# imironhead/ml_super_resolution

Measured on AMD Instinct MI355X. Metric: VDSR-20 training patches/sec (41x41, batch 256 per GPU); fwd HR megapixels/sec alongside, higher is better.
Workload: dtype f32; 1 GPU; BASELINE configs[2]: VDSR 20-layer 3x3x64 residual, RGB, batch 256x41x41 per GPU, fwd+bwd+TF-Adam, random-init weights; global_batch=256, patch=41, parallelism=dp1

## Files before the change

### include/srx.h

```cpp
#ifndef SRX_H_
#define SRX_H_

#include <stddef.h>
#include <stdint.h>

#ifdef __cplusplus
extern "C" {
#endif

typedef void* srx_stream_t;

typedef enum {
    SRX_OK = 0,
    SRX_ERR_BAD_ARG = -1,
    SRX_ERR_UNSUPPORTED = -2,
    SRX_ERR_WORKSPACE = -3,
    SRX_ERR_LAUNCH = -4,
    SRX_ERR_ALIGN = -5
} srx_status;

typedef enum { SRX_PAD_SAME = 0, SRX_PAD_VALID = 1 } srx_pad_mode;

typedef enum {
    SRX_ACT_NONE = 0,
    SRX_ACT_RELU = 1,
    SRX_ACT_TANH = 2,
    SRX_ACT_LRELU = 3,
    SRX_ACT_SIGMOID = 4
} srx_act;

typedef enum { SRX_OP_FWD = 0, SRX_OP_BWD_DATA = 1, SRX_OP_BWD_FILTER = 2 } srx_conv_op;

typedef enum { SRX_PRECISION_FP32 = 0, SRX_PRECISION_BF16X3 = 1 } srx_precision;

typedef struct {
    int32_t N, H, W, Cin, Cout, KH, KW;
    int32_t stride;
    int32_t pad_mode;
    int32_t act;
    int32_t post_add_relu;
    int32_t precision;
    int32_t subpixel_r;
} srx_conv_desc;

const char* srx_version(void);
const char* srx_last_error(void);

int srx_set_conv_path(int pipelined);

int srx_set_wgrad_path(int path);

int srx_conv_chain(const srx_conv_desc* d, int op, int in_act, int layers, const float* const* x, const float* const* w,
                   const float* const* bias, const float* const* aux, float* const* y, srx_stream_t stream);

int srx_conv_chain_supported(const srx_conv_desc* d, int op, int in_act);

int srx_set_chain(int on);

int srx_set_chain_fixed(int on);

int srx_conv2d_precision_supported(const srx_conv_desc* d, int op);

size_t srx_conv2d_workspace_bytes(const srx_conv_desc* d, int op);

int srx_conv2d_fwd(const srx_conv_desc* d, const float* x, const float* w, const float* bias,
                   const float* skip, float* y, void* ws, size_t ws_bytes, srx_stream_t stream);

int srx_conv2d_bwd_data(const srx_conv_desc* d, const float* dpre, const float* w,
                        const float* x_in, int in_act, float* dx_out, void* ws, size_t ws_bytes,
                        srx_stream_t stream);

int srx_conv2d_bwd_data_acc(const srx_conv_desc* d, const float* dpre, const float* w, const float* dx_acc,
                            float* dx_out, void* ws, size_t ws_bytes, srx_stream_t stream);

int srx_conv2d_bwd_filter(const srx_conv_desc* d, const float* x, const float* dpre, float* dw,
                          float* dbias, const float* w_for_decay, float wd_scale, void* ws,
                          size_t ws_bytes, srx_stream_t stream);

int srx_conv2d_bwd_filter_partials(const srx_conv_desc* d, const float* x, const float* dpre, void* ws,
                                   size_t ws_bytes, int* n_partials, srx_stream_t stream);
int srx_conv2d_bwd_filter_reduce(const srx_conv_desc* d, const void* ws, int n_partials, float* dw,
                                 float* dbias, const float* w_for_decay, float wd_scale,
                                 srx_stream_t stream);

int srx_conv2d_bwd_filter_batch(const srx_conv_desc* d, int n_layers, const float* const* x, const float* const* dpre,
                                float* const* dw, float* const* dbias, const float* const* w_for_decay, float wd_scale,
                                void* ws, size_t ws_bytes, srx_stream_t stream);
size_t srx_conv2d_bwd_filter_batch_workspace_bytes(const srx_conv_desc* d, int n_layers);
int srx_conv2d_bwd_filter_batch_plan(const srx_conv_desc* d, int n_layers, int* wgs_per_layer, int* grid);
int srx_set_wgrad_batch(int on);

int srx_act_bwd(const float* dy, const float* y, float* dpre, size_t numel, int act,
                srx_stream_t stream);

int srx_depth_to_space(const float* in, float* out, int N, int H, int W, int C, int r,
                       srx_stream_t stream);

int srx_stream_copy(const void* in, void* out, size_t bytes, srx_stream_t stream);

int srx_espcn_forward(const float* x, const float* w1, const float* b1, const float* w2, const float* b2,
                      const float* w3, const float* b3, float* hr, int N, int H, int W, int r,
                      srx_stream_t stream);
int srx_espcn_forward_keep(const float* x, const float* w1, const float* b1, const float* w2, const float* b2,
                           const float* w3, const float* b3, float* t1, float* t2, float* y, int N, int H, int W, int r,
                           srx_stream_t stream);

int srx_srcnn_forward(const float* x, const float* w1, const float* b1, const float* w2, const float* b2,
                      const float* w3, const float* b3, float* y, int N, int H, int W, srx_stream_t stream);

int srx_space_to_depth(const float* in, float* out, int N, int H, int W, int C, int r,
                       srx_stream_t stream);

int srx_mse_fwd_bwd(const float* pred, const float* target, size_t numel, float inv_numel,
                    float* loss_out, int accumulate, float* dpred, void* scratch,
                    srx_stream_t stream);

int srx_l2_loss(const float* w, const float* mask, size_t numel, float scale, float* loss_out,
                int accumulate, void* scratch, srx_stream_t stream);

size_t srx_reduce_scratch_bytes(void);

int srx_adam_tf_step(float* w, const float* g, float* m, float* v, size_t numel, float lr,
                     float beta1, float beta2, float eps, int64_t t, float grad_scale,
                     srx_stream_t stream);

int srx_adam_tf_step_dev(float* w, const float* g, float* m, float* v, size_t numel, void* state,
                         float beta1, float beta2, float eps, float grad_scale, srx_stream_t stream);

int srx_momentum_clip_step(float* w, const float* g, float* acc, size_t numel, float lr,
                           float momentum, float cap, float grad_scale, srx_stream_t stream);

int srx_rownorm_loss_fwd_bwd(const float* pred, const float* target, size_t rows, size_t row_len,
                             float* loss_out, float* dpred, float* row_norms, srx_stream_t stream);

int srx_psnr(const float* a, const float* b, float* out, int N, size_t per_image, float max_val,
             srx_stream_t stream);

int srx_ssim(const float* a, const float* b, float* out, int N, int H, int W, int C, float max_val,
             void* scratch, srx_stream_t stream);
size_t srx_ssim_scratch_bytes(int N);

#define SRX_SCORES_MAX_CAND 4
#define SRX_SCORES_RGB 0
#define SRX_SCORES_Y   1
#define SRX_SCORES_MAX_TAP_STRIDE 46
typedef struct srx_scores_desc {
    int32_t N, H, W, C;
    int32_t n_cand;
    int32_t space;
    int32_t unit_clip;
    float   max_val;
} srx_scores_desc;
size_t srx_image_scores_scratch_bytes(const srx_scores_desc* d);
int srx_image_scores_plan(const srx_scores_desc* d, int* tile_h, int* tile_w, int* tiles_y, int* tiles_x);
size_t srx_image_scores_lds_bytes(const srx_scores_desc* d);
int srx_image_scores(const srx_scores_desc* d, const float* ref, const float* const* cand, float* out, void* scratch,
                     srx_stream_t stream);

int srx_saturate_u8(const float* x, uint8_t* out, size_t numel, srx_stream_t stream);

#define SRX_FEATURE_MOSAIC_TW 128
int srx_feature_mosaic_u8(const float* x, uint8_t* out, int N, int H, int W, srx_stream_t stream);

#define SRX_SUMMARY_PANEL_MAX_SRC 8
#define SRX_SUMMARY_RANGE_BLOCKS 256
typedef struct srx_panel_src {
    const float* x;
    int32_t W;
    int32_t reserved;
    int64_t row_pitch;
    int64_t image_pitch;
} srx_panel_src;
size_t srx_summary_panel_bytes(const srx_panel_src* srcs, int n_src, int N, int H, int r);
size_t srx_summary_panel_range_bytes(void);
int srx_summary_panel_u8(const srx_panel_src* srcs, int n_src, int N, int H, int r, const float* range_dev, uint8_t* out,
                         srx_stream_t stream);
int srx_summary_panel_range(const srx_panel_src* srcs, int n_src, int N, int H, int r, float* range_dev,
                            srx_stream_t stream);

int srx_affine(const float* x, float* out, size_t numel, float a, float b, srx_stream_t stream);


int srx_u8_to_unit_float(const uint8_t* in, float* out, size_t numel, srx_stream_t stream);

int srx_gaussian_blur(const float* in, float* out, float* tmp, int N, int H, int W, int C, float sigma,
                      srx_stream_t stream);

int srx_resize_bilinear(const float* in, float* out, int N, int H, int W, int C, int OH, int OW,
                        srx_stream_t stream);


typedef struct srx_patch_src {
    uint64_t offset;
    int32_t width, height;
    int32_t x, y;
    int32_t flip;
    float scaling_factor;
} srx_patch_src;

int srx_vdsr_patch_table_check(const srx_patch_src* table_host, int B, int S, size_t arena_bytes);

int srx_vdsr_patch_pairs(const uint8_t* arena, const srx_patch_src* table_dev, int B, int S,
                         float* sd, float* hd, srx_stream_t stream);


int srx_espcn_patch_table_check(const srx_patch_src* table_host, int n, int r, int p, size_t arena_bytes);

int srx_espcn_patch_pairs(const uint8_t* arena, const srx_patch_src* table_dev, int B, int r, int p,
                          float* lr, float* label, srx_stream_t stream);


#define SRX_ESPCN_EVAL_TILE 16

typedef struct srx_eval_image {
    uint64_t offset;
    int32_t width, height;
    uint64_t lr_offset;
    uint32_t first_tile;
    uint32_t reserved;
} srx_eval_image;

int srx_espcn_eval_table_check(const srx_eval_image* table_host, int n, int r, size_t arena_bytes, size_t lr_floats);

size_t srx_espcn_eval_tiles(const srx_eval_image* table_host, int n, int r);

int srx_espcn_eval_pairs(const uint8_t* arena, const srx_eval_image* table_dev, int n, int r,
                         float* lr, float* label, srx_stream_t stream);


int srx_enet_pairs_table_words(int S);

int srx_enet_pairs_tables(int S, int32_t* words_host);

int srx_enet_patch_table_check(const srx_patch_src* table_host, int B, int S, size_t arena_bytes);

int srx_enet_patch_pairs(const uint8_t* arena, const srx_patch_src* table_dev, int B, int S, const int32_t* tables_dev,
                         float* sd, float* bq, float* hd, srx_stream_t stream);


int srx_srcnn_pairs_band(int S, int f);

int srx_srcnn_pairs_lds_bytes(int S, int f);

// ... 95 lines not shown
```

### ml_super_resolution_amd/_lib.py

```python
import ctypes
import os

_HERE = os.path.dirname(os.path.abspath(__file__))
LIB_PATH = os.path.join(_HERE, 'libsrx.so')

SRX_OK = 0
PAD_SAME, PAD_VALID = 0, 1
ACT_NONE, ACT_RELU, ACT_TANH, ACT_LRELU, ACT_SIGMOID = 0, 1, 2, 3, 4
OP_FWD, OP_BWD_DATA, OP_BWD_FILTER = 0, 1, 2
PRECISION_FP32, PRECISION_BF16X3 = 0, 1
PRECISION_BY_NAME = {'highest': PRECISION_FP32, 'high': PRECISION_BF16X3}

ACT_BY_NAME = {None: ACT_NONE, 'none': ACT_NONE, 'relu': ACT_RELU, 'tanh': ACT_TANH,
               'lrelu': ACT_LRELU, 'leaky_relu': ACT_LRELU, 'sigmoid': ACT_SIGMOID}
PAD_BY_NAME = {'same': PAD_SAME, 'valid': PAD_VALID}

EXPORTS = [
    'srx_version', 'srx_last_error', 'srx_set_conv_path', 'srx_set_wgrad_path', 'srx_set_chain', 'srx_set_chain_fixed', 'srx_conv_chain', 'srx_conv_chain_supported', 'srx_conv2d_precision_supported', 'srx_conv2d_workspace_bytes', 'srx_conv2d_fwd',
    'srx_conv2d_bwd_data', 'srx_conv2d_bwd_filter', 'srx_conv2d_bwd_filter_partials', 'srx_conv2d_bwd_filter_reduce',
    'srx_conv2d_bwd_filter_batch', 'srx_conv2d_bwd_filter_batch_workspace_bytes', 'srx_conv2d_bwd_filter_batch_plan', 'srx_set_wgrad_batch', 'srx_act_bwd', 'srx_depth_to_space',
    'srx_space_to_depth', 'srx_stream_copy', 'srx_mse_fwd_bwd', 'srx_l2_loss', 'srx_reduce_scratch_bytes',
    'srx_adam_tf_step', 'srx_adam_tf_step_dev', 'srx_momentum_clip_step', 'srx_rownorm_loss_fwd_bwd', 'srx_psnr', 'srx_ssim', 'srx_ssim_scratch_bytes', 'srx_saturate_u8', 'srx_affine', 'srx_u8_to_unit_float', 'srx_gaussian_blur', 'srx_resize_bilinear',
    'srx_upsample_nearest', 'srx_upsample_nearest_bwd', 'srx_add_relu_grad',
    'srx_conv2d_bwd_data_acc', 'srx_conv3x3_blocked', 'srx_conv3x3_blocked_bwd_filter_workspace_bytes', 'srx_conv3x3_blocked_bwd_filter',
    'srx_conv3x3_blocked_ex', 'srx_conv3x3_blocked_bwd_filter_ex_workspace_bytes', 'srx_conv3x3_blocked_bwd_filter_ex',
    'srx_espcn_forward', 'srx_espcn_forward_keep', 'srx_debug_poison_lds', 'srx_srcnn_forward', 'srx_maxpool2x2', 'srx_maxpool2x2_bwd', 'srx_maxpool2x2_bwd_masked', 'srx_subsample2', 'srx_subsample2_bwd',
    'srx_channel_blocks_to_nhwc', 'srx_nhwc_to_channel_blocks', 'srx_channel_normalize', 'srx_channel_normalize_bwd',
    'srx_extract_patches16', 'srx_texture_gram', 'srx_texture_gram_bwd', 'srx_pil_resample_ksize', 'srx_pil_resample_coeffs', 'srx_resample_u8', 'srx_u8_to_pm1', 'srx_log_loss', 'srx_vgg_preprocess', 'srx_add_scaled', 'srx_resize_bicubic_tf', 'srx_column_sums', 'srx_gemm_workspace_bytes', 'srx_gemm',
    'srx_feature_mosaic_u8', 'srx_summary_panel_bytes', 'srx_summary_panel_range_bytes', 'srx_summary_panel_u8', 'srx_summary_panel_range',
    'srx_vdsr_patch_table_check', 'srx_vdsr_patch_pairs',
    'srx_espcn_patch_table_check', 'srx_espcn_patch_pairs',
    'srx_espcn_eval_table_check', 'srx_espcn_eval_tiles', 'srx_espcn_eval_pairs',
    'srx_enet_pairs_table_words', 'srx_enet_pairs_tables', 'srx_enet_patch_table_check', 'srx_enet_patch_pairs',
    'srx_image_scores_scratch_bytes', 'srx_image_scores_plan', 'srx_image_scores_lds_bytes', 'srx_image_scores',
    'srx_srcnn_pairs_band', 'srx_srcnn_pairs_lds_bytes', 'srx_srcnn_patch_table_check', 'srx_srcnn_patch_pairs',
]


class SrxError(RuntimeError):
    pass


class ConvDesc(ctypes.Structure):
    _fields_ = [(n, ctypes.c_int32) for n in
                ('N', 'H', 'W', 'Cin', 'Cout', 'KH', 'KW', 'stride', 'pad_mode', 'act',
                 'post_add_relu', 'precision', 'subpixel_r')]


class PatchSrc(ctypes.Structure):
    _fields_ = [('offset', ctypes.c_uint64), ('width', ctypes.c_int32), ('height', ctypes.c_int32), ('x', ctypes.c_int32),
                ('y', ctypes.c_int32), ('flip', ctypes.c_int32), ('scaling_factor', ctypes.c_float)]


class EvalImage(ctypes.Structure):
    _fields_ = [('offset', ctypes.c_uint64), ('width', ctypes.c_int32), ('height', ctypes.c_int32), ('lr_offset', ctypes.c_uint64),
                ('first_tile', ctypes.c_uint32), ('reserved', ctypes.c_uint32)]


ESPCN_EVAL_TILE = 16


class PanelSrc(ctypes.Structure):
    _fields_ = [('x', ctypes.c_void_p), ('W', ctypes.c_int32), ('reserved', ctypes.c_int32), ('row_pitch', ctypes.c_int64),
                ('image_pitch', ctypes.c_int64)]


class ScoresDesc(ctypes.Structure):
    _fields_ = [(n, ctypes.c_int32) for n in ('N', 'H', 'W', 'C', 'n_cand', 'space', 'unit_clip')] + [('max_val', ctypes.c_float)]


SCORES_MAX_CAND = 4
SCORES_RGB, SCORES_Y = 0, 1
SCORES_MAX_TAP_STRIDE = 46
SCORES_SPACE_BY_NAME = {'rgb': SCORES_RGB, 'y': SCORES_Y}


class GemmDesc(ctypes.Structure):
    _fields_ = ([(n, ctypes.c_int32) for n in ('M', 'N', 'K', 'batch')] +
                [(n, ctypes.c_int64) for n in ('a_row_stride', 'a_col_stride', 'a_batch_stride', 'b_row_stride',
                                               'b_col_stride', 'b_batch_stride', 'c_row_stride', 'c_col_stride',
                                               'c_batch_stride')] +
                [('alpha', ctypes.c_float), ('act', ctypes.c_int32), ('accumulate', ctypes.c_int32)])


_lib = None


def lib():
    global _lib
    if _lib is not None:
        return _lib
    if not os.path.exists(LIB_PATH):
        raise SrxError('libsrx.so not found at %s -- build it with `make -C %s` (or '
                       '__graft_entry__.build()); there is no CPU fallback' %
                       (LIB_PATH, os.path.join(_HERE, 'csrc')))
    import torch
    L = ctypes.CDLL(LIB_PATH)
    vp, sz, i, f = ctypes.c_void_p, ctypes.c_size_t, ctypes.c_int, ctypes.c_float
    dp = ctypes.POINTER(ConvDesc)
    L.srx_version.restype = ctypes.c_char_p
    L.srx_last_error.restype = ctypes.c_char_p
    L.srx_set_conv_path.argtypes = [i]
    L.srx_set_wgrad_path.argtypes = [i]
    L.srx_set_chain.argtypes = [i]
    L.srx_set_chain_fixed.argtypes = [i]
    L.srx_conv_chain_supported.argtypes = [dp, i, i]
    L.srx_conv_chain.argtypes = [dp, i, i, i, vp, vp, vp, vp, vp, vp]
    L.srx_conv2d_precision_supported.argtypes = [dp, i]
    L.srx_conv2d_workspace_bytes.argtypes = [dp, i]
    L.srx_conv2d_workspace_bytes.restype = sz
    L.srx_reduce_scratch_bytes.restype = sz
    L.srx_conv2d_fwd.argtypes = [dp, vp, vp, vp, vp, vp, vp, sz, vp]
    L.srx_conv2d_bwd_data.argtypes = [dp, vp, vp, vp, i, vp, vp, sz, vp]
    L.srx_conv2d_bwd_filter.argtypes = [dp, vp, vp, vp, vp, vp, f, vp, sz, vp]
    L.srx_conv2d_bwd_filter_partials.argtypes = [dp, vp, vp, vp, sz, ctypes.POINTER(ctypes.c_int), vp]
    L.srx_conv2d_bwd_filter_reduce.argtypes = [dp, vp, i, vp, vp, vp, f, vp]
    L.srx_conv2d_bwd_filter_batch.argtypes = [dp, i, vp, vp, vp, vp, vp, f, vp, sz, vp]
    L.srx_conv2d_bwd_filter_batch_workspace_bytes.argtypes = [dp, i]
    L.srx_conv2d_bwd_filter_batch_workspace_bytes.restype = sz
    L.srx_conv2d_bwd_filter_batch_plan.argtypes = [dp, i, ctypes.POINTER(ctypes.c_int), ctypes.POINTER(ctypes.c_int)]
    L.srx_set_wgrad_batch.argtypes = [i]
    L.srx_act_bwd.argtypes = [vp, vp, vp, sz, i, vp]
    L.srx_depth_to_space.argtypes = [vp, vp, i, i, i, i, i, vp]
    L.srx_space_to_depth.argtypes = [vp, vp, i, i, i, i, i, vp]
    L.srx_stream_copy.argtypes = [vp, vp, sz, vp]
    L.srx_mse_fwd_bwd.argtypes = [vp, vp, sz, f, vp, i, vp, vp, vp]
    L.srx_l2_loss.argtypes = [vp, vp, sz, f, vp, i, vp, vp]
    L.srx_adam_tf_step.argtypes = [vp, vp, vp, vp, sz, f, f, f, f, ctypes.c_int64, f, vp]
    L.srx_adam_tf_step_dev.argtypes = [vp, vp, vp, vp, sz, vp, f, f, f, f, vp]
    L.srx_momentum_clip_step.argtypes = [vp, vp, vp, sz, f, f, f, f, vp]
    L.srx_rownorm_loss_fwd_bwd.argtypes = [vp, vp, sz, sz, vp, vp, vp, vp]
    L.srx_psnr.argtypes = [vp, vp, vp, i, sz, f, vp]
    L.srx_ssim.argtypes = [vp, vp, vp, i, i, i, i, f, vp, vp]
    L.srx_ssim_scratch_bytes.argtypes = [i]
    L.srx_ssim_scratch_bytes.restype = sz
    sp, ip = ctypes.POINTER(ScoresDesc), ctypes.POINTER(ctypes.c_int)
    L.srx_image_scores_scratch_bytes.argtypes = [sp]
    L.srx_image_scores_scratch_bytes.restype = sz
    L.srx_image_scores_plan.argtypes = [sp, ip, ip, ip, ip]
    L.srx_image_scores_lds_bytes.argtypes = [sp]
    L.srx_image_scores_lds_bytes.restype = sz
    L.srx_image_scores.argtypes = [sp, vp, vp, vp, vp, vp]
    L.srx_saturate_u8.argtypes = [vp, vp, sz, vp]
    L.srx_feature_mosaic_u8.argtypes = [vp, vp, i, i, i, vp]
    L.srx_summary_panel_bytes.argtypes = [vp, i, i, i, i]
    L.srx_summary_panel_bytes.restype = sz
    L.srx_summary_panel_range_bytes.restype = sz
    L.srx_summary_panel_u8.argtypes = [vp, i, i, i, i, vp, vp, vp]
    L.srx_summary_panel_range.argtypes = [vp, i, i, i, i, vp, vp]
    L.srx_vdsr_patch_table_check.argtypes = [vp, i, i, sz]
    L.srx_vdsr_patch_pairs.argtypes = [vp, vp, i, i, vp, vp, vp]
    L.srx_espcn_patch_table_check.argtypes = [vp, i, i, i, sz]
    L.srx_espcn_patch_pairs.argtypes = [vp, vp, i, i, i, vp, vp, vp]
    L.srx_espcn_eval_table_check.argtypes = [vp, i, i, sz, sz]
    L.srx_espcn_eval_tiles.argtypes = [vp, i, i]
    L.srx_espcn_eval_tiles.restype = sz
    L.srx_espcn_eval_pairs.argtypes = [vp, vp, i, i, vp, vp, vp]
    L.srx_enet_pairs_table_words.argtypes = [i]
    L.srx_enet_pairs_tables.argtypes = [i, vp]
    L.srx_enet_patch_table_check.argtypes = [vp, i, i, sz]
    L.srx_enet_patch_pairs.argtypes = [vp, vp, i, i, vp, vp, vp, vp, vp]
    L.srx_srcnn_pairs_band.argtypes = [i, i]
    L.srx_srcnn_pairs_lds_bytes.argtypes = [i, i]
    L.srx_srcnn_patch_table_check.argtypes = [vp, i, i, i, i, sz]
    L.srx_srcnn_patch_pairs.argtypes = [vp, vp, i, i, i, i, vp, vp, vp]
    L.srx_affine.argtypes = [vp, vp, sz, f, f, vp]
    L.srx_u8_to_unit_float.argtypes = [vp, vp, sz, vp]
    L.srx_gaussian_blur.argtypes = [vp, vp, vp, i, i, i, i, f, vp]
    L.srx_resize_bilinear.argtypes = [vp, vp, i, i, i, i, i, i, vp]
    L.srx_upsample_nearest.argtypes = [vp, vp, i, i, i, i, i, vp]
    L.srx_upsample_nearest_bwd.argtypes = [vp, vp, i, i, i, i, i, vp]
    L.srx_add_relu_grad.argtypes = [vp, vp, vp, vp, sz, vp]
    L.srx_conv2d_bwd_data_acc.argtypes = [dp, vp, vp, vp, vp, vp, sz, vp]
    L.srx_espcn_forward.argtypes = [vp] * 8 + [i, i, i, i, vp]
    L.srx_espcn_forward_keep.argtypes = [vp] * 10 + [i, i, i, i, vp]
    L.srx_debug_poison_lds.argtypes = [vp]
    L.srx_srcnn_forward.argtypes = [vp, vp, vp, vp, vp, vp, vp, vp, i, i, i, vp]
    L.srx_conv3x3_blocked.argtypes = [vp, vp, vp, vp, i, vp, i, i, i, i, i, i, i, vp]
    L.srx_conv3x3_blocked_bwd_filter_workspace_bytes.restype = sz
    L.srx_conv3x3_blocked_bwd_filter_workspace_bytes.argtypes = [i, i, i, i, i]
    L.srx_conv3x3_blocked_bwd_filter.argtypes = [vp, vp, vp, vp, i, i, i, i, i, vp, sz, vp]
    L.srx_conv3x3_blocked_ex.argtypes = [vp, vp, vp, vp, i, vp, i, i, i, i, i, i, i, i, vp]
    L.srx_conv3x3_blocked_bwd_filter_ex_workspace_bytes.restype = sz
    L.srx_conv3x3_blocked_bwd_filter_ex_workspace_bytes.argtypes = [i, i, i, i, i, i]
    L.srx_conv3x3_blocked_bwd_filter_ex.argtypes = [vp, vp, vp, vp, i, i, i, i, i, i, vp, sz, vp]
    L.srx_texture_gram.argtypes = [vp, vp, i, i, i, i, f, vp]
    L.srx_texture_gram_bwd.argtypes = [vp, vp, vp, i, i, i, i, f, f, vp]
    L.srx_pil_resample_ksize.argtypes = [i, i, i]
    L.srx_pil_resample_coeffs.argtypes = [i, i, i, vp, vp]
    L.srx_resample_u8.argtypes = [vp, vp, ctypes.c_long, i, i, ctypes.c_long, vp, vp, i, vp]
    L.srx_u8_to_pm1.argtypes = [vp, vp, sz, vp]
    L.srx_maxpool2x2.argtypes = [vp, vp, i, i, i, i, vp]
    L.srx_maxpool2x2_bwd.argtypes = [vp, vp, vp, i, i, i, i, vp]
    L.srx_maxpool2x2_bwd_masked.argtypes = [vp, vp, vp, i, i, i, i, i, vp]
    L.srx_subsample2.argtypes = [vp, vp, i, i, i, i, i, i, vp]
    L.srx_subsample2_bwd.argtypes = [vp, vp, i, i, i, i, i, i, vp]
    L.srx_channel_blocks_to_nhwc.argtypes = [vp, vp, sz, i, vp]
    L.srx_nhwc_to_channel_blocks.argtypes = [vp, vp, sz, i, vp]
    L.srx_channel_normalize.argtypes = [vp, vp, sz, i, f, vp]
    L.srx_channel_normalize_bwd.argtypes = [vp, vp, vp, sz, i, f, vp]
    L.srx_extract_patches16.argtypes = [vp, vp, i, i, i, i, i, vp]
    L.srx_log_loss.argtypes = [vp, f, i, f, f, f, vp, i, vp, vp]
    L.srx_vgg_preprocess.argtypes = [vp, vp, sz, i, vp]
    L.srx_column_sums.argtypes = [vp, vp, i, i, i, vp]
    L.srx_add_scaled.argtypes = [vp, vp, vp, sz, f, f, vp]
    L.srx_resize_bicubic_tf.argtypes = [vp, vp, i, i, i, i, i, i, vp]
    L.srx_gemm_workspace_bytes.argtypes = [i, i, i, i]
    L.srx_gemm_workspace_bytes.restype = sz
    L.srx_gemm.argtypes = [ctypes.POINTER(GemmDesc), vp, vp, vp, vp, vp, sz, vp]
    for name in EXPORTS:
        getattr(L, name)
    _lib = L
    return L


def check(rc, what):
    if rc != SRX_OK:
        raise SrxError('%s failed (status %d): %s' % (what, rc, lib().srx_last_error().decode()))
```

### ml_super_resolution_amd/csrc/conv_kernels.hip.h

```cpp
#pragma once
#include <hip/hip_runtime.h>
#include <stdint.h>
#include <type_traits>

namespace srx {

typedef float f32x4 __attribute__((ext_vector_type(4)));

enum { ACT_NONE = 0, ACT_RELU = 1, ACT_TANH = 2, ACT_LRELU = 3, ACT_SIGMOID = 4 };

struct ConvArgs {
    const float* x;
    const float* w;
    const float* bias;
    const float* skip;
    const float* mask;
    float* y;
    int N, H, W, OH, OW, Cin, Cout;
    int pad_t, pad_l;
    int TH, TW, NTX, RS;
    int units_total;
    int act, post_relu, mask_act;
    float inv_rs;
    int stagger;
// ... 2627 lines not shown
                       "+a"(bnext[21]), "+a"(bnext[22]), "+a"(bnext[23]), "+a"(bnext[24]), "+a"(bnext[25]),        \
                       "+a"(bnext[26]), "+a"(bnext[27]), "+a"(bnext[28]), "+a"(bnext[29]), "+a"(bnext[30]));       \
        _Pragma("unroll") for (int j = 0; j < U; ++j)                                                              \
            asm volatile("v_accvgpr_read_b32 %0, %1" : "=v"(bcur[j]) : "a"(bnext[j]));                             \
    } while (0)

    int u = u0;
    int n, h, th;
    tile_of(u, n, h, th);
    [[maybe_unused]] unsigned long long t_loop = 0, t_end = 0;
    [[maybe_unused]] const unsigned long long t_begin = SRX_STAMP();
    __syncthreads();
    {
        StageSeq qi, qc;
        stage_setup(qi, qc, h, th, 0, true);
        stage_tile_scalar<CINP, 6>(qi, qc, SG, x_rsrc(n), voff_lane, wl_lane);
        dpre_window_now(b_rsrc(n, h, th));
        lds_barrier();
        SRX_TAKE_OVER_B();
    }
    int cur_buf = 0;
    while (u < u1) {
        tile_of(u, n, h, th);
        const int un_ = u + th;
        const bool has_next = un_ < u1;
        int n2 = n, h2 = h, th2 = th;
        if (has_next) tile_of(un_, n2, h2, th2);
        StageSeq qi, qc;
        stage_setup(qi, qc, h2, th2, cur_buf ^ 1, has_next);
        const __amdgpu_buffer_rsrc_t xrs = x_rsrc(n2);
        const __amdgpu_buffer_rsrc_t brs_pf = b_rsrc(n2, h2, has_next ? th2 : 0);

        auto xaddr = [&](int k, int i) -> unsigned {
            if (i == U - 1) return (unsigned)(xw[k] + dX + (OWC - 1) * PS * 4);
            const int r = i >= U ? THC : i / SPR, j = i >= U ? 0 : i % SPR;
            return (unsigned)(xw[k] + (r * RSZ + 4 * j) * PS * 4);
        };
        auto read_x = [&](int k, int i) -> f32x4 { return *(lds_f32x4*)(uintptr_t)xaddr(k, i); };
        f32x4 ring[RN];
#pragma unroll
        for (int f = 0; f < LA; ++f) ring[f] = read_x(f % QW, f / QW);

        const unsigned long long ts_l = SRX_STAMP();
        f32x4 stg[NPASSES];
        auto step = [&](auto IC) {
            constexpr int i = decltype(IC)::value;
            const float b = bcur[i];
            bsum += b;
            unsigned long long smk = 0, smt = 0;
            int sso = 0;
#pragma unroll
            for (int k = 0; k < QW; ++k) {
                const int idx = (i * QW + k) % RN;
                const int kk = k + LA;
                ring[(idx + LA) % RN] = read_x(kk % QW, i + kk / QW);
                mfma4_wgrad(acc[k], ring[idx], b);
                if ((k == 1 && 2 * i < U) || (k == 7 && 2 * i + 1 < U)) {
                    const int p = 2 * i + (k == 7 ? 1 : 0);
                    if (p == U - 1) {
                        bnext[p] = dpre_fire_imm<0>(brs_pf, vX, 0);
                    } else {
                        const int r = p / SPR, j = p % SPR;
                        const int vb = j < 4 ? vb0 : (j < 8 ? vb1 : vb2);
                        const int so = r == 0 ? 0 : (r == 1 ? srow1 : srow2);
                        switch (j % 4) {
                            case 0: bnext[p] = dpre_fire_imm<0>(brs_pf, vb, so); break;
                            case 1: bnext[p] = dpre_fire_imm<16 * COUTC>(brs_pf, vb, so); break;
                            case 2: bnext[p] = dpre_fire_imm<32 * COUTC>(brs_pf, vb, so); break;
                            default: bnext[p] = dpre_fire_imm<48 * COUTC>(brs_pf, vb, so); break;
                        }
                    }
                }
                if constexpr (i < NPASSES) {
                    if (k == 2) { if (i > 0) stage_next<PPP * CINP * 4>(qi, SG.JP1, SG.rowfix_g); }
                    if (k == 3) stage_mask_a(qi, SG, smk, smt);
                    if (k == 4) stage_mask_b(qi, smk, smt, sso);
                    if (k == 6) stg[i < NPASSES ? i : 0] = stage_fire_a(smk, sso, xrs, voff_lane);
                }
                if constexpr (i == NPASSES) { if (k == 2) stage_next<PPP * CINP * 4>(qi, SG.JP1, SG.rowfix_g); }
                if constexpr (i >= C0 && i < C0 + NPASSES) {
                    constexpr int jj = i - C0;
                    constexpr int after = 1 + 3 * (NPASSES - 1 - jj) + (U - 2 * NPASSES);
                    if (k == 0) stage_commit_a(after >= 14 ? 14 : (after & ~1), qc, stage_mask_full(qc, SG), wl_lane, stg[jj < NPASSES ? jj : 0]);
                    if (k == 4) stage_next<PPP * PS * 4>(qc, SG.JP1, SG.rowfix_l);
                }
            }
        };
#define SRX_ONE_STEP(I) step(std::integral_constant<int, I>{});
        SRX_ONE_STEP(0) SRX_ONE_STEP(1) SRX_ONE_STEP(2) SRX_ONE_STEP(3) SRX_ONE_STEP(4) SRX_ONE_STEP(5) SRX_ONE_STEP(6) SRX_ONE_STEP(7)
        SRX_ONE_STEP(8) SRX_ONE_STEP(9) SRX_ONE_STEP(10) SRX_ONE_STEP(11) SRX_ONE_STEP(12) SRX_ONE_STEP(13) SRX_ONE_STEP(14) SRX_ONE_STEP(15)
        SRX_ONE_STEP(16) SRX_ONE_STEP(17) SRX_ONE_STEP(18) SRX_ONE_STEP(19) SRX_ONE_STEP(20) SRX_ONE_STEP(21) SRX_ONE_STEP(22) SRX_ONE_STEP(23)
        SRX_ONE_STEP(24) SRX_ONE_STEP(25) SRX_ONE_STEP(26) SRX_ONE_STEP(27) SRX_ONE_STEP(28) SRX_ONE_STEP(29) SRX_ONE_STEP(30)
#undef SRX_ONE_STEP
        SRX_TAKE_OVER_B();
        const unsigned long long ts_e = SRX_STAMP();
        t_loop += ts_e - ts_l;
        {
            const int flip = __builtin_amdgcn_readfirstlane(cur_buf ? -buf_bytes : buf_bytes);
#pragma unroll
            for (int k = 0; k < QW; ++k) { xw[k] += flip; SRX_PIN(xw[k]); }
        }
        stage_tile_scalar<CINP, 6>(qi, qc, SG, xrs, voff_lane, wl_lane);
        lds_barrier();
        cur_buf ^= 1;
        u = un_;
        t_end += SRX_STAMP() - ts_e;
    }
#undef SRX_TAKE_OVER_B
#ifdef SRX_TRACE
    if (a.trace && lane == 0) {
        unsigned long long* tr = a.trace + ((size_t)blockIdx.x * 4 + wave) * 12;
        tr[0] = t_begin; tr[1] = SRX_STAMP(); tr[2] = t_loop; tr[3] = t_end; tr[4] = 0;
    }
#endif

    asm volatile("s_nop 15\n\ts_nop 7" ::: "memory");
#pragma unroll
    for (int k = 0; k < QW; ++k) {
        const int q = qpart + k * NQP;
        if (q >= Q) continue;
#pragma unroll
        for (int g = 0; g < 4; ++g) {
#pragma unroll
            for (int r = 0; r < 4; ++r) {
                const int R = 64 * q + 4 * (4 * kq + r) + g;
                const int tap = R / CINP, ci = R % CINP;
                if (R < ROWS && ci < a.Cin && co_ok) pw[((size_t)tap * a.Cin + ci) * a.Cout + co] = acc[k][g][r];
            }
        }
    }
    bsum += __shfl_xor(bsum, 16);
    bsum += __shfl_xor(bsum, 32);
    if (qpart == 0 && kq == 0 && co_ok) pw[(size_t)TAPS * a.Cin * a.Cout + co] = bsum;
}

template <int KH, int KW, int CINP, int NCH, int OWC>
__global__ __launch_bounds__(256, 1) void wgrad_rows_full_kernel(const WgradArgs a) {
    const long G_ = gridDim.x;
    const int u0 = (int)(((long)blockIdx.x * a.units_total) / G_);
    const int u1 = (int)(((long)(blockIdx.x + 1) * a.units_total) / G_);
    wgrad_rows_full_body<KH, KW, CINP, NCH, OWC>(a, a.x, a.dpre, a.part + (size_t)blockIdx.x * a.part_stride, u0, u1);
}

struct WgradBatchPtrs {
    const float* x[kChainMax];
    const float* dpre[kChainMax];
};
struct WgradBatchOut {
    float* dw[kChainMax];
    float* dbias[kChainMax];
    const float* w[kChainMax];
};

template <int KH, int KW, int CINP, int NCH, int OWC>
__global__ __launch_bounds__(256, 1) void wgrad_rows_batch_kernel(const WgradArgs a, const WgradBatchPtrs c, const int wpl) {
    const int layer = __builtin_amdgcn_readfirstlane((int)blockIdx.x / wpl);
    const int sub = (int)blockIdx.x - layer * wpl;
    const int u0 = (int)(((long)sub * a.units_total) / wpl);
    const int u1 = (int)(((long)(sub + 1) * a.units_total) / wpl);
    wgrad_rows_full_body<KH, KW, CINP, NCH, OWC>(a, c.x[layer], c.dpre[layer], a.part + (size_t)blockIdx.x * a.part_stride, u0, u1);
}

}
```

### ml_super_resolution_amd/csrc/conv_narrow.hip

```cpp
#include "launchers.h"
namespace srx {
typedef float f32x3 __attribute__((ext_vector_type(3)));
typedef unsigned u32x3v __attribute__((ext_vector_type(3)));

template <int CTRL>
__device__ __forceinline__ float dpp_add(float v) {
    const int moved = __builtin_amdgcn_update_dpp(0, __float_as_int(v), CTRL, 0xf, 0xf, false);
    return v + __int_as_float(moved);
}

struct PixWalk {
    int n, oh, ow;
    __device__ __forceinline__ void init(unsigned p, int OH, int OW) {
        const unsigned t = p / (unsigned)OW;
        ow = (int)(p - t * (unsigned)OW);
        n = (int)(t / (unsigned)OH);
        oh = (int)(t - (unsigned)n * (unsigned)OH);
    }
    __device__ __forceinline__ void step16(int OH, int OW) { step(16, OH, OW); }
    __device__ __forceinline__ void step(int d, int OH, int OW) {
        ow += d;
        while (ow >= OW) {
            ow -= OW;
            oh += 1;
            if (oh == OH) { oh = 0; n += 1; }
        }
    }
};
template <int KH, int KW>
__device__ __forceinline__ void tap_offsets(int (&off)[KH * KW], const PixWalk& q, bool live, int H, int W, int pad_t, int pad_l,
                                            int PB, int lane_b) {
    const int centre = ((q.n * H + q.oh - pad_t) * W + (q.ow - pad_l)) * PB + lane_b;
    bool rok[KH], cok[KW];
#pragma unroll
    for (int kh = 0; kh < KH; ++kh) rok[kh] = live && (unsigned)(q.oh + kh - pad_t) < (unsigned)H;
#pragma unroll
    for (int kw = 0; kw < KW; ++kw) cok[kw] = (unsigned)(q.ow + kw - pad_l) < (unsigned)W;
#pragma unroll
    for (int kh = 0; kh < KH; ++kh)
#pragma unroll
        for (int kw = 0; kw < KW; ++kw)
            off[kh * KW + kw] = (rok[kh] && cok[kw]) ? centre + (kh * W + kw) * PB : kOobOffset;
}

template <int KH, int KW, int CIN, int CO>
__global__ __launch_bounds__(256) void conv_narrow_kernel(const ConvArgs a, long total_px, int iters) {
    static_assert(CIN == 64, "16 lanes x 4 channels per pixel");
    constexpr int TAPS = KH * KW;
    const int c4 = threadIdx.x & 15;
    const int sub = threadIdx.x >> 4;
    float wr[TAPS][4][CO];
#pragma unroll
    for (int t = 0; t < TAPS; ++t)
#pragma unroll
        for (int e = 0; e < 4; ++e)
#pragma unroll
            for (int c = 0; c < CO; ++c) wr[t][e][c] = a.w[((size_t)t * CIN + 4 * c4 + e) * CO + c];
    float bias[CO];
#pragma unroll
    for (int c = 0; c < CO; ++c) bias[c] = a.bias ? a.bias[c] : 0.0f;
    const __amdgpu_buffer_rsrc_t xrs = __builtin_amdgcn_make_buffer_rsrc(const_cast<float*>(a.x), 0,
                                                                         a.N * a.H * a.W * CIN * 4, 0x00020000);
    const unsigned p0 = blockIdx.x * (unsigned)iters * 16u + sub;
    PixWalk q;
    q.init(p0 < (unsigned)total_px ? p0 : 0u, a.OH, a.OW);
    for (int it = 0; it < iters; ++it, q.step16(a.OH, a.OW)) {
        const unsigned p = p0 + (unsigned)it * 16u;
        const bool live = p < (unsigned)total_px;
        int off[TAPS];
        tap_offsets<KH, KW>(off, q, live, a.H, a.W, a.pad_t, a.pad_l, CIN * 4, 16 * c4);
        f32x4 v[TAPS];
#pragma unroll
        for (int tp = 0; tp < TAPS; ++tp)
            v[tp] = __builtin_bit_cast(f32x4, __builtin_amdgcn_raw_buffer_load_b128(xrs, off[tp], 0, 0));
        float acc[CO];
#pragma unroll
        for (int c = 0; c < CO; ++c) acc[c] = 0.0f;
#pragma unroll
        for (int tp = 0; tp < TAPS; ++tp)
#pragma unroll
            for (int e = 0; e < 4; ++e)
#pragma unroll
                for (int c = 0; c < CO; ++c) acc[c] = fmaf(v[tp][e], wr[tp][e][c], acc[c]);
#pragma unroll
        for (int c = 0; c < CO; ++c) {
            float r = acc[c];
            r = dpp_add<0xB1>(r);
            r = dpp_add<0x4E>(r);
            r = dpp_add<0x124>(r);
            r = dpp_add<0x128>(r);
            acc[c] = r;
        }
        if (live && c4 < CO) {
            float r = (c4 == 0) ? acc[0] : (c4 == 1 ? acc[1 < CO ? 1 : 0] : acc[2 < CO ? 2 : 0]);
            r = act_apply(r + ((c4 == 0) ? bias[0] : (c4 == 1 ? bias[1 < CO ? 1 : 0] : bias[2 < CO ? 2 : 0])), a.act);
            const size_t o = (size_t)p * CO + c4;
            if (a.skip) r += a.skip[o];
            if (a.post_relu) r = act_apply(r, a.post_relu);
            a.y[o] = r;
        }
    }
}

template <int KH, int KW, bool NOUT, int CW = 64>
__global__ __launch_bounds__(256) void wgrad_narrow_kernel(const WgradArgs a, long total_px, int iters) {
    constexpr int TAPS = KH * KW, CN = 3;
    constexpr int LPP = CW / 4;
    constexpr int PPI = 256 / LPP;
    constexpr int NB = NOUT ? CN : 4;
    constexpr int NV = TAPS * 4 * CN + NB;
    __shared__ float red[4 * NV * LPP];
    const int c4 = threadIdx.x & (LPP - 1);
    const int sub = threadIdx.x / LPP;
    const int wave = threadIdx.x >> 6;
    float acc[NV];
#pragma unroll
    for (int i = 0; i < NV; ++i) acc[i] = 0.0f;
    const __amdgpu_buffer_rsrc_t xrs = __builtin_amdgcn_make_buffer_rsrc(
        const_cast<float*>(a.x), 0, a.N * a.H * a.W * (NOUT ? CW : CN) * 4, 0x00020000);
    const __amdgpu_buffer_rsrc_t drs = __builtin_amdgcn_make_buffer_rsrc(
        const_cast<float*>(a.dpre), 0, a.N * a.OH * a.OW * (NOUT ? CN : CW) * 4, 0x00020000);
    const unsigned p0 = blockIdx.x * (unsigned)iters * (unsigned)PPI + sub;
    PixWalk q;
    q.init(p0 < (unsigned)total_px ? p0 : 0u, a.OH, a.OW);
    for (int it = 0; it < iters; ++it, q.step(PPI, a.OH, a.OW)) {
        const unsigned p = p0 + (unsigned)it * (unsigned)PPI;
        const bool live = p < (unsigned)total_px;
        int off[TAPS];
        tap_offsets<KH, KW>(off, q, live, a.H, a.W, a.pad_t, a.pad_l, (NOUT ? CW : CN) * 4, NOUT ? 16 * c4 : 0);
        if constexpr (NOUT) {
            const f32x3 d = __builtin_bit_cast(f32x3, __builtin_amdgcn_raw_buffer_load_b96(drs, live ? (int)(p * CN * 4) : kOobOffset, 0, 0));
            f32x4 v[TAPS];
#pragma unroll
            for (int tp = 0; tp < TAPS; ++tp)
                v[tp] = __builtin_bit_cast(f32x4, __builtin_amdgcn_raw_buffer_load_b128(xrs, off[tp], 0, 0));
#pragma unroll
            for (int tp = 0; tp < TAPS; ++tp)
#pragma unroll
                for (int e = 0; e < 4; ++e)
#pragma unroll
                    for (int c = 0; c < CN; ++c) acc[(tp * 4 + e) * CN + c] = fmaf(v[tp][e], d[c], acc[(tp * 4 + e) * CN + c]);
#pragma unroll
            for (int c = 0; c < CN; ++c) acc[TAPS * 4 * CN + c] += d[c];
        } else {
            const f32x4 d = __builtin_bit_cast(f32x4, __builtin_amdgcn_raw_buffer_load_b128(
                drs, live ? (int)((p * CW + 4 * c4) * 4) : kOobOffset, 0, 0));
            f32x3 v[TAPS];
#pragma unroll
            for (int tp = 0; tp < TAPS; ++tp)
                v[tp] = __builtin_bit_cast(f32x3, __builtin_amdgcn_raw_buffer_load_b96(xrs, off[tp], 0, 0));
#pragma unroll
            for (int tp = 0; tp < TAPS; ++tp)
#pragma unroll
                for (int cn = 0; cn < CN; ++cn)
#pragma unroll
                    for (int e = 0; e < 4; ++e) acc[(tp * CN + cn) * 4 + e] = fmaf(v[tp][cn], d[e], acc[(tp * CN + cn) * 4 + e]);
#pragma unroll
            for (int e = 0; e < 4; ++e) acc[TAPS * 4 * CN + e] += d[e];
        }
    }
#pragma unroll
    for (int i = 0; i < NV; ++i) {
        float r = acc[i];
#pragma unroll
        for (int o = LPP; o < 64; o <<= 1) r += __shfl_xor(r, o);
        if (sub % (64 / LPP) == 0) red[(wave * NV + i) * LPP + c4] = r;
    }
    __syncthreads();
    float* part = a.part + (size_t)blockIdx.x * a.part_stride;
    const int wn = TAPS * CW * CN;
    for (int q = threadIdx.x; q < NV * LPP; q += 256) {
        const int i = q / LPP, l = q % LPP;
        const float r = (red[(0 * NV + i) * LPP + l] + red[(1 * NV + i) * LPP + l]) +
                        (red[(2 * NV + i) * LPP + l] + red[(3 * NV + i) * LPP + l]);
        if (i < TAPS * 4 * CN) {
            int idx;
            if constexpr (NOUT) {
                const int c = i % CN, te = i / CN, e = te & 3, tp = te >> 2;
                idx = (tp * CW + 4 * l + e) * CN + c;
            } else {
                const int e = i & 3, tc = i >> 2;
                idx = tc * CW + 4 * l + e;
            }
            part[idx] = r;
        } else {
            const int b = i - TAPS * 4 * CN;
            if constexpr (NOUT) {
                if (l == 0) part[wn + b] = r;
            } else {
                part[wn + 4 * l + b] = r;
            }
        }
    }
}

bool launch_wgrad_narrow(const ConvKey& k, const WgradArgs& a, int grid, hipStream_t s, hipError_t* err) {
    if (k.kh != 3 || k.kw != 3) return false;
    const bool nout = a.Cin == 64 && a.Cout == 3, nin = a.Cin == 3 && a.Cout == 64, nin32 = a.Cin == 3 && a.Cout == 32;
    if (!nout && !nin && !nin32) return false;
    const long total = (long)a.N * a.OH * a.OW;
    if (total >= (1L << 31) - 4096 || (long)a.N * a.H * a.W * 64 * 4 >= (1L << 31) - 4096 || total * 64 * 4 >= (1L << 31) - 4096)
        return false;
    const long ppi = nin32 ? 32 : 16;
    const int iters = (int)((total + ppi * grid - 1) / (ppi * grid));
    if (nout)
        hipLaunchKernelGGL((wgrad_narrow_kernel<3, 3, true>), dim3(grid), dim3(256), 0, s, a, total, iters);
    else if (nin)
        hipLaunchKernelGGL((wgrad_narrow_kernel<3, 3, false>), dim3(grid), dim3(256), 0, s, a, total, iters);
    else
        hipLaunchKernelGGL((wgrad_narrow_kernel<3, 3, false, 32>), dim3(grid), dim3(256), 0, s, a, total, iters);
    *err = hipGetLastError();
    return true;
}

bool launch_conv_narrow(const ConvKey& k, const ConvArgs& a, hipStream_t s, hipError_t* err) {
    if (k.wt || a.Cout != 3 || a.mask) return false;
    if ((long)a.N * a.H * a.W * a.Cin * 4 >= (1L << 31) - 4096) return false;
    const long total = (long)a.N * a.OH * a.OW;
    int iters = 16;
    while (iters > 1 && total / (16L * iters) < 2048) iters >>= 1;
    const long blocks = (total + 16L * iters - 1) / (16L * iters);
    if (total >= (1L << 31) - 4096) return false;
    if (k.kh == 3 && k.kw == 3 && a.Cin == 64) {
        hipLaunchKernelGGL((conv_narrow_kernel<3, 3, 64, 3>), dim3((unsigned)blocks), dim3(256), 0, s, a, total, iters);
    } else {
        return false;
    }
    *err = hipGetLastError();
    return true;
}
}
```

### ml_super_resolution_amd/csrc/launchers.h

```cpp
#pragma once
#include "conv_kernels.hip.h"

namespace srx {

struct ConvKey {
    int kh, kw, cinp, nch;
    bool wt;
};

bool launch_conv_k3c64(const ConvKey& k, const ConvArgs& a, int grid, size_t lds, hipStream_t s, hipError_t* err);
bool launch_conv_k3c32(const ConvKey& k, const ConvArgs& a, int grid, size_t lds, hipStream_t s, hipError_t* err);
bool launch_conv_c4(const ConvKey& k, const ConvArgs& a, int grid, size_t lds, hipStream_t s, hipError_t* err);
bool launch_conv_misc(const ConvKey& k, const ConvArgs& a, int grid, size_t lds, hipStream_t s, hipError_t* err);
bool launch_pipe_k3c64(const ConvKey& k, const ConvArgs& a, int grid, size_t lds, hipStream_t s, hipError_t* err);
bool launch_pipe_other(const ConvKey& k, const ConvArgs& a, int grid, size_t lds, hipStream_t s, hipError_t* err);
bool launch_wgrad_narrow(const ConvKey& k, const WgradArgs& a, int grid, hipStream_t s, hipError_t* err);
bool launch_conv_narrow(const ConvKey& k, const ConvArgs& a, hipStream_t s, hipError_t* err);
bool launch_conv_1x1(const ConvKey& k, const ConvArgs& a, long min_pixels, hipStream_t s, hipError_t* err);
bool launch_conv_rows3x3(const ConvKey& k, const ConvArgs& a, long min_pixels, hipStream_t s, hipError_t* err);
bool launch_conv_pack3(const ConvKey& k, const ConvArgs& a, long min_pixels, hipStream_t s, hipError_t* err);
bool launch_conv_kwrows(const ConvKey& k, const ConvArgs& a, long min_pixels, hipStream_t s, hipError_t* err);
bool launch_pipe_strip(const ConvKey& k, const ConvArgs& a, int grid, size_t lds, hipStream_t s, hipError_t* err);
bool launch_conv_generic(const ConvKey& k, const ConvArgs& a, int grid, size_t lds, hipStream_t s, hipError_t* err);
bool launch_wgrad(const ConvKey& k, const WgradArgs& a, int grid, size_t lds, hipStream_t s, hipError_t* err);
bool launch_wgrad_generic(const ConvKey& k, const WgradArgs& a, int grid, size_t lds, hipStream_t s, hipError_t* err);
bool launch_wgrad_lin(const ConvKey& k, const WgradArgs& a, int grid, size_t lds, hipStream_t s, hipError_t* err);
bool launch_wgrad_lin_pack3(const ConvKey& k, const WgradArgs& a, int grid, size_t lds, hipStream_t s, hipError_t* err);
bool launch_wgrad_lin_strip(const ConvKey& k, const WgradArgs& a, int grid, size_t lds, hipStream_t s, hipError_t* err);
bool launch_wgrad_pipe(const ConvKey& k, const WgradArgs& a, int grid, size_t lds, hipStream_t s, hipError_t* err);
bool launch_wgrad_kwcols(const ConvKey& k, const WgradArgs& a, int max_partials, long min_pixels, int* n_partials, hipStream_t s, hipError_t* err);
bool launch_wgrad_1x1(const ConvKey& k, const WgradArgs& a, int max_partials, int* n_partials, hipStream_t s, hipError_t* err);
bool launch_wgrad_rows_full(const ConvKey& k, const WgradArgs& a, int grid, size_t lds, hipStream_t s, hipError_t* err);
bool launch_wgrad_rows_strip(const ConvKey& k, const WgradArgs& a, int grid, size_t lds, hipStream_t s, hipError_t* err);
bool launch_wgrad_lin_pairs(const ConvKey& k, const WgradPairs& q, int grid, int pairs, bool strips, size_t lds, hipStream_t s, hipError_t* err);

__attribute__((weak)) hipError_t launch_conv_chain(bool wt, bool aux, bool fixed, const ConvArgs& a, const ChainPtrs& c, int grid, size_t lds, hipStream_t s);

__attribute__((weak)) hipError_t launch_wgrad_rows_batch(const WgradArgs& a, const WgradBatchPtrs& c, int wpl, int layers, size_t lds, hipStream_t s);
__attribute__((weak)) hipError_t launch_wgrad_batch_reduce(const float* part, int wpl, int layers, int stride, int wn, int cout,
                                                           const WgradBatchOut& o, float wd, hipStream_t s);

hipError_t launch_reduce_partials(const float* part, int G, int stride, int wn, int cout, float* dw, float* dbias,
                                  const float* w, float wd, hipStream_t s);
hipError_t launch_reduce_partials_pairs(const float* part, int G, int stride, int wn, int cout, float* dw, float* dbias,
                                        int pairs, int cob, hipStream_t s);

template <typename K, typename A>
inline hipError_t launch_with_lds(K kernel, const A& a, int grid, size_t lds, hipStream_t s, int grid_y = 1) {
    static thread_local const void* configured[64];
    static thread_local int n_configured = 0;
    const void* fn = reinterpret_cast<const void*>(kernel);
    bool known = false;
    for (int i = 0; i < n_configured; ++i) known |= (configured[i] == fn);
    if (!known) {
        hipError_t e = hipFuncSetAttribute(fn, hipFuncAttributeMaxDynamicSharedMemorySize, 160 * 1024);
        if (e != hipSuccess) return e;
        if (n_configured < 64) configured[n_configured++] = fn;
    }
    hipLaunchKernelGGL(kernel, dim3(grid, grid_y), dim3(256), lds, s, a);
    return hipGetLastError();
}

template <typename K>
inline hipError_t launch_chain_with_lds(K kernel, const ConvArgs& a, const ChainPtrs& c, int grid, size_t lds, hipStream_t s) {
    static thread_local const void* configured[8];
    static thread_local int n_configured = 0;
    const void* fn = reinterpret_cast<const void*>(kernel);
    bool known = false;
    for (int i = 0; i < n_configured; ++i) known |= (configured[i] == fn);
    if (!known) {
        hipError_t e = hipFuncSetAttribute(fn, hipFuncAttributeMaxDynamicSharedMemorySize, 160 * 1024);
        if (e != hipSuccess) return e;
        if (n_configured < 8) configured[n_configured++] = fn;
    }
    hipLaunchKernelGGL(kernel, dim3(grid), dim3(256), lds, s, a, c);
    return hipGetLastError();
}

#define SRX_CONV_CASE(KH, KW, CINP, NCH, WT, MINW)                                                        \
    if (k.kh == KH && k.kw == KW && k.cinp == CINP && k.nch == NCH && k.wt == WT) {                       \
        if (a.skip || a.mask)                                                                             \
            *err = launch_with_lds(conv_mfma_kernel<KH, KW, CINP, NCH, WT, MINW, true>, a, grid, lds, s); \
        else                                                                                              \
            *err = launch_with_lds(conv_mfma_kernel<KH, KW, CINP, NCH, WT, MINW, false>, a, grid, lds, s);\
        return true;                                                                                      \
    }
#define SRX_PIPE_CASE_FWD(KH, KW, CINP, NCH)                                                              \
    if (k.kh == KH && k.kw == KW && k.cinp == CINP && k.nch == NCH && !k.wt) {                            \
        if (a.skip)                                                                                       \
            *err = launch_with_lds(conv_pipe_kernel<KH, KW, CINP, NCH, false, 2>, a, grid, lds, s);       \
        else                                                                                              \
            *err = launch_with_lds(conv_pipe_kernel<KH, KW, CINP, NCH, false, 0>, a, grid, lds, s);       \
        return true;                                                                                      \
    }
#define SRX_PIPE_CASE_DGRAD(KH, KW, CINP, NCH)                                                            \
    if (k.kh == KH && k.kw == KW && k.cinp == CINP && k.nch == NCH && k.wt) {                             \
        if (a.mask)                                                                                       \
            *err = launch_with_lds(conv_pipe_kernel<KH, KW, CINP, NCH, true, 1>, a, grid, lds, s);        \
        else                                                                                              \
            *err = launch_with_lds(conv_pipe_kernel<KH, KW, CINP, NCH, true, 0>, a, grid, lds, s);        \
        return true;                                                                                      \
    }
#define SRX_PIPE_STRIP_CASE(KH, KW, CINP, NCH)                                                            \
    if (k.kh == KH && k.kw == KW && k.cinp == CINP && k.nch == NCH && !k.wt) {                            \
        if (a.skip)                                                                                       \
            *err = launch_with_lds(conv_pipe_strip_kernel<KH, KW, CINP, NCH, false, 2>, a, grid, lds, s); \
        else                                                                                              \
            *err = launch_with_lds(conv_pipe_strip_kernel<KH, KW, CINP, NCH, false, 0>, a, grid, lds, s); \
        return true;                                                                                      \
    }                                                                                                     \
    if (k.kh == KH && k.kw == KW && k.cinp == CINP && k.nch == NCH && k.wt) {                             \
        if (a.mask)                                                                                       \
            *err = launch_with_lds(conv_pipe_strip_kernel<KH, KW, CINP, NCH, true, 1>, a, grid, lds, s);  \
        else                                                                                              \
            *err = launch_with_lds(conv_pipe_strip_kernel<KH, KW, CINP, NCH, true, 0>, a, grid, lds, s);  \
        return true;                                                                                      \
    }
#define SRX_PIPE_STRIP_CASE_FWD2(KH, KW, CINP, NCH)                                                       \
    if (k.kh == KH && k.kw == KW && k.cinp == CINP && k.nch == NCH && !k.wt && !a.skip && !a.mask) {      \
        if (a.act == ACT_TANH)                                                                            \
            *err = launch_with_lds(conv_pipe_strip_kernel<KH, KW, CINP, NCH, false, 3>, a, grid, lds, s); \
        else                                                                                              \
            *err = launch_with_lds(conv_pipe_strip_kernel<KH, KW, CINP, NCH, false, 0>, a, grid, lds, s); \
        return true;                                                                                      \
    }
#define SRX_PIPE_STRIP_CASE_D2S(KH, KW, CINP, NCH)                                                        \
    if (k.kh == KH && k.kw == KW && k.cinp == CINP && k.nch == NCH && !k.wt && !a.skip && !a.mask && a.d2s_r) { \
        *err = launch_with_lds(conv_pipe_strip_kernel<KH, KW, CINP, NCH, false, 4>, a, grid, lds, s);     \
        return true;                                                                                      \
    }
#define SRX_WGRAD_LIN_CASE(KH, KW, CINP, NCH, MINW)                                                       \
    if (k.kh == KH && k.kw == KW && k.cinp == CINP && k.nch == NCH) {                                     \
        *err = launch_with_lds(wgrad_lin_kernel<KH, KW, CINP, NCH, MINW>, a, grid, lds, s);               \
        return true;                                                                                      \
    }
#define SRX_WGRAD_LIN_STRIP_CASE(KH, KW, CINP, NCH, MINW)                                                 \
    if (k.kh == KH && k.kw == KW && k.cinp == CINP && k.nch == NCH) {                                     \
        *err = launch_with_lds(wgrad_lin_strip_kernel<KH, KW, CINP, NCH, MINW>, a, grid, lds, s);         \
        return true;                                                                                      \
    }
#define SRX_WGRAD_PIPE_CASE(KH, KW, CINP, NCH)                                                            \
    if (k.kh == KH && k.kw == KW && k.cinp == CINP && k.nch == NCH) {                                     \
        *err = launch_with_lds(wgrad_pipe_kernel<KH, KW, CINP, NCH>, a, grid, lds, s);                    \
        return true;                                                                                      \
    }
#define SRX_WGRAD_CASE(KH, KW, CINP, NCH, MINW)                                                           \
    if (k.kh == KH && k.kw == KW && k.cinp == CINP && k.nch == NCH) {                                     \
        *err = launch_with_lds(wgrad_mfma_kernel<KH, KW, CINP, NCH, MINW>, a, grid, lds, s);              \
        return true;                                                                                      \
    }

}
```

### ml_super_resolution_amd/csrc/srx_api.hip

```cpp
#include <math.h>
#include <stdarg.h>
#include <atomic>
#include <stdio.h>
#include <stdlib.h>
#include <string.h>

#include "../../include/srx.h"
#include "elementwise.h"
#include "launchers.h"
#include "bf16x3.h"
#include "patch_pairs.h"
#include "image_scores.h"

using namespace srx;

namespace {

thread_local char g_err[512] = "";

struct Knobs {
    int pipe_default, narrow, wgrad_lin, wgrad_pipe, wgrad_pipe_strip, wgrad_rows_full, wgrad_1x1, wgrad_pack3, kwrows_min_pixels, big_route_min_pixels, strip_d2s, conv_1x1_min_pixels, pack3_dgrad;
    int chain, chain_fixed, wgrad_batch;
    unsigned long long* trace;
    int dbg;
};
int env_int(const char* name, int dflt) { const char* e = getenv(name); return e ? atoi(e) : dflt; }
Knobs read_knobs() {
    Knobs k;
    k.pipe_default = env_int("SRX_PIPE", 1);
    k.narrow = env_int("SRX_NARROW", 1);
    k.wgrad_lin = env_int("SRX_WGRAD_LIN", 1);
    k.wgrad_pipe = env_int("SRX_WGRAD_PIPE", 1);
    k.wgrad_pipe_strip = env_int("SRX_WGRAD_PIPE_STRIP", 1);
    k.kwrows_min_pixels = env_int("SRX_KWROWS_MIN_PIXELS", 4096);
    k.big_route_min_pixels = env_int("SRX_BIG_ROUTE_MIN_PIXELS", 60000);
    k.conv_1x1_min_pixels = env_int("SRX_CONV_1X1_MIN_PIXELS", 100000);
    k.pack3_dgrad = env_int("SRX_PACK3_DGRAD", 1);
    k.strip_d2s = env_int("SRX_STRIP_D2S", 1);
    k.wgrad_rows_full = env_int("SRX_WGRAD_ROWS_FULL", 1);
    k.wgrad_1x1 = env_int("SRX_WGRAD_1X1", 1);
    k.wgrad_pack3 = env_int("SRX_WGRAD_PACK3", 1);
    k.chain = env_int("SRX_CHAIN", 1);
    k.chain_fixed = env_int("SRX_CHAIN_FIXED", 1);
    k.wgrad_batch = env_int("SRX_WGRAD_BATCH", 1);
    k.trace = nullptr;
    k.dbg = 0;
#ifdef SRX_TRACE
    { const char* tp = getenv("SRX_TRACE_PTR"); k.trace = tp ? (unsigned long long*)strtoull(tp, nullptr, 0) : nullptr; }
    k.dbg = env_int("SRX_DBG", 0);
#endif
    return k;
}
const Knobs& knobs() { static const Knobs k = read_knobs(); return k; }

std::atomic<int> g_use_pipe{-1};
std::atomic<int> g_chain{-1};
int use_chain() { const int v = g_chain.load(std::memory_order_relaxed); return v < 0 ? (knobs().chain ? 1 : 0) : v; }
std::atomic<int> g_chain_fixed{-1};
int use_chain_fixed() { const int v = g_chain_fixed.load(std::memory_order_relaxed); return v < 0 ? (knobs().chain_fixed ? 1 : 0) : v; }
std::atomic<int> g_wgrad_batch{-1};
int use_wgrad_batch() { const int v = g_wgrad_batch.load(std::memory_order_relaxed); return v < 0 ? (knobs().wgrad_batch ? 1 : 0) : v; }
int use_pipe() { const int v = g_use_pipe.load(std::memory_order_relaxed); return v < 0 ? knobs().pipe_default : v; }
std::atomic<int> g_wgrad_path{-1};
int wgrad_path_default() { return !knobs().wgrad_lin ? 0 : ((knobs().wgrad_pipe || knobs().wgrad_pipe_strip) ? 2 : 1); }
int wgrad_path() { const int v = g_wgrad_path.load(std::memory_order_relaxed); return v < 0 ? wgrad_path_default() : v; }

int cu_count() {
    static std::atomic<int> cached[64];
    int dev = 0;
    if (hipGetDevice(&dev) != hipSuccess || dev < 0 || dev >= 64) { (void)hipGetLastError(); return 256; }
    int n = cached[dev].load(std::memory_order_relaxed);
    if (n > 0) return n;
    if (hipDeviceGetAttribute(&n, hipDeviceAttributeMultiprocessorCount, dev) != hipSuccess || n <= 0) {
        (void)hipGetLastError();
        n = 256;
    }
    if (n > 256) n = 256;
    cached[dev].store(n, std::memory_order_relaxed);
    return n;
}

int fail(int code, const char* fmt, ...) {
    va_list ap;
    va_start(ap, fmt);
    vsnprintf(g_err, sizeof(g_err), fmt, ap);
    va_end(ap);
    return code;
}
}
namespace srx {
int set_error(int code, const char* fmt, ...) {
    va_list ap;
    va_start(ap, fmt);
    vsnprintf(g_err, sizeof(g_err), fmt, ap);
    va_end(ap);
    return code;
}
}
namespace {

inline bool aligned16(const void* p) { return (reinterpret_cast<uintptr_t>(p) & 15u) == 0; }

constexpr size_t kLdsBudget = 80 * 1024 - 336;
constexpr int kMaxGridLimit = 512;
inline int max_grid() { return 2 * cu_count(); }
inline int pipe_grid() { return cu_count(); }

struct Plan {
    int KH, KW, cinp, nch;
    int pad_t, pad_l, OH, OW;
    int TH, TW, NTX, RS;
    int units_total, grid;
    size_t lds_bytes;
};

int pad_channels(int c) { return c <= 4 ? 4 : (c <= 32 ? 32 : (c <= 64 ? 64 : -1)); }
int chunks_for(int c) { return c <= 16 ? 1 : (c <= 32 ? 2 : (c <= 64 ? 4 : -1)); }

int make_plan(int N, int H, int W, int OH, int OW, int in_c, int out_c, int KH, int KW, int pad_t, int pad_l,
              Plan* p, bool lean_epilogue = true) {
    p->KH = KH; p->KW = KW;
    p->cinp = pad_channels(in_c);
    p->nch = chunks_for(out_c);
    if (p->cinp < 0 || p->nch < 0)
        return fail(SRX_ERR_UNSUPPORTED, "channel counts %d->%d outside the kernel set (<=64)", in_c, out_c);
    p->pad_t = pad_t; p->pad_l = pad_l; p->OH = OH; p->OW = OW;
    const int ps = (p->cinp == 4) ? 4 : p->cinp + 4;
    const size_t slot_bytes = (size_t)ps * 4;
    const size_t max_slots = kLdsBudget / slot_bytes;
    int RS = W + pad_l;
    if (RS < OW + KW - 1 - (KW - 1 - pad_l)) RS = OW + pad_l;
    if (RS < OW + KW - 1 - pad_l) RS = OW + KW - 1 - pad_l;
    int TW = OW, NTX = 1;
    long th_max = ((long)max_slots - (KW - 1)) / RS - (KH - 1);
    const int kMaxGrid = max_grid();
    if (th_max < 3) {
        for (TW = 32; TW >= 8; TW >>= 1) {
            RS = TW + KW - 1;
            th_max = ((long)max_slots - (KW - 1)) / RS - (KH - 1);
            if (th_max >= 1) break;
        }
        if (th_max < 1) return fail(SRX_ERR_UNSUPPORTED, "filter %dx%d too large for the LDS tile", KH, KW);
        NTX = (OW + TW - 1) / TW;
    }
    if (th_max > OH) th_max = OH;
    if (th_max > 16) th_max = 16;
    const long rows_total = (long)N * NTX * OH;
    bool small = false, rows_split = false;
    if (rows_total / th_max < 2 * kMaxGrid && KH == 3 && KW == 3 && p->cinp >= 16 && in_c == p->cinp && lean_epilogue &&
        (out_c & 3) == 0 && RS >= 256 / (p->cinp / 4) && (NTX > 1 ? p->nch == 4 : 16 * (4 / p->nch) <= OW)) {
        rows_split = true;
    } else if (rows_total / th_max < 2 * kMaxGrid) {
        const int npart = 4 / p->nch;
        double best_cost = 1e30;
        int best_th = 1;
        for (int th = 1; th <= (int)th_max; ++th) {
            const long tiles = (long)N * NTX * ((OH + th - 1) / th);
            const long slots = tiles < kMaxGrid ? tiles : kMaxGrid;
            const long per_wg = (tiles + slots - 1) / slots;
            const long sub = ((long)th * TW + 15) / 16;
            const double cost = (double)per_wg * (1.5 + (double)((sub + npart - 1) / npart));
            if (cost <= best_cost + 1e-9) { best_cost = cost; best_th = th; }
        }
        th_max = best_th;
        small = true;
    }
    int best = (int)th_max;
    double best_eff = 0.0;
    for (int th = (int)th_max; !small && th >= (int)((th_max + 1) / 2) && th >= 1; --th) {
        const int px = th * TW;
        const double eff = (double)px / (16.0 * ((px + 15) / 16));
        if (eff > best_eff + 1e-9) { best_eff = eff; best = th; }
    }
    p->TH = best; p->TW = TW; p->NTX = NTX; p->RS = RS;
    p->units_total = (int)rows_total;
    long g = rows_total / p->TH;
    if (small) g = (long)N * NTX * ((OH + p->TH - 1) / p->TH);
    if (rows_split) g = rows_total;
    if (g < 1) g = 1;
    p->grid = (int)(g < kMaxGrid ? g : kMaxGrid);
    p->lds_bytes = ((size_t)(p->TH + KH - 1) * RS + (KW - 1)) * slot_bytes;
    return SRX_OK;
}

int check_desc(const srx_conv_desc* d) {
    if (!d) return fail(SRX_ERR_BAD_ARG, "null descriptor");
    if (d->N <= 0 || d->H <= 0 || d->W <= 0 || d->Cin <= 0 || d->Cout <= 0 || d->KH <= 0 || d->KW <= 0)
        return fail(SRX_ERR_BAD_ARG, "non-positive dimension in descriptor");
    if (d->stride != 1 && d->stride != 2) return fail(SRX_ERR_UNSUPPORTED, "stride %d: strides 1 and 2 are implemented", d->stride);
    if (d->stride == 2 && d->subpixel_r > 1) return fail(SRX_ERR_UNSUPPORTED, "stride 2 with the sub-pixel store is not implemented");
    if (d->pad_mode != SRX_PAD_SAME && d->pad_mode != SRX_PAD_VALID) return fail(SRX_ERR_BAD_ARG, "bad pad_mode");
    if (d->act < SRX_ACT_NONE || d->act > SRX_ACT_SIGMOID) return fail(SRX_ERR_BAD_ARG, "bad activation");
    if (d->post_add_relu != 0 && d->post_add_relu != SRX_ACT_RELU && d->post_add_relu != SRX_ACT_LRELU)
        return fail(SRX_ERR_BAD_ARG, "post_add_relu must be 0, SRX_ACT_RELU (1) or SRX_ACT_LRELU (3)");
    if (d->precision != SRX_PRECISION_FP32 && d->precision != SRX_PRECISION_BF16X3)
        return fail(SRX_ERR_BAD_ARG, "bad precision %d: 0 (exact fp32) or 1 (bf16x3)", d->precision);
    if (d->subpixel_r < 0 || d->subpixel_r > 16) return fail(SRX_ERR_BAD_ARG, "bad subpixel_r %d", d->subpixel_r);
    if (d->subpixel_r > 1 && d->Cout % (d->subpixel_r * d->subpixel_r))
        return fail(SRX_ERR_BAD_ARG, "subpixel_r %d: Cout %d is not a multiple of r*r", d->subpixel_r, d->Cout);
    if (d->pad_mode == SRX_PAD_VALID && (d->H < d->KH || d->W < d->KW))
        return fail(SRX_ERR_BAD_ARG, "VALID convolution with input smaller than the filter");
    if ((long)d->H * d->W * (long)(d->Cin > d->Cout ? d->Cin : d->Cout) >= (1L << 31))
        return fail(SRX_ERR_UNSUPPORTED, "one image has >= 2^31 elements: beyond the kernels' 32-bit in-image offsets");
    if ((long)d->N * d->H * 64 >= (1L << 31))
        return fail(SRX_ERR_UNSUPPORTED, "too many rows for 32-bit unit indexing");
    return SRX_OK;
}

void geometry(const srx_conv_desc* d, int* pad_t, int* pad_l, int* OH, int* OW) {
    const int s = d->stride;
    if (d->pad_mode == SRX_PAD_SAME) {
        *OH = (d->H + s - 1) / s; *OW = (d->W + s - 1) / s;
        const int ph = (*OH - 1) * s + d->KH - d->H, pw = (*OW - 1) * s + d->KW - d->W;
        *pad_t = (ph > 0 ? ph : 0) / 2; *pad_l = (pw > 0 ? pw : 0) / 2;
// ... 452 lines not shown
    const int use_lin = wpath >= 1 && !s2;
    const int kPipeGrid = pipe_grid();
    const bool lin_ok = use_lin && p.NTX == 1 && OW >= 4 && p.RS >= 8 && p.RS == d->W + pl && (long)p.TH * OW * d->Cout * 4 < (1L << 30) &&
                        (long)d->H * d->W * d->Cin * 4 < (1L << 31) - 4096;
    const size_t lin_lds = p.lds_bytes + 4 * (size_t)((p.cinp == 4) ? 4 : p.cinp + 4) * 4;
    const int use_wpipe = wpath >= 2 && knobs().wgrad_pipe;
    const int wppp = (p.cinp >= 16) ? 256 / (p.cinp / 4) : 256;
    int wgrid = p.grid;
    bool wdone = false;
    if (knobs().wgrad_1x1 && wpath >= 1 && !s2) {
        int n1 = 0;
        if (launch_wgrad_1x1(k, a, p.grid, &n1, s, &err)) { wdone = true; wgrid = n1; }
    }
    if (!wdone && knobs().big_route_min_pixels >= 0 && wpath >= 1 && !s2) {
        int n1 = 0;
        if (launch_wgrad_kwcols(k, a, p.grid, knobs().big_route_min_pixels, &n1, s, &err)) { wdone = true; wgrid = n1; }
    }
    if (!wdone && use_wpipe && knobs().wgrad_rows_full && lin_ok && d->KH == 3 && d->KW == 3 && d->Cin == 64 && d->Cout == 64 && OW == 41 && d->W == 41 &&
        pl == 1 && pt == 1 && p.RS == 42) {
        WgradArgs ap = a;
        ap.TH = 3;
        ap.zero_slot = (3 + 3) * 42 + 2;
        wgrid = p.grid < kPipeGrid ? p.grid : kPipeGrid;
        wdone = launch_wgrad_rows_full(k, ap, wgrid, 2 * (size_t)(ap.zero_slot + 4) * (64 + 4) * 4, s, &err);
        if (!wdone) wgrid = p.grid;
    }
    if (!wdone && use_wpipe && lin_ok && d->Cin == p.cinp && p.RS >= wppp && 2 * lin_lds <= 160 * 1024) {
        const int kWin = 14 * 4;
        int best_th = 0;
        double best_waste = 1e9;
        for (int th = p.TH; th >= 1; --th) {
            const long pos = (long)th * p.RS, padded = (pos + kWin - 1) / kWin * kWin;
            const double waste = (double)(padded - pos) / (double)pos;
            const bool fits = padded + 2L * p.RS + 6 <= (long)a.zero_slot + 4;
            if (fits && waste < best_waste - 1e-9) { best_waste = waste; best_th = th; }
        }
        if (best_th > 0 && best_waste <= 0.10) {
            WgradArgs ap = a;
            ap.TH = best_th;
            wgrid = p.grid < kPipeGrid ? p.grid : kPipeGrid;
            wdone = launch_wgrad_pipe(k, ap, wgrid, 2 * lin_lds, s, &err);
            if (!wdone) wgrid = p.grid;
        }
    }
    {
        if (!wdone && knobs().narrow && !s2) wdone = launch_wgrad_narrow(k, a, p.grid, s, &err);
    }
    const bool lin_strip_ok = use_lin && p.NTX > 1 && d->Cin == p.cinp && p.RS >= wppp && p.TW >= 4 && lin_lds <= 80 * 1024 &&
                              (OW % p.TW == 0 || OW % p.TW >= 4) && p.RS <= 3 * wppp &&
                              (long)d->H * d->W * d->Cin * 4 < (1L << 31) - 4096 && (long)OH * OW * d->Cout * 4 < (1L << 30);
    const bool rows_ok = wpath >= 2 && knobs().wgrad_pipe_strip && !s2 && p.NTX > 1 && p.TW == 32 && p.RS == 32 + d->KW - 1 &&
                         d->Cin == p.cinp && 2 * lin_lds <= 160 * 1024 &&
                         (long)d->H * d->W * d->Cin * 4 < (1L << 31) - 4096 && (long)OH * OW * d->Cout * 4 < (1L << 30);
    if (!wdone && rows_ok) {
        wgrid = p.grid < kPipeGrid ? p.grid : kPipeGrid;
        wdone = launch_wgrad_rows_strip(k, a, wgrid, 2 * lin_lds, s, &err);
        if (!wdone) wgrid = p.grid;
    }
    if (!wdone && knobs().wgrad_pack3 && lin_ok && lin_lds <= 80 * 1024 && d->Cin == 3) wdone = launch_wgrad_lin_pack3(k, a, p.grid, lin_lds, s, &err);
    if (wdone) {
    } else if (lin_strip_ok && launch_wgrad_lin_strip(k, a, p.grid, lin_lds, s, &err)) {
    } else if (lin_ok && lin_lds <= 80 * 1024 && launch_wgrad_lin(k, a, p.grid, lin_lds, s, &err)) {
    } else if (!launch_wgrad(k, a, p.grid, wg_lds, s, &err) && !(wg_lds <= 80 * 1024 && launch_wgrad_generic(k, a, p.grid, wg_lds, s, &err)))
        return fail(SRX_ERR_UNSUPPORTED, "no wgrad instance for %dx%d, Cin<=%d, Cout chunks %d%s", d->KH, d->KW, p.cinp,
                    p.nch, s2 ? " at stride 2" : "");
    if (err != hipSuccess) return fail(SRX_ERR_LAUNCH, "wgrad launch failed: %s", hipGetErrorString(err));
    *n_partials = wgrid;
    return SRX_OK;
}

int srx_conv2d_bwd_filter_reduce(const srx_conv_desc* d, const void* ws, int n_partials, float* dw, float* dbias,
                                 const float* w_for_decay, float wd_scale, srx_stream_t stream) {
    int rc = check_desc(d);
    if (rc) return rc;
    if (!ws || !dw) return fail(SRX_ERR_BAD_ARG, "null tensor pointer");
    if (d->precision == SRX_PRECISION_BF16X3 && (rc = bf16x3_supported(d, SRX_OP_BWD_FILTER)) != SRX_OK) return rc;
    if (n_partials <= 0 || n_partials > kMaxGridLimit) return fail(SRX_ERR_BAD_ARG, "bad partial count %d", n_partials);
    const size_t wn = (size_t)d->KH * d->KW * d->Cin * d->Cout;
    hipError_t err = launch_reduce_partials((const float*)ws, n_partials, (int)part_stride(d), (int)wn, d->Cout, dw, dbias,
                                            w_for_decay, wd_scale, (hipStream_t)stream);
    if (err != hipSuccess) return fail(SRX_ERR_LAUNCH, "reduce launch failed: %s", hipGetErrorString(err));
    return SRX_OK;
}

int srx_conv2d_bwd_filter(const srx_conv_desc* d, const float* x, const float* dpre, float* dw, float* dbias,
                          const float* w_for_decay, float wd_scale, void* ws, size_t ws_bytes, srx_stream_t stream) {
    if (!dw) return fail(SRX_ERR_BAD_ARG, "null tensor pointer");
    int n = 0;
    const int rc = srx_conv2d_bwd_filter_partials(d, x, dpre, ws, ws_bytes, &n, stream);
    if (rc) return rc;
    return srx_conv2d_bwd_filter_reduce(d, ws, n, dw, dbias, w_for_decay, wd_scale, stream);
}

namespace {
int wgrad_batch_plan(const srx_conv_desc* d, int layers, WgradArgs* a, int* wpl, int* grid) {
    int rc = check_desc(d);
    if (rc) return rc;
    if (!use_wgrad_batch()) return fail(SRX_ERR_UNSUPPORTED, "bwd_filter_batch: switched off (srx_set_wgrad_batch / SRX_WGRAD_BATCH)");
    if (!launch_wgrad_rows_batch || !launch_wgrad_batch_reduce) return fail(SRX_ERR_UNSUPPORTED, "bwd_filter_batch: this build has no batch kernels");
    if (layers < 2 || layers > kChainMax) return fail(SRX_ERR_UNSUPPORTED, "bwd_filter_batch: %d layers (2..%d)", layers, kChainMax);
    if (d->precision != SRX_PRECISION_FP32) return fail(SRX_ERR_UNSUPPORTED, "bwd_filter_batch: precision %d (exact fp32 only)", d->precision);
    if (d->KH != 3 || d->KW != 3 || d->Cin != 64 || d->Cout != 64 || d->stride != 1 || d->pad_mode != SRX_PAD_SAME)
        return fail(SRX_ERR_UNSUPPORTED, "bwd_filter_batch: only 3x3 64->64 stride-1 SAME layers");
    if (d->W != 41) return fail(SRX_ERR_UNSUPPORTED, "bwd_filter_batch: W %d (only 41-pixel rows: wgrad_rows_full_kernel's shape)", d->W);
    if (wgrad_path() < 2 || !knobs().wgrad_pipe || !knobs().wgrad_rows_full)
        return fail(SRX_ERR_UNSUPPORTED, "bwd_filter_batch: the filter-gradient path is not wgrad_rows_full_kernel's (srx_set_wgrad_path)");
    int pt, pl, OH, OW;
    geometry(d, &pt, &pl, &OH, &OW);
    Plan p;
    rc = make_plan(d->N, d->H, d->W, OH, OW, d->Cin, d->Cout, d->KH, d->KW, pt, pl, &p);
    if (rc) return rc;
    wgrad_tile_for_linear_walk(d, &p);
    const bool ok = p.NTX == 1 && p.RS == 42 && pl == 1 && pt == 1 && OW == 41 && (long)d->H * d->W * d->Cin * 4 < (1L << 31) - 4096;
    if (!ok) return fail(SRX_ERR_UNSUPPORTED, "bwd_filter_batch: the shape is not on wgrad_rows_full_kernel's route");
    const long rows = (long)d->N * OH;
    long w = pipe_grid() / layers;
    if (w > rows) w = rows;
    if (w < 1) return fail(SRX_ERR_UNSUPPORTED, "bwd_filter_batch: %d layers on a grid of %d", layers, pipe_grid());
    *wpl = (int)w;
    *grid = pipe_grid();
    memset(a, 0, sizeof(*a));
    a->part_stride = (int)part_stride(d);
    a->N = d->N; a->H = d->H; a->W = d->W; a->OH = OH; a->OW = OW; a->Cin = d->Cin; a->Cout = d->Cout;
    a->pad_t = pt; a->pad_l = pl; a->TH = 3; a->TW = p.TW; a->NTX = p.NTX; a->RS = p.RS;
    a->units_total = p.units_total; a->inv_rs = 1.0f / (float)p.RS;
    a->stride = 1;
    a->zero_slot = (3 + 3) * 42 + 2;
    return SRX_OK;
}
}

int srx_set_wgrad_batch(int on) {
    const int old = g_wgrad_batch.exchange(on < 0 ? -1 : (on ? 1 : 0), std::memory_order_relaxed);
    return old < 0 ? (knobs().wgrad_batch ? 1 : 0) : old;
}

int srx_conv2d_bwd_filter_batch_plan(const srx_conv_desc* d, int n_layers, int* wgs_per_layer, int* grid) {
    WgradArgs a;
    int wpl = 0, g = 0;
    const int rc = wgrad_batch_plan(d, n_layers, &a, &wpl, &g);
    if (rc) { wpl = 0; g = 0; }
    if (wgs_per_layer) *wgs_per_layer = wpl;
    if (grid) *grid = g;
    return rc;
}

size_t srx_conv2d_bwd_filter_batch_workspace_bytes(const srx_conv_desc* d, int n_layers) {
    WgradArgs a;
    int wpl = 0, g = 0;
    if (wgrad_batch_plan(d, n_layers, &a, &wpl, &g) != SRX_OK) return 0;
    return (size_t)n_layers * wpl * part_stride(d) * sizeof(float);
}

int srx_conv2d_bwd_filter_batch(const srx_conv_desc* d, int n_layers, const float* const* x, const float* const* dpre, float* const* dw,
                                float* const* dbias, const float* const* w_for_decay, float wd_scale, void* ws, size_t ws_bytes,
                                srx_stream_t stream) {
    WgradArgs a;
    int wpl = 0, g = 0;
    int rc = wgrad_batch_plan(d, n_layers, &a, &wpl, &g);
    if (rc) return rc;
    if (!x || !dpre || !dw) return fail(SRX_ERR_BAD_ARG, "null pointer array");
    WgradBatchPtrs c;
    WgradBatchOut o;
    memset(&c, 0, sizeof(c));
    memset(&o, 0, sizeof(o));
    for (int l = 0; l < n_layers; ++l) {
        if (!x[l] || !dpre[l] || !dw[l]) return fail(SRX_ERR_BAD_ARG, "bwd_filter_batch: null tensor pointer in layer %d", l);
        float* const db = dbias ? dbias[l] : nullptr;
        const float* const wl = w_for_decay ? w_for_decay[l] : nullptr;
        if (!aligned16(x[l]) || !aligned16(dpre[l]) || !aligned16(dw[l]) || (db && !aligned16(db)) || (wl && !aligned16(wl)))
            return fail(SRX_ERR_UNSUPPORTED, "bwd_filter_batch: layer %d: every pointer must be 16-byte aligned", l);
        c.x[l] = x[l]; c.dpre[l] = dpre[l];
        o.dw[l] = dw[l]; o.dbias[l] = db; o.w[l] = wl;
    }
    const size_t need = (size_t)n_layers * wpl * part_stride(d) * sizeof(float);
    if (!ws || ws_bytes < need) return fail(SRX_ERR_WORKSPACE, "bwd_filter_batch needs %zu workspace bytes, got %zu", need, ws_bytes);
    if (!aligned16(ws)) return fail(SRX_ERR_UNSUPPORTED, "bwd_filter_batch: the workspace must be 16-byte aligned");
    a.part = (float*)ws;
    hipError_t err = launch_wgrad_rows_batch(a, c, wpl, n_layers, 2 * (size_t)(a.zero_slot + 4) * (64 + 4) * 4, (hipStream_t)stream);
    if (err != hipSuccess) return fail(SRX_ERR_LAUNCH, "wgrad batch launch failed: %s", hipGetErrorString(err));
    err = launch_wgrad_batch_reduce((const float*)ws, wpl, n_layers, a.part_stride, d->KH * d->KW * d->Cin * d->Cout, d->Cout, o, wd_scale,
                                    (hipStream_t)stream);
    if (err != hipSuccess) return fail(SRX_ERR_LAUNCH, "reduce launch failed: %s", hipGetErrorString(err));
    return SRX_OK;
}

namespace {
void blocked_desc(srx_conv_desc* d, int N, int H, int W) {
    memset(d, 0, sizeof(*d));
    d->N = N; d->H = H; d->W = W; d->Cin = 64; d->Cout = 64; d->KH = 3; d->KW = 3; d->stride = 1; d->pad_mode = SRX_PAD_SAME;
}
int pairs_route(const srx_conv_desc* d, const Plan& p, int pairs, int* G, size_t* lin_lds) {
    *lin_lds = p.lds_bytes + 4 * (size_t)(p.cinp + 4) * 4;
    const bool common = wgrad_path() >= 1 && p.cinp == 64 && p.nch == 4 && d->W >= 4 && p.RS >= 8 && *lin_lds <= 80 * 1024 &&
                        (long)d->H * d->W * 64 * 4 < (1L << 31) - 4096;
    const bool lin_ok = common && p.NTX == 1 && p.RS == d->W + p.pad_l && (long)p.TH * d->W * 64 * 4 < (1L << 30);
    const int wppp = 256 / (64 / 4);
    const bool strip_ok = common && p.NTX > 1 && p.RS >= wppp && p.TW >= 4 && (d->W % p.TW == 0 || d->W % p.TW >= 4) &&
                          p.RS <= 3 * wppp && (long)d->H * d->W * 64 * 4 < (1L << 30);
    int g = max_grid() / pairs;
    if (g < 1) g = 1;
    if (g > p.grid) g = p.grid;
    *G = g;
    if (pairs <= 1 || pairs > 65535) return 0;
    return lin_ok ? 1 : (strip_ok ? 2 : 0);
}
}

static void bf16x3_pairs_plan(int N, int H, int W, int pairs, Bf3Plan* p) {
    int g = max_grid() / pairs;
    if (g < 1) g = 1;
    bf16x3_plan(N, H, W, g, true, p);
}
static size_t bf16x3_pairs_workspace(int N, int H, int W, int pairs) {
    srx_conv_desc d;
    blocked_desc(&d, N, H, W);
    Bf3Plan one, all;
    bf16x3_plan(N, H, W, max_grid(), true, &one);
    bf16x3_pairs_plan(N, H, W, pairs, &all);
    const size_t a = (size_t)pairs * all.grid * part_stride(&d) * sizeof(float), b = (size_t)one.grid * part_stride(&d) * sizeof(float);
    return pairs > 65535 ? b : (a > b ? a : b);
}

size_t srx_conv3x3_blocked_bwd_filter_ex_workspace_bytes(int N, int H, int W, int staged_blocks, int produced_blocks, int precision) {
    if (precision == SRX_PRECISION_FP32) return srx_conv3x3_blocked_bwd_filter_workspace_bytes(N, H, W, staged_blocks, produced_blocks);
    if (precision != SRX_PRECISION_BF16X3) return 0;
    srx_conv_desc d;
    blocked_desc(&d, N, H, W);
    if (check_desc(&d) || staged_blocks <= 0 || produced_blocks <= 0) return 0;
    return bf16x3_pairs_workspace(N, H, W, staged_blocks * produced_blocks);
}

int srx_conv3x3_blocked_bwd_filter_ex(const float* x, const float* dpre, float* dw, float* dbias, int N, int H, int W,
                                      int staged_blocks, int produced_blocks, int precision, void* ws, size_t ws_bytes,
                                      srx_stream_t stream) {
    if (precision != SRX_PRECISION_FP32 && precision != SRX_PRECISION_BF16X3)
        return fail(SRX_ERR_BAD_ARG, "bad precision %d: 0 (exact fp32) or 1 (bf16x3)", precision);
    if (precision == SRX_PRECISION_FP32)
        return srx_conv3x3_blocked_bwd_filter(x, dpre, dw, dbias, N, H, W, staged_blocks, produced_blocks, ws, ws_bytes, stream);
    if (!x || !dpre || !dw) return fail(SRX_ERR_BAD_ARG, "null tensor pointer");
    if (staged_blocks <= 0 || produced_blocks <= 0) return fail(SRX_ERR_BAD_ARG, "non-positive block count");
    srx_conv_desc d;
    blocked_desc(&d, N, H, W);
    d.precision = SRX_PRECISION_BF16X3;
    int rc = check_desc(&d);
    if (rc) return rc;
    if ((rc = bf16x3_supported(&d, SRX_OP_BWD_FILTER)) != SRX_OK) return rc;
    if (!launch_wgrad3x3c64_bf16x3_pairs) return fail(SRX_ERR_UNSUPPORTED, "precision 1 (bf16x3): this build has no bf16x3 kernels");
    if (!aligned16(x) || !aligned16(dpre) || !aligned16(dw) || !aligned16(ws) || !aligned16(dbias))
        return fail(SRX_ERR_ALIGN, "tensor base pointers must be 16-byte aligned");
    const int pairs = staged_blocks * produced_blocks;
    const size_t need = bf16x3_pairs_workspace(N, H, W, pairs);
    if (!ws || ws_bytes < need) return fail(SRX_ERR_WORKSPACE, "blocked bwd_filter needs %zu workspace bytes, got %zu", need, ws_bytes);
    const size_t blk = (size_t)N * H * W * 64, wn = (size_t)9 * 64 * 64;
    if (pairs > 65535) {
        for (int ib = 0; ib < staged_blocks; ++ib)
            for (int ob = 0; ob < produced_blocks; ++ob) {
                rc = srx_conv2d_bwd_filter(&d, x + ib * blk, dpre + ob * blk, dw + ((size_t)ib * produced_blocks + ob) * wn,
                                           (ib == 0 && dbias) ? dbias + ob * 64 : nullptr, nullptr, 0.f, ws, ws_bytes, stream);
                if (rc) return rc;
            }
        return SRX_OK;
    }
    Bf3Plan bp;
    bf16x3_pairs_plan(N, H, W, pairs, &bp);
    const int stride = (int)part_stride(&d);
    hipError_t err = launch_wgrad3x3c64_bf16x3_pairs(x, dpre, (float*)ws, stride, staged_blocks, produced_blocks, N, H, W, bp,
                                                     (hipStream_t)stream);
    if (err != hipSuccess) return fail(SRX_ERR_LAUNCH, "blocked wgrad launch failed: %s", hipGetErrorString(err));
    err = launch_reduce_partials_pairs((const float*)ws, bp.grid, stride, (int)wn, 64, dw, dbias, pairs, produced_blocks,
                                       (hipStream_t)stream);
    if (err != hipSuccess) return fail(SRX_ERR_LAUNCH, "blocked reduce launch failed: %s", hipGetErrorString(err));
    return SRX_OK;
}

size_t srx_conv3x3_blocked_bwd_filter_workspace_bytes(int N, int H, int W, int staged_blocks, int produced_blocks) {
    srx_conv_desc d;
    blocked_desc(&d, N, H, W);
    if (check_desc(&d) || staged_blocks <= 0 || produced_blocks <= 0) return 0;
    Plan p;
    if (make_plan(N, H, W, H, W, 64, 64, 3, 3, 1, 1, &p)) return 0;
    wgrad_tile_for_linear_walk(&d, &p);
    int G;
    size_t lin_lds;
    const int pairs = staged_blocks * produced_blocks;
    const size_t one = (size_t)p.grid * part_stride(&d) * sizeof(float);
    if (!pairs_route(&d, p, pairs, &G, &lin_lds)) return one;
    const size_t all = (size_t)pairs * G * part_stride(&d) * sizeof(float);
    return all > one ? all : one;
}

int srx_conv3x3_blocked_bwd_filter(const float* x, const float* dpre, float* dw, float* dbias, int N, int H, int W,
                                   int staged_blocks, int produced_blocks, void* ws, size_t ws_bytes, srx_stream_t stream) {
    if (!x || !dpre || !dw) return fail(SRX_ERR_BAD_ARG, "null tensor pointer");
    if (staged_blocks <= 0 || produced_blocks <= 0) return fail(SRX_ERR_BAD_ARG, "non-positive block count");
    srx_conv_desc d;
    blocked_desc(&d, N, H, W);
    int rc = check_desc(&d);
    if (rc) return rc;
    if (!aligned16(x) || !aligned16(dpre) || !aligned16(dw) || !aligned16(ws))
        return fail(SRX_ERR_ALIGN, "tensor base pointers must be 16-byte aligned");
    const size_t need = srx_conv3x3_blocked_bwd_filter_workspace_bytes(N, H, W, staged_blocks, produced_blocks);
    if (!ws || ws_bytes < need) return fail(SRX_ERR_WORKSPACE, "blocked bwd_filter needs %zu workspace bytes, got %zu", need, ws_bytes);
    Plan p;
    rc = make_plan(N, H, W, H, W, 64, 64, 3, 3, 1, 1, &p);
    if (rc) return rc;
    wgrad_tile_for_linear_walk(&d, &p);
    const int pairs = staged_blocks * produced_blocks;
    const size_t blk = (size_t)N * H * W * 64, wn = (size_t)9 * 64 * 64;
    int G;
    size_t lin_lds;
    const int route = pairs_route(&d, p, pairs, &G, &lin_lds);
    if (!route) {
        for (int ib = 0; ib < staged_blocks; ++ib)
            for (int ob = 0; ob < produced_blocks; ++ob) {
                rc = srx_conv2d_bwd_filter(&d, x + ib * blk, dpre + ob * blk, dw + ((size_t)ib * produced_blocks + ob) * wn,
                                           (ib == 0 && dbias) ? dbias + ob * 64 : nullptr, nullptr, 0.f, ws, ws_bytes, stream);
                if (rc) return rc;
            }
        return SRX_OK;
    }
    WgradPairs q;
    memset(&q, 0, sizeof(q));
    WgradArgs& a = q.a;
    a.x = x; a.dpre = dpre;
    a.part = (float*)ws;
    a.part_stride = (int)part_stride(&d);
    a.N = N; a.H = H; a.W = W; a.OH = H; a.OW = W; a.Cin = 64; a.Cout = 64;
    a.pad_t = 1; a.pad_l = 1; a.TH = p.TH; a.TW = p.TW; a.NTX = p.NTX; a.RS = p.RS;
    a.units_total = p.units_total; a.inv_rs = 1.0f / (float)p.RS;
    a.stagger = 0;
    a.stride = 1;
    a.zero_slot = (p.TH + 2) * p.RS + 2;
    a.trace = nullptr;
    q.x_pair_stride = (long)blk; q.d_pair_stride = (long)blk;
    q.part_pair_stride = (long)G * a.part_stride;
    q.cob = produced_blocks;
// ... 490 lines not shown
```

### ml_super_resolution_amd/csrc/wgrad_batch.hip

```cpp
#include "launchers.h"
namespace srx {

__global__ __launch_bounds__(256) void wgrad_batch_reduce_kernel(const float* __restrict__ part, const int wpl, const int stride,
                                                                 const int wn, const int n, const WgradBatchOut o, const float wd) {
    const int layer = blockIdx.y;
    const int j = (blockIdx.x * 256 + threadIdx.x) * 4;
    if (j >= n) return;
    const float* p = part + (size_t)layer * wpl * stride + j;
    f32x4 s = {0.f, 0.f, 0.f, 0.f};
    int g = 0;
    for (; g + 8 <= wpl; g += 8) {
        f32x4 v[8];
#pragma unroll
        for (int i = 0; i < 8; ++i) v[i] = *reinterpret_cast<const f32x4*>(p + (size_t)(g + i) * stride);
#pragma unroll
        for (int i = 0; i < 8; ++i) s += v[i];
    }
    for (; g < wpl; ++g) s += *reinterpret_cast<const f32x4*>(p + (size_t)g * stride);
    float* __restrict__ dw = o.dw[layer];
    float* __restrict__ dbias = o.dbias[layer];
    const float* __restrict__ w = o.w[layer];
#pragma unroll
    for (int e = 0; e < 4; ++e) {
        const int jj = j + e;
        if (jj < wn)
            dw[jj] = s[e] + (w ? wd * w[jj] : 0.f);
        else if (jj < n && dbias)
            dbias[jj - wn] = s[e];
    }
}

hipError_t launch_wgrad_rows_batch(const WgradArgs& a, const WgradBatchPtrs& c, int wpl, int layers, size_t lds, hipStream_t s) {
    static thread_local bool configured = false;
    const void* fn = reinterpret_cast<const void*>(wgrad_rows_batch_kernel<3, 3, 64, 4, 41>);
    if (!configured) {
        hipError_t e = hipFuncSetAttribute(fn, hipFuncAttributeMaxDynamicSharedMemorySize, 160 * 1024);
        if (e != hipSuccess) return e;
        configured = true;
    }
    hipLaunchKernelGGL((wgrad_rows_batch_kernel<3, 3, 64, 4, 41>), dim3((unsigned)(wpl * layers)), dim3(256), lds, s, a, c, wpl);
    return hipGetLastError();
}

hipError_t launch_wgrad_batch_reduce(const float* part, int wpl, int layers, int stride, int wn, int cout, const WgradBatchOut& o,
                                     float wd, hipStream_t s) {
    const int n = wn + cout;
    hipLaunchKernelGGL(wgrad_batch_reduce_kernel, dim3((unsigned)((n + 1023) / 1024), (unsigned)layers), dim3(256), 0, s, part, wpl,
                       stride, wn, n, o, wd);
    return hipGetLastError();
}
}
```

### ml_super_resolution_amd/engine.py

```python
import contextlib
import gc
import math
import os

import torch

from . import ops


@contextlib.contextmanager
def capture_graph(g):
    gc.collect()
    was_enabled = gc.isenabled()
    gc.disable()
    try:
        with torch.cuda.graph(g):
            yield
    finally:
        if was_enabled:
            gc.enable()


class LayerSpec(object):

    def __init__(self, ksize, cin, cout, padding='same', act=None, scope=None):
        self.kh, self.kw = (ksize, ksize) if isinstance(ksize, int) else ksize
        self.cin, self.cout = cin, cout
        self.padding = padding.lower()
        self.act = act
        self.scope = scope

    @property
    def kernel_shape(self):
        return (self.kh, self.kw, self.cin, self.cout)

    def out_hw(self, h, w):
        if self.padding == 'same':
            return h, w
        return h - self.kh + 1, w - self.kw + 1


def _align4(n):
    return (n + 3) // 4 * 4


class ConvStack(object):
    def __init__(self, specs, device='cuda', residual=False, weight_decay=0.0, precision='highest'):
        self.specs = list(specs)
        self.device = torch.device(device)
        self.residual = residual
        self.weight_decay = float(weight_decay)
        self.slices = []
        off = 0
        for s in self.specs:
            kn = s.kh * s.kw * s.cin * s.cout
            k_off = off
            off = _align4(off + kn)
            b_off = off
            off = _align4(off + s.cout)
            self.slices.append((k_off, kn, b_off, s.cout))
        self.flat_size = off
        self.num_params = sum(kn + bn for _, kn, _, bn in self.slices)
        z = lambda: torch.zeros(self.flat_size, dtype=torch.float32, device=self.device)
        self.params, self.grads = z(), z()
        self.opt_m, self.opt_v = None, None
        self.global_step = 0
        self.loss = torch.zeros(1, dtype=torch.float32, device=self.device)
        self._acts = None
        self.step_graph_max_pixels = None
        self.forward_keep_hook = None
        self._bufs = {}
        self._ws = None
        self.grad_hook = None
        self.loss_kind = 'mse'
        self._decay_mask = None
        self.kernel_name, self.bias_name = 'kernel', 'bias'
        self.use_step_graph = os.environ.get('SRX_STEP_GRAPH', '1') != '0'
        self._adam_state = None
        self._state_t, self._state_lr = None, None
        self._step_graphs = {}
        self.set_precision(precision)

    def set_precision(self, precision):
        if precision not in ('highest', 'high'):
            raise ValueError("precision must be 'highest' or 'high', got %r" % (precision,))
        self.precision = precision
        choice = []
        last = len(self.specs) - 1
        for i, s in enumerate(self.specs):
            ok = precision == 'high' and not (self.residual and i == last)
            if ok:
                x_shape = (1, 1, 1, s.cin)
                ok = all(ops.precision_supported(x_shape, s.kernel_shape, op, s.padding, s.act if op == ops._lib.OP_FWD else None,
                                                 precision='high')[0]
                         for op in (ops._lib.OP_FWD, ops._lib.OP_BWD_DATA, ops._lib.OP_BWD_FILTER))
            choice.append('high' if ok else 'highest')
        self.layer_precision = choice
        self._step_graphs.clear()

    def kernel(self, i, buf=None):
        k_off, kn, _, _ = self.slices[i]
        return (self.params if buf is None else buf)[k_off:k_off + kn].view(self.specs[i].kernel_shape)

    def bias(self, i, buf=None):
        _, _, b_off, bn = self.slices[i]
        return (self.params if buf is None else buf)[b_off:b_off + bn]

    def variables(self):
        out = {}
        for i, s in enumerate(self.specs):
            scope = s.scope or ('layer%d' % i)
            out[scope + '/' + self.kernel_name] = self.kernel(i)
            out[scope + '/' + self.bias_name] = self.bias(i)
        return out

    def load_variables(self, values):
        mine = self.variables()
        for name, val in values.items():
            key = name[:-2] if name.endswith(':0') else name
            if key not in mine:
                raise KeyError('unknown variable %r' % name)
            t = torch.as_tensor(val, dtype=torch.float32)
            if tuple(t.shape) != tuple(mine[key].shape):
                raise ValueError('%s: shape %s != %s' % (name, tuple(t.shape), tuple(mine[key].shape)))
            mine[key].copy_(t.to(self.device))

    def set_params(self, pairs):
        for i, (k, b) in enumerate(pairs):
            self.kernel(i).copy_(torch.as_tensor(k, dtype=torch.float32).to(self.device))
            self.bias(i).copy_(torch.as_tensor(b, dtype=torch.float32).to(self.device))

    def _buf(self, key, shape):
        t = self._bufs.get(key)
        if t is None or tuple(t.shape) != tuple(shape):
            if t is not None:
                self._step_graphs.clear()
            t = torch.empty(shape, dtype=torch.float32, device=self.device)
            self._bufs[key] = t
        return t

    def _shapes(self, x_shape):
        n, h, w, _ = x_shape
        shapes = []
        for s in self.specs:
            h, w = s.out_hw(h, w)
            shapes.append((n, h, w, s.cout))
        return shapes

    def forward(self, x, keep=True):
        shapes = self._shapes(x.shape)
        if keep and self.forward_keep_hook is not None:
            outs = [self._buf(('act', i), shapes[i]) for i in range(len(self.specs))]
            if self.forward_keep_hook(x, outs):
                self._acts = self.acts = [x] + outs
                return outs[-1]
        acts = [x]
        t = x
        last = len(self.specs) - 1

        def out_buf(i):
            if keep:
                return self._buf(('act', i), shapes[i])
            return self._buf(('tmp', i & 1, self.specs[i].cout), shapes[i])

        i = 0
        while i <= last:
            s = self.specs[i]
            j = self._chain_end(i, [x.shape] + shapes, ops._lib.OP_FWD)
            if j > i + 1:
                outs = [out_buf(k) for k in range(i, j)]
                xs = [t] + outs[:-1]
                t = ops.conv2d_fwd_chain(xs, [self.kernel(k) for k in range(i, j)], [self.bias(k) for k in range(i, j)], outs,
                                         s.padding, s.act)
                acts.extend(outs)
                i = j
                continue
            skip = x if (self.residual and i == last) else None
            t = ops.conv2d_fwd(t, self.kernel(i), self.bias(i), s.padding, s.act, skip=skip, out=out_buf(i),
                               precision=self.layer_precision[i])
            acts.append(t)
            i += 1
        self._acts = acts if keep else None
        self.acts = acts
        return t

    def _chain_ok(self, i, in_shape, op):
        s = self.specs[i]
        if self.layer_precision[i] != 'highest' or s.kh != 3 or s.kw != 3 or s.cin != 64 or s.cout != 64 or s.act not in (None, 'relu'):
            return False
        if op == ops._lib.OP_FWD:
            if self.residual and i == len(self.specs) - 1:
                return False
            return ops.chain_supported(in_shape, s.kernel_shape, op, s.padding, s.act)
        if i == 0 or self.specs[i - 1].act not in (None, 'relu'):
            return False
        return ops.chain_supported(in_shape, s.kernel_shape, op, s.padding, in_act=self.specs[i - 1].act)

    def _chain_end(self, i, in_shapes, op):
        s = self.specs[i]
        j = i
        while (j < len(self.specs) and j - i < 32 and self.specs[j].padding == s.padding and self.specs[j].act == s.act and
               tuple(in_shapes[j]) == tuple(in_shapes[i]) and self._chain_ok(j, in_shapes[j], op)):
            j += 1
        return j

    def _dgrad_chain(self, acts):
        last = len(self.specs) - 1
        for hi in range(last - 1, 0, -1):
            s = self.specs[hi]
            lo = hi
            while (lo >= 1 and hi - lo < 32 and self.specs[lo].padding == s.padding and self.specs[lo - 1].act == self.specs[hi - 1].act and
                   tuple(acts[lo].shape) == tuple(acts[hi].shape) and self._chain_ok(lo, acts[lo].shape, ops._lib.OP_BWD_DATA)):
                lo -= 1
            if hi - lo >= 2:
                return lo + 1, hi
        return None

    def _wgrad_batch(self, acts):
        best = None
        i, n = 0, len(self.specs)
        while i < n:
            s = self.specs[i]
            j = i
            while (j < n and j - i < 32 and self.layer_precision[j] == 'highest' and self.specs[j].kernel_shape == s.kernel_shape and
                   self.specs[j].padding == s.padding and tuple(acts[j].shape) == tuple(acts[i].shape) and
                   tuple(acts[j + 1].shape) == tuple(acts[i + 1].shape)):
                j += 1
            if j - i >= 2 and (best is None or j - i > best[1] - best[0] + 1):
                if ops.bwd_filter_batch_plan(acts[i].shape, s.kernel_shape, j - i, s.padding)[0] > 0:
                    best = (i, j - 1)
            i = max(j, i + 1)
        return best

    def loss_and_backward(self, target, numel_global=None):
        if self._acts is None:
            raise RuntimeError('forward(keep=True) must run before loss_and_backward')
        acts = self._acts
        y = acts[-1]
        last = len(self.specs) - 1
        inv = 1.0 / (y.numel() if numel_global is None else numel_global)
        if self.loss_kind == 'rownorm':
            row_len = y.shape[1] * y.shape[2]
            dy = ops.rownorm_loss_fwd_bwd(y, target, row_len, self.loss, dpred=self._buf(('dy', 0), y.shape),
                                          norms=self._buf(('rownorms',), (y.numel() // row_len,)))
        else:
            dy = self._buf(('dy', 0), y.shape)
            ops.mse_fwd_bwd(y, target, self.loss, inv_numel=inv, accumulate=False, dpred=dy)
        if self.weight_decay:
            self.add_regulariser_loss()
        if self.specs[last].act is not None:
            dpre = ops.act_bwd(dy, y, self.specs[last].act, out=self._buf(('dpre_last',), y.shape))
        else:
            dpre = dy
        prec = self.layer_precision
        need = max(ops.bwd_filter_workspace_bytes(acts[i].shape, s.kernel_shape, s.padding, precision=prec[i])
                   for i, s in enumerate(self.specs))
        batch = self._wgrad_batch(acts)
        if batch is not None:
            b_lo, b_hi = batch
            need = max(need, ops.bwd_filter_batch_workspace_bytes(acts[b_lo].shape, self.specs[b_lo].kernel_shape, b_hi - b_lo + 1,
                                                                  self.specs[b_lo].padding))
        if self._ws is None or self._ws.numel() * 4 < need:
            self._step_graphs.clear()
            self._ws = torch.empty((need + 3) // 4, dtype=torch.float32, device=self.device)
        chain = self._dgrad_chain(acts)
        in_batch = lambda k: batch is not None and batch[0] <= k <= batch[1]
        dpres = {}

        def wgrad(i, dpre_i):
            s = self.specs[i]
            if not in_batch(i):
                ops.conv2d_bwd_filter(acts[i], dpre_i, s.kernel_shape, s.padding,
                                      w_for_decay=self.kernel(i) if self.weight_decay else None,
                                      wd_scale=self.weight_decay, dw=self.kernel(i, self.grads),
                                      dbias=self.bias(i, self.grads), workspace=self._ws, precision=prec[i])
                return
            dpres[i] = dpre_i
            if i == batch[0]:
                ks = list(range(batch[0], batch[1] + 1))
                ops.conv2d_bwd_filter_batch([acts[k] for k in ks], [dpres[k] for k in ks], [self.kernel(k, self.grads) for k in ks],
                                            [self.bias(k, self.grads) for k in ks],
                                            [self.kernel(k) for k in ks] if self.weight_decay else None, self.weight_decay,
                                            s.padding, workspace=self._ws)

        for i in range(last, -1, -1):
            s = self.specs[i]
            if chain is not None and chain[0] <= i <= chain[1]:
                lo, hi = chain
                if i == hi:
                    outs = [self._buf(('dpre_chain', k - 1), acts[k].shape) for k in range(hi, lo - 1, -1)]
                    ops.conv2d_bwd_data_chain([dpre] + outs[:-1], [self.kernel(k) for k in range(hi, lo - 1, -1)],
                                              [acts[k] for k in range(hi, lo - 1, -1)], outs, acts[hi].shape, s.padding,
                                              in_act=self.specs[hi - 1].act)
                    cdpres = {hi: dpre}
                    for k in range(hi, lo - 1, -1):
                        cdpres[k - 1] = outs[hi - k]
                wgrad(i, cdpres[i])
                if i == lo:
                    dpre = cdpres[lo - 1]
                continue
            wgrad(i, dpre)
            if i > 0:
                prev_act = self.specs[i - 1].act
                out = (self._buf(('dpre_chain', i - 1), acts[i].shape) if in_batch(i - 1)
                       else self._buf(('dx', i % 3, acts[i].shape[3]), acts[i].shape))
                dpre = ops.conv2d_bwd_data(dpre, self.kernel(i), acts[i].shape, s.padding,
                                           x_in=acts[i] if prev_act is not None else None, in_act=prev_act, out=out,
                                           precision=prec[i])
        if self.grad_hook is not None:
            self.grad_hook(self.grads)
        return self.loss

    def add_regulariser_loss(self):
        if self._decay_mask is None:
            self._decay_mask = torch.zeros_like(self.params)
            for k_off, kn, _, _ in self.slices:
                self._decay_mask[k_off:k_off + kn] = 1.0
        ops.l2_loss(self.params, self.weight_decay, self.loss, accumulate=True, mask=self._decay_mask)

    def adam_step(self, lr, beta1=0.9, beta2=0.999, eps=1e-8):
        if self.opt_m is None:
            self.opt_m = torch.zeros_like(self.params)
            self.opt_v = torch.zeros_like(self.params)
        self.global_step += 1
        ops.adam_tf_step(self.params, self.grads, self.opt_m, self.opt_v, lr, self.global_step, beta1, beta2, eps)

    def _sync_adam_state(self, lr):
        if self._adam_state is None:
            self._adam_state = ops.adam_state(self.device, t=self.global_step, lr=lr)
            self._state_t, self._state_lr = self.global_step, float(lr)
        if self._state_t != self.global_step:
            ops.adam_state_set(self._adam_state, t=self.global_step)
            self._state_t = self.global_step
        if self._state_lr != float(lr):
            ops.adam_state_set(self._adam_state, lr=lr)
            self._state_lr = float(lr)

    def adam_step_dev(self, lr, beta1=0.9, beta2=0.999, eps=1e-8):
        if self.opt_m is None:
            self.opt_m = torch.zeros_like(self.params)
            self.opt_v = torch.zeros_like(self.params)
        self._sync_adam_state(lr)
        ops.adam_tf_step_dev(self.params, self.grads, self.opt_m, self.opt_v, self._adam_state, beta1, beta2, eps)
        self.global_step += 1
        self._state_t += 1

    def train_step_replay(self, x, target, lr, beta1=0.9, beta2=0.999, eps=1e-8, momentum=None, gradient_cap=0.01):
        def optimizer_launch():
            if momentum is None:
                ops.adam_tf_step_dev(self.params, self.grads, self.opt_m, self.opt_v, self._adam_state, beta1, beta2, eps)
            else:
                ops.momentum_clip_step(self.params, self.grads, self.opt_m, lr, momentum, gradient_cap / lr)

        def eager(xx, tt):
            self.forward(xx, keep=True)
            self.loss_and_backward(tt)
            if momentum is None:
                self.adam_step_dev(lr, beta1, beta2, eps)
            else:
                self.momentum_clip_step(lr, momentum, gradient_cap)
            return self.loss
        if not self.use_step_graph or self.grad_hook is not None or self.device.type != 'cuda':
            return eager(x, target)
        if self.step_graph_max_pixels is not None and x.shape[0] * x.shape[1] * x.shape[2] > self.step_graph_max_pixels:
            return eager(x, target)
        opt_key = (float(beta1), float(beta2), float(eps)) if momentum is None else ('momentum', float(lr), float(momentum), float(gradient_cap))
        key = (tuple(x.shape), tuple(target.shape)) + opt_key
        ent = self._step_graphs.get(key)
        if ent is None:
            if len(self._step_graphs) >= 4:
                self._step_graphs.clear()
            ent = self._step_graphs[key] = {'warm': 0, 'graph': None}
        if ent['graph'] is None:
            if ent['warm'] < 2:
                ent['warm'] += 1
                loss = eager(x, target)
                if key not in self._step_graphs:
                    self._step_graphs[key] = ent
                return loss
            if self.opt_m is None:
                self.opt_m = torch.zeros_like(self.params)
                if momentum is None:
                    self.opt_v = torch.zeros_like(self.params)
            if momentum is None:
                self._sync_adam_state(lr)
            sx, st = x.clone(), target.clone()
            torch.cuda.synchronize(self.device)
            g = torch.cuda.CUDAGraph()
            with capture_graph(g):
                self.forward(sx, keep=True)
                self.loss_and_backward(st)
                optimizer_launch()
            ent.update(graph=g, x=sx, t=st)
        if momentum is None:
            self._sync_adam_state(lr)
        if x.data_ptr() != ent['x'].data_ptr():
            ent['x'].copy_(x)
        if target.data_ptr() != ent['t'].data_ptr():
            ent['t'].copy_(target)
        ent['graph'].replay()
        self.global_step += 1
        if momentum is None:
            self._state_t += 1
        return self.loss

    def static_step_inputs(self, x_shape, target_shape):
        for key, ent in self._step_graphs.items():
            if ent.get('graph') is not None and key[0] == tuple(x_shape) and key[1] == tuple(target_shape):
                return ent['x'], ent['t']
        return None

    def momentum_clip_step(self, lr, momentum=0.9, gradient_cap=0.01):
        if self.opt_m is None:
            self.opt_m = torch.zeros_like(self.params)
        self.global_step += 1
        ops.momentum_clip_step(self.params, self.grads, self.opt_m, lr, momentum, gradient_cap / lr)

    def state_dict(self):
        sd = {'global_step': self.global_step, 'params': self.params.detach().cpu()}
        if self.opt_m is not None:
            sd['opt_m'] = self.opt_m.detach().cpu()
        if self.opt_v is not None:
            sd['opt_v'] = self.opt_v.detach().cpu()
        return sd

    def tf_checkpoint_tensors(self, adam_betas=(0.9, 0.999), extra=None):
        import numpy as np
        out = {k: v.detach().cpu().numpy() for k, v in self.variables().items()}
        out['global_step'] = np.asarray(self.global_step, dtype=np.int64)
        for k, v in (extra or {}).items():
            out[k] = np.asarray(v)
        if self.opt_m is not None:
            two = self.opt_v is not None
            for i, s in enumerate(self.specs):
                scope = s.scope or ('layer%d' % i)
                for kind, view in ((self.kernel_name, self.kernel), (self.bias_name, self.bias)):
                    out['%s/%s/%s' % (scope, kind, 'Adam' if two else 'Momentum')] = view(i, self.opt_m).detach().cpu().numpy()
                    if two:
                        out['%s/%s/Adam_1' % (scope, kind)] = view(i, self.opt_v).detach().cpu().numpy()
            if two:
                from . import tf_bundle
                out['beta1_power'] = tf_bundle.tf_beta_power(adam_betas[0], self.global_step)
                out['beta2_power'] = tf_bundle.tf_beta_power(adam_betas[1], self.global_step)
        return out

    def save_tf_checkpoint(self, prefix, adam_betas=(0.9, 0.999), extra=None, write_state=True):
        from . import tf_bundle
        tf_bundle.save_checkpoint(prefix, self.tf_checkpoint_tensors(adam_betas, extra))
        if write_state:
            tf_bundle.update_checkpoint_state(prefix)
# ... 76 lines not shown
```

### ml_super_resolution_amd/espcn/model_espcn.py

```python
import os

import numpy as np
import torch

from .. import graph, ops
from ..engine import ConvStack, LayerSpec, capture_graph, truncated_normal_


def layer_specs(scaling_factor=3):
    r2 = scaling_factor * scaling_factor
    return [LayerSpec(5, 3, 64, 'same', 'tanh', 'f1'),
            LayerSpec(3, 64, 32, 'same', 'tanh', 'f2'),
            LayerSpec(3, 32, 3 * r2, 'same', None, 'f3')]


class EspcnModel(object):
    def __init__(self, scaling_factor=3, device='cuda', seed=None):
        self.scaling_factor = scaling_factor
        self.stack = ConvStack(layer_specs(scaling_factor), device=device, residual=False, weight_decay=0.0)
        gen = torch.Generator().manual_seed(seed) if seed is not None else None
        for i in range(3):
            truncated_normal_(self.stack.kernel(i), 0.02, gen)
        self.placeholders = {}
        self.use_graph = os.environ.get('SRX_ESPCN_GRAPH', '1') != '0'
        self._graphs = {}
        self.use_single_launch = os.environ.get('SRX_ESPCN_FUSED', '1') != '0'
        self.single_launch_max_pixels = int(os.environ.get('SRX_ESPCN_FUSED_MAX_PIXELS', '131072'))
        self.inference_path = ('<= %d LR pixels: ONE launch, the three layers chained through LDS per <= 16x16 tile with the '
                               'sub-pixel store (srx_espcn_forward); larger: f1, f2, f3 with the sub-pixel store fused into '
                               "f3's epilogue, 3 launches%s" % (self.single_launch_max_pixels,
                                                               ' replayed as one HIP graph' if self.use_graph else ', eager'))

        self.use_single_launch_train = os.environ.get('SRX_ESPCN_FUSED_TRAIN', '1') != '0'
        self.single_launch_train_max_pixels = int(os.environ.get('SRX_ESPCN_FUSED_TRAIN_MAX_PIXELS', '30000'))
        self.stack.forward_keep_hook = self._forward_keep_one_launch
        self.stack.step_graph_max_pixels = int(os.environ.get('SRX_ESPCN_STEP_GRAPH_MAX_PIXELS', '12000'))

    def _forward_keep_one_launch(self, x, outs):
        n, h, w, _ = x.shape
        if not (self.use_single_launch and self.use_single_launch_train and x.is_cuda and n * h * w <= self.single_launch_train_max_pixels
                and 2 <= self.scaling_factor <= 4):
            return False
        st = self.stack
        ops.espcn_forward_keep(x.contiguous(), [(st.kernel(i), st.bias(i)) for i in range(3)], self.scaling_factor, outs[0], outs[1], outs[2])
        return True

    def forward(self, lr_source, keep=False):
        return self.stack.forward(lr_source, keep=keep)

    def super_resolve_two_step(self, lr_source):
        return ops.depth_to_space(self.forward(lr_source), self.scaling_factor)

    def _super_resolve_launches(self, lr_source, out=None, mids=None):
        st, r = self.stack, self.scaling_factor
        n, h, w, _ = lr_source.shape
        t1, t2 = mids if mids is not None else (st._buf(('sr', 0), (n, h, w, 64)), st._buf(('sr', 1), (n, h, w, 32)))
        t = ops.conv2d_fwd(lr_source, st.kernel(0), st.bias(0), 'same', 'tanh', out=t1)
        t = ops.conv2d_fwd(t, st.kernel(1), st.bias(1), 'same', 'tanh', out=t2)
        return ops.conv2d_fwd(t, st.kernel(2), st.bias(2), 'same', None, subpixel_r=r,
                              out=out if out is not None else st._buf(('sr', 2), (n, h * r, w * r, 3)))

    def super_resolve(self, lr_source, use_graph=None, single_launch=None):
        if single_launch is None:
            single_launch = self.use_single_launch and lr_source.shape[0] * lr_source.shape[1] * lr_source.shape[2] <= self.single_launch_max_pixels
        if single_launch and lr_source.is_cuda:
            st, r = self.stack, self.scaling_factor
            n, h, w, _ = lr_source.shape
            return ops.espcn_forward(lr_source.contiguous(), [(st.kernel(i), st.bias(i)) for i in range(3)], r,
                                     out=st._buf(('sr1',), (n, h * r, w * r, 3)))
        if not (self.use_graph if use_graph is None else use_graph) or not lr_source.is_cuda:
            return self._super_resolve_launches(lr_source)
        key = tuple(lr_source.shape)
        g = self._graphs.get(key)
        if g is None:
            g = self._graphs[key] = self._capture(lr_source)
        static_in, graph_obj, out = g[:3]
        if lr_source.data_ptr() != static_in.data_ptr():
            static_in.copy_(lr_source)
        graph_obj.replay()
        return out

    def _capture(self, lr_source):
        if len(self._graphs) >= 8:
            self._graphs.pop(next(iter(self._graphs)))
        static_in = lr_source.clone()
        n, h, w, _ = lr_source.shape
        r = self.scaling_factor
        out = torch.empty((n, h * r, w * r, 3), dtype=torch.float32, device=lr_source.device)
        mids = (torch.empty((n, h, w, 64), dtype=torch.float32, device=lr_source.device),
                torch.empty((n, h, w, 32), dtype=torch.float32, device=lr_source.device))
        side = torch.cuda.Stream(device=lr_source.device)
        side.wait_stream(torch.cuda.current_stream(lr_source.device))
        with torch.cuda.stream(side):
            for _ in range(2):
                self._super_resolve_launches(static_in, out=out, mids=mids)
        torch.cuda.current_stream(lr_source.device).wait_stream(side)
        graph_obj = torch.cuda.CUDAGraph()
        with capture_graph(graph_obj):
            self._super_resolve_launches(static_in, out=out, mids=mids)
        return static_in, graph_obj, out, mids

    def train_step(self, lr_source, hr_target, learning_rate):
        return self.stack.train_step_replay(lr_source, hr_target, learning_rate)

    def save(self, path):
        arrays = {k + ':0': v.detach().cpu().numpy() for k, v in self.stack.variables().items()}
        arrays['global_step'] = np.int64(self.stack.global_step)
        np.savez(path, **arrays)

    def run(self, keys, feed_dict):
        dev = self.stack.device
        feeds = {name: feed_dict[ph] for name, ph in self.placeholders.items() if ph in feed_dict}
        needs_forward = [k for k in keys if k != 'step']
        lr = hr = y = loss = None
        if needs_forward:
            if 'lr_source' not in feeds:
                raise ValueError('lr_source must be fed to fetch %s' % ', '.join(needs_forward))
            lr = graph.to_device(feeds['lr_source'], dev)
            hr = graph.to_device(feeds['hr_target'], dev) if 'hr_target' in feeds else None
            if 'optimizer' in keys:
                if hr is None or 'learning_rate' not in feeds:
                    raise ValueError('hr_target and learning_rate must be fed to run the optimizer')
                loss = self.train_step(lr, hr, float(feeds['learning_rate']))
                y = self.stack.acts[-1]
            else:
                y = self.stack.forward(lr, keep=True)
                if 'loss' in keys:
                    if hr is None:
                        raise ValueError('hr_target must be fed to fetch loss')
                    loss = self.stack.loss
                    ops.mse_fwd_bwd(y, hr, loss, accumulate=False, want_grad=False)
        out = {}
        for k in keys:
            if k == 'optimizer':
                out[k] = None
            elif k == 'loss':
                out[k] = float(loss.item())
            elif k == 'step':
                out[k] = self.stack.global_step
            elif k in ('sr_result', 'sr_results'):
                out[k] = y.detach().cpu().numpy()
            elif k in ('lr_source', 'lr_sources'):
                out[k] = lr.detach().cpu().numpy()
            elif k == 'hr_target':
                out[k] = hr.detach().cpu().numpy()
            else:
                raise KeyError(k)
        return out


def build_model(lr_source, scaling_factor=3, hr_target=None, device='cuda', seed=None):
    m = EspcnModel(scaling_factor, device=device, seed=seed)
    m.placeholders['lr_source'] = lr_source
    model = {'lr_source': lr_source, '_model': m}
    model['sr_result'] = graph.Tensor('sr_result', owner=m, key='sr_result')
    if hr_target is None:
        return model
    m.placeholders['hr_target'] = hr_target
    lr = graph.placeholder([], name='learning_rate')
    m.placeholders['learning_rate'] = lr
    model['hr_target'] = hr_target
    model['step'] = graph.Tensor('global_step', owner=m, key='step')
    model['loss'] = graph.Tensor('loss', owner=m, key='loss')
    model['optimizer'] = graph.Tensor('optimizer', owner=m, key='optimizer')
    model['learning_rate'] = lr
    return model


def extract_weights(meta_path, ckpt_path):
    from .. import tf_bundle
    if tf_bundle.is_checkpoint_prefix(ckpt_path):
        values = tf_bundle.load_checkpoint(ckpt_path)
        return {k + ':0': v for k, v in values.items()
                if k.count('/') == 1 and k.split('/')[1] in ('kernel', 'bias')}
    z = np.load(ckpt_path)
    return {k: z[k] for k in z.files if k.endswith(':0')}


def build_test_model(meta_path, ckpt_path, device='cuda'):
    variables = ckpt_path if isinstance(ckpt_path, dict) else extract_weights(meta_path, ckpt_path)
    scaling_factor = int((np.asarray(variables['f3/bias:0']).size // 3) ** 0.5)
    m = EspcnModel(scaling_factor, device=device)
    m.stack.load_variables(variables)
    lr_sources = graph.placeholder([None, None, None, 3], name='lr_sources')
    m.placeholders['lr_source'] = lr_sources
    return {'lr_sources': lr_sources,
            'sr_results': graph.Tensor('sr_results', owner=m, key='sr_results'),
            'scaling_factor': scaling_factor,
# ... 2 lines not shown
```

### ml_super_resolution_amd/ops.py

```python
import ctypes
import os

import numpy as np
import torch

from . import _lib
from ._lib import ACT_BY_NAME, PAD_BY_NAME, ConvDesc, check
from ._lib import lib as _load_lib

_POISON_LDS = os.environ.get('SRX_POISON_LDS', '0') == '1'


def lib():
    L = _load_lib()
    if _POISON_LDS and torch.cuda.is_available():
        L.srx_debug_poison_lds(_stream())
    return L



def _stream():
    return ctypes.c_void_p(torch.cuda.current_stream().cuda_stream)


# ... 57 lines not shown
               precision='highest'):
    for t, n in ((x, 'x'), (w, 'w'), (bias, 'bias'), (skip, 'skip')):
        _chk(t, n)
    d = conv_desc(x.shape, w.shape, padding, act, post_add_relu, subpixel_r, stride, precision)
    shape = out_shape(d)
    if subpixel_r > 1:
        r = int(subpixel_r)
        if shape[3] % (r * r):
            raise ValueError('subpixel_r %d: %d output channels are not a multiple of r*r' % (r, shape[3]))
        shape = (shape[0], shape[1] * r, shape[2] * r, shape[3] // (r * r))
    if out is not None and tuple(out.shape) != tuple(shape):
        raise ValueError('out has shape %s, expected %s' % (tuple(out.shape), tuple(shape)))
    y = out if out is not None else torch.empty(shape, dtype=torch.float32, device=x.device)
    check(lib().srx_conv2d_fwd(ctypes.byref(d), _ptr(x), _ptr(w), _ptr(bias), _ptr(skip), _ptr(y), None, 0, _stream()),
          'srx_conv2d_fwd')
    return y


def conv2d_bwd_data(dpre, w, x_shape, padding='same', x_in=None, in_act=None, out=None, precision='highest'):
    for t, n in ((dpre, 'dpre'), (w, 'w'), (x_in, 'x_in')):
        _chk(t, n)
    d = conv_desc(x_shape, w.shape, padding, precision=precision)
    dx = out if out is not None else torch.empty(tuple(x_shape), dtype=torch.float32, device=dpre.device)
    check(lib().srx_conv2d_bwd_data(ctypes.byref(d), _ptr(dpre), _ptr(w), _ptr(x_in), ACT_BY_NAME[in_act],
                                    _ptr(dx), None, 0, _stream()), 'srx_conv2d_bwd_data')
    return dx


def chain_supported(x_shape, w_shape, op=_lib.OP_FWD, padding='same', act=None, in_act=None, precision='highest'):
    d = conv_desc(x_shape, w_shape, padding, act, precision=precision)
    return lib().srx_conv_chain_supported(ctypes.byref(d), int(op), ACT_BY_NAME[in_act]) == 1


def _ptr_array(ts):
    return (ctypes.c_void_p * len(ts))(*[None if t is None else t.data_ptr() for t in ts])


def conv2d_fwd_chain(xs, ws, biases, outs, padding='same', act=None):
    for l in range(len(xs)):
        _chk(xs[l], 'x'); _chk(ws[l], 'w'); _chk(biases[l], 'bias'); _chk(outs[l], 'out')
    d = conv_desc(xs[0].shape, ws[0].shape, padding, act)
    shape = out_shape(d)
    for l in range(len(xs)):
        if tuple(xs[l].shape) != tuple(xs[0].shape) or tuple(ws[l].shape) != tuple(ws[0].shape) or tuple(outs[l].shape) != shape:
            raise ValueError('conv2d_fwd_chain: layer %d does not have the shape of layer 0' % l)
    check(lib().srx_conv_chain(ctypes.byref(d), _lib.OP_FWD, _lib.ACT_NONE, len(xs), _ptr_array(xs), _ptr_array(ws), _ptr_array(biases),
                               None, _ptr_array(outs), _stream()), 'srx_conv_chain')
    return outs[-1]


def conv2d_bwd_data_chain(dpres, ws, x_ins, outs, x_shape, padding='same', in_act=None):
    masks = x_ins if (x_ins is not None and in_act is not None) else None
    for l in range(len(dpres)):
        _chk(dpres[l], 'dpre'); _chk(ws[l], 'w'); _chk(outs[l], 'out')
        if masks is not None:
            _chk(masks[l], 'x_in')
        if tuple(outs[l].shape) != tuple(x_shape) or tuple(ws[l].shape) != tuple(ws[0].shape) or tuple(dpres[l].shape) != tuple(dpres[0].shape):
            raise ValueError('conv2d_bwd_data_chain: layer %d does not have the shape of layer 0' % l)
    d = conv_desc(x_shape, ws[0].shape, padding)
    check(lib().srx_conv_chain(ctypes.byref(d), _lib.OP_BWD_DATA, ACT_BY_NAME[in_act] if masks is not None else _lib.ACT_NONE, len(dpres),
                               _ptr_array(dpres), _ptr_array(ws), None, None if masks is None else _ptr_array(masks),
                               _ptr_array(outs), _stream()), 'srx_conv_chain')
    return outs[-1]


def set_chain(on):
    return lib().srx_set_chain(int(on))


def set_chain_fixed(on):
    return lib().srx_set_chain_fixed(int(on))


def bwd_filter_workspace_bytes(x_shape, w_shape, padding='same', stride=1, precision='highest'):
    d = conv_desc(x_shape, w_shape, padding, stride=stride, precision=precision)
    return lib().srx_conv2d_workspace_bytes(ctypes.byref(d), _lib.OP_BWD_FILTER)


def conv2d_bwd_filter(x, dpre, w_shape, padding='same', w_for_decay=None, wd_scale=0.0, dw=None, dbias=None,
                      want_dbias=True, workspace=None, stride=1, precision='highest'):
    for t, n in ((x, 'x'), (dpre, 'dpre'), (w_for_decay, 'w_for_decay')):
        _chk(t, n)
    d = conv_desc(x.shape, w_shape, padding, stride=stride, precision=precision)
    if tuple(dpre.shape) != tuple(out_shape(d)):
        raise ValueError('dpre has shape %s, the layer output is %s' % (tuple(dpre.shape), tuple(out_shape(d))))
    if dw is None:
        dw = torch.empty(tuple(w_shape), dtype=torch.float32, device=x.device)
    if dbias is None and want_dbias:
        dbias = torch.empty((w_shape[3],), dtype=torch.float32, device=x.device)
    need = lib().srx_conv2d_workspace_bytes(ctypes.byref(d), _lib.OP_BWD_FILTER)
    if workspace is None:
        workspace = torch.empty((need + 3) // 4, dtype=torch.float32, device=x.device)
    check(lib().srx_conv2d_bwd_filter(ctypes.byref(d), _ptr(x), _ptr(dpre), _ptr(dw), _ptr(dbias),
                                      _ptr(w_for_decay), float(wd_scale), _ptr(workspace),
                                      workspace.numel() * 4, _stream()), 'srx_conv2d_bwd_filter')
    return dw, dbias


def conv2d_bwd_filter_partials(x, dpre, w_shape, padding, workspace, precision='highest'):
    _chk(x, 'x'); _chk(dpre, 'dpre'); _chk(workspace, 'workspace')
    d = conv_desc(x.shape, w_shape, padding, precision=precision)
    n = ctypes.c_int(0)
    check(lib().srx_conv2d_bwd_filter_partials(ctypes.byref(d), _ptr(x), _ptr(dpre), _ptr(workspace), workspace.numel() * 4,
                                               ctypes.byref(n), _stream()), 'srx_conv2d_bwd_filter_partials')
    return n.value


def conv2d_bwd_filter_reduce(x_shape, w_shape, padding, workspace, n_partials, dw, dbias=None, w_for_decay=None, wd_scale=0.0,
                             precision='highest'):
    _chk(workspace, 'workspace'); _chk(dw, 'dw')
    d = conv_desc(x_shape, w_shape, padding, precision=precision)
    check(lib().srx_conv2d_bwd_filter_reduce(ctypes.byref(d), _ptr(workspace), int(n_partials), _ptr(dw), _ptr(dbias),
                                             _ptr(w_for_decay), float(wd_scale), _stream()), 'srx_conv2d_bwd_filter_reduce')
    return dw, dbias


def bwd_filter_batch_plan(x_shape, w_shape, n_layers, padding='same', stride=1, precision='highest'):
    d = conv_desc(x_shape, w_shape, padding, stride=stride, precision=precision)
    wpl, grid = ctypes.c_int(0), ctypes.c_int(0)
    _load_lib().srx_conv2d_bwd_filter_batch_plan(ctypes.byref(d), int(n_layers), ctypes.byref(wpl), ctypes.byref(grid))
    return wpl.value, grid.value


def bwd_filter_batch_workspace_bytes(x_shape, w_shape, n_layers, padding='same', stride=1, precision='highest'):
    d = conv_desc(x_shape, w_shape, padding, stride=stride, precision=precision)
    return _load_lib().srx_conv2d_bwd_filter_batch_workspace_bytes(ctypes.byref(d), int(n_layers))


def conv2d_bwd_filter_batch(xs, dpres, dws, dbiases=None, w_for_decay=None, wd_scale=0.0, padding='same', workspace=None,
                            stride=1, precision='highest'):
    L = len(xs)
    if not (len(dpres) == len(dws) == L) or (dbiases is not None and len(dbiases) != L) or (w_for_decay is not None and len(w_for_decay) != L):
        raise ValueError('conv2d_bwd_filter_batch: the per-layer lists differ in length')
    for l in range(L):
        _chk(xs[l], 'x'); _chk(dpres[l], 'dpre'); _chk(dws[l], 'dw')
        _chk(None if dbiases is None else dbiases[l], 'dbias'); _chk(None if w_for_decay is None else w_for_decay[l], 'w_for_decay')
    d = conv_desc(xs[0].shape, dws[0].shape, padding, stride=stride, precision=precision)
    for l in range(L):
        if tuple(xs[l].shape) != tuple(xs[0].shape) or tuple(dpres[l].shape) != tuple(out_shape(d)) or tuple(dws[l].shape) != tuple(dws[0].shape):
            raise ValueError('conv2d_bwd_filter_batch: layer %d does not have the shape of layer 0' % l)
    if workspace is None:
        need = _load_lib().srx_conv2d_bwd_filter_batch_workspace_bytes(ctypes.byref(d), L)
        workspace = torch.empty((max(need, 16) + 3) // 4, dtype=torch.float32, device=xs[0].device)
    _chk(workspace, 'workspace')
    check(lib().srx_conv2d_bwd_filter_batch(ctypes.byref(d), L, _ptr_array(xs), _ptr_array(dpres), _ptr_array(dws),
                                            None if dbiases is None else _ptr_array(dbiases),
                                            None if w_for_decay is None else _ptr_array(w_for_decay), float(wd_scale),
                                            _ptr(workspace), workspace.numel() * 4, _stream()), 'srx_conv2d_bwd_filter_batch')
    return dws, dbiases


def set_wgrad_batch(on):
    return lib().srx_set_wgrad_batch(int(on))


def act_bwd(dy, y, act, out=None):
    _chk(dy, 'dy'); _chk(y, 'y')
    out = out if out is not None else torch.empty_like(dy)
    check(lib().srx_act_bwd(_ptr(dy), _ptr(y), _ptr(out), dy.numel(), ACT_BY_NAME[act], _stream()), 'srx_act_bwd')
    return out


def depth_to_space(x, r, out=None):
    _chk(x, 'x')
    N, H, W, D = x.shape
    if D % (r * r):
        raise ValueError('depth %d not divisible by r*r=%d' % (D, r * r))
    C = D // (r * r)
    out = out if out is not None else torch.empty((N, H * r, W * r, C), dtype=torch.float32, device=x.device)
    check(lib().srx_depth_to_space(_ptr(x), _ptr(out), N, H, W, C, r, _stream()), 'srx_depth_to_space')
    return out


def espcn_forward(x, params, r, out=None):
    _chk(x, 'x')
    for k, b in params:
        _chk(k, 'kernel'); _chk(b, 'bias')
    (w1, b1), (w2, b2), (w3, b3) = params
    N, H, W, C = x.shape
    if C != 3 or tuple(w1.shape) != (5, 5, 3, 64) or tuple(w2.shape) != (3, 3, 64, 32) or tuple(w3.shape) != (3, 3, 32, 3 * r * r):
        raise ValueError('espcn_forward: shapes do not describe ESPCN 5-3-3 with scaling factor %d' % r)
    out = out if out is not None else torch.empty((N, H * r, W * r, 3), dtype=torch.float32, device=x.device)
    check(lib().srx_espcn_forward(_ptr(x), _ptr(w1), _ptr(b1), _ptr(w2), _ptr(b2), _ptr(w3), _ptr(b3), _ptr(out),
                                  N, H, W, int(r), _stream()), 'srx_espcn_forward')
    return out


def espcn_forward_keep(x, params, r, t1, t2, y):
    _chk(x, 'x')
    for k, b in params:
        _chk(k, 'kernel'); _chk(b, 'bias')
    (w1, b1), (w2, b2), (w3, b3) = params
    N, H, W, C = x.shape
    if C != 3 or tuple(w1.shape) != (5, 5, 3, 64) or tuple(w2.shape) != (3, 3, 64, 32) or tuple(w3.shape) != (3, 3, 32, 3 * r * r):
        raise ValueError('espcn_forward_keep: shapes do not describe ESPCN 5-3-3 with scaling factor %d' % r)
    for t, c, name in ((t1, 64, 't1'), (t2, 32, 't2'), (y, 3 * r * r, 'y')):
        _chk(t, name)
        if tuple(t.shape) != (N, H, W, c):
            raise ValueError('espcn_forward_keep: %s has shape %s, expected %s' % (name, tuple(t.shape), (N, H, W, c)))
    check(lib().srx_espcn_forward_keep(_ptr(x), _ptr(w1), _ptr(b1), _ptr(w2), _ptr(b2), _ptr(w3), _ptr(b3), _ptr(t1), _ptr(t2),
                                       _ptr(y), N, H, W, int(r), _stream()), 'srx_espcn_forward_keep')
    return y


def srcnn_forward(x, params, out=None):
    _chk(x, 'x')
    for k, b in params:
        _chk(k, 'kernel'); _chk(b, 'bias')
    (w1, b1), (w2, b2), (w3, b3) = params
    N, H, W, C = x.shape
    if C != 3 or tuple(w1.shape) != (9, 9, 3, 64) or tuple(w2.shape) != (1, 1, 64, 32) or tuple(w3.shape) != (5, 5, 32, 3):
        raise ValueError('srcnn_forward: shapes do not describe SRCNN 9-1-5')
    if H < 13 or W < 13:
        raise ValueError('srcnn_forward: image %dx%d smaller than the 13-pixel receptive field' % (H, W))
    out = out if out is not None else torch.empty((N, H - 12, W - 12, 3), dtype=torch.float32, device=x.device)
    check(lib().srx_srcnn_forward(_ptr(x), _ptr(w1), _ptr(b1), _ptr(w2), _ptr(b2), _ptr(w3), _ptr(b3), _ptr(out),
                                  N, H, W, _stream()), 'srx_srcnn_forward')
    return out


def space_to_depth(x, r, out=None):
    _chk(x, 'x')
    N, HR, WR, C = x.shape
    if HR % r or WR % r:
        raise ValueError('spatial dims %dx%d not divisible by r=%d' % (HR, WR, r))
    H, W = HR // r, WR // r
    out = out if out is not None else torch.empty((N, H, W, C * r * r), dtype=torch.float32, device=x.device)
    check(lib().srx_space_to_depth(_ptr(x), _ptr(out), N, H, W, C, r, _stream()), 'srx_space_to_depth')
    return out


def stream_copy(src, dst):
    _chk(src, 'src'); _chk(dst, 'dst')
    if src.numel() != dst.numel():
        raise ValueError('stream_copy: sizes differ')
    check(lib().srx_stream_copy(_ptr(src), _ptr(dst), src.numel() * 4, _stream()), 'srx_stream_copy')
    return dst


def mse_fwd_bwd(pred, target, loss_out, inv_numel=None, accumulate=False, dpred=None, want_grad=True):
    _chk(pred, 'pred'); _chk(target, 'target')
    if inv_numel is None:
        inv_numel = 1.0 / pred.numel()
    if dpred is None and want_grad:
        dpred = torch.empty_like(pred)
    check(lib().srx_mse_fwd_bwd(_ptr(pred), _ptr(target), pred.numel(), float(inv_numel), _ptr(loss_out),
                                int(accumulate), _ptr(dpred), _ptr(reduce_scratch(pred.device)), _stream()),
          'srx_mse_fwd_bwd')
    return dpred


def l2_loss(w, scale, loss_out, accumulate=True, mask=None):
    _chk(w, 'w'); _chk(mask, 'mask')
    check(lib().srx_l2_loss(_ptr(w), _ptr(mask), w.numel(), float(scale), _ptr(loss_out), int(accumulate),
                            _ptr(reduce_scratch(w.device)), _stream()), 'srx_l2_loss')


def adam_tf_step(w, g, m, v, lr, t, beta1=0.9, beta2=0.999, eps=1e-8, grad_scale=1.0):
    for tns, n in ((w, 'w'), (g, 'g'), (m, 'm'), (v, 'v')):
        _chk(tns, n)
    check(lib().srx_adam_tf_step(_ptr(w), _ptr(g), _ptr(m), _ptr(v), w.numel(), float(lr), float(beta1),
                                 float(beta2), float(eps), int(t), float(grad_scale), _stream()), 'srx_adam_tf_step')


def adam_state(device, t=0, lr=0.0):
    st = torch.zeros(8, dtype=torch.int32, device=device)
    adam_state_set(st, t=t, lr=lr)
    return st


def adam_state_set(st, t=None, lr=None):
    if t is not None:
        st[0:2].copy_(torch.tensor([int(t)], dtype=torch.int64).view(torch.int32))
    if lr is not None:
        st[2:3].copy_(torch.tensor([float(lr)], dtype=torch.float32).view(torch.int32))


def adam_state_get(st):
    h = st.cpu()
    return int(h[0:2].view(torch.int64).item()), float(h[2:3].view(torch.float32).item()), float(h[3:4].view(torch.float32).item())


def adam_tf_step_dev(w, g, m, v, state, beta1=0.9, beta2=0.999, eps=1e-8, grad_scale=1.0):
    for tns, n in ((w, 'w'), (g, 'g'), (m, 'm'), (v, 'v')):
        _chk(tns, n)
    check(lib().srx_adam_tf_step_dev(_ptr(w), _ptr(g), _ptr(m), _ptr(v), w.numel(), _ptr(state), float(beta1), float(beta2),
                                     float(eps), float(grad_scale), _stream()), 'srx_adam_tf_step_dev')


def momentum_clip_step(w, g, acc, lr, momentum=0.9, cap=float('inf'), grad_scale=1.0):
    for tns, n in ((w, 'w'), (g, 'g'), (acc, 'acc')):
        _chk(tns, n)
    cap = min(float(cap), 3.0e38)
    check(lib().srx_momentum_clip_step(_ptr(w), _ptr(g), _ptr(acc), w.numel(), float(lr), float(momentum), cap,
                                       float(grad_scale), _stream()), 'srx_momentum_clip_step')


def rownorm_loss_fwd_bwd(pred, target, row_len, loss_out, want_grad=True, dpred=None, norms=None):
    _chk(pred, 'pred'); _chk(target, 'target'); _chk(dpred, 'dpred'); _chk(norms, 'norms')
    rows = pred.numel() // row_len
    if rows * row_len != pred.numel():
        raise ValueError('numel %d not divisible by row_len %d' % (pred.numel(), row_len))
    if norms is None:
        norms = torch.empty(rows, dtype=torch.float32, device=pred.device)
    if dpred is None and want_grad:
        dpred = torch.empty_like(pred)
# ... 712 lines not shown
```

Baseline: 20010 patches/s.

## Fold first-layer narrow wgrad into the batched 64x64 wgrad launch as side blocks

Adds a side job to the batched row-wise weight-gradient kernel. Extra workgroups in the same launch compute the narrow 3->64 first-layer wgrad, so that layer's gradient no longer needs its own kernel launch and idle CUs are used. The narrow wgrad body is moved into a shared header so both kernels can call it, and the engine routes layer batch[0]-1 through the new API when the planner finds spare slots. This adds a workspace, plan logic and scheduling complexity, and puts extra register/LDS pressure on the combined kernel.

Measured after the change: 20120 patches/s, median of 6. Within noise of the previous version (+0.6%).

```diff
diff --git a/include/srx.h b/include/srx.h
--- a/include/srx.h
+++ b/include/srx.h
@@ -89,6 +89,16 @@
 size_t srx_conv2d_bwd_filter_batch_workspace_bytes(const srx_conv_desc* d, int n_layers);
 int srx_conv2d_bwd_filter_batch_plan(const srx_conv_desc* d, int n_layers, int* wgs_per_layer, int* grid);
 int srx_set_wgrad_batch(int on);
+
+int srx_conv2d_bwd_filter_batch_side(const srx_conv_desc* d, int n_layers, const float* const* x, const float* const* dpre,
+                                     float* const* dw, float* const* dbias, const float* const* w_for_decay, float wd_scale,
+                                     void* ws, size_t ws_bytes, const srx_conv_desc* side, const float* side_x,
+                                     const float* side_dpre, float* side_dw, float* side_dbias, const float* side_w_for_decay,
+                                     void* side_ws, size_t side_ws_bytes, int* n_side, srx_stream_t stream);
+int srx_conv2d_bwd_filter_batch_side_plan(const srx_conv_desc* d, int n_layers, const srx_conv_desc* side, int* n_side,
+                                          int* side_partials);
+size_t srx_conv2d_bwd_filter_batch_side_workspace_bytes(const srx_conv_desc* d, int n_layers, const srx_conv_desc* side);
+int srx_set_wgrad_side(int on);
 
 int srx_act_bwd(const float* dy, const float* y, float* dpre, size_t numel, int act,
                 srx_stream_t stream);
diff --git a/ml_super_resolution_amd/_lib.py b/ml_super_resolution_amd/_lib.py
--- a/ml_super_resolution_amd/_lib.py
+++ b/ml_super_resolution_amd/_lib.py
@@ -18,7 +18,8 @@
 EXPORTS = [
     'srx_version', 'srx_last_error', 'srx_set_conv_path', 'srx_set_wgrad_path', 'srx_set_chain', 'srx_set_chain_fixed', 'srx_conv_chain', 'srx_conv_chain_supported', 'srx_conv2d_precision_supported', 'srx_conv2d_workspace_bytes', 'srx_conv2d_fwd',
     'srx_conv2d_bwd_data', 'srx_conv2d_bwd_filter', 'srx_conv2d_bwd_filter_partials', 'srx_conv2d_bwd_filter_reduce',
-    'srx_conv2d_bwd_filter_batch', 'srx_conv2d_bwd_filter_batch_workspace_bytes', 'srx_conv2d_bwd_filter_batch_plan', 'srx_set_wgrad_batch', 'srx_act_bwd', 'srx_depth_to_space',
+    'srx_conv2d_bwd_filter_batch', 'srx_conv2d_bwd_filter_batch_workspace_bytes', 'srx_conv2d_bwd_filter_batch_plan', 'srx_set_wgrad_batch',
+    'srx_conv2d_bwd_filter_batch_side', 'srx_conv2d_bwd_filter_batch_side_plan', 'srx_conv2d_bwd_filter_batch_side_workspace_bytes', 'srx_set_wgrad_side', 'srx_act_bwd', 'srx_depth_to_space',
     'srx_space_to_depth', 'srx_stream_copy', 'srx_mse_fwd_bwd', 'srx_l2_loss', 'srx_reduce_scratch_bytes',
     'srx_adam_tf_step', 'srx_adam_tf_step_dev', 'srx_momentum_clip_step', 'srx_rownorm_loss_fwd_bwd', 'srx_psnr', 'srx_ssim', 'srx_ssim_scratch_bytes', 'srx_saturate_u8', 'srx_affine', 'srx_u8_to_unit_float', 'srx_gaussian_blur', 'srx_resize_bilinear',
     'srx_upsample_nearest', 'srx_upsample_nearest_bwd', 'srx_add_relu_grad',
@@ -120,6 +121,11 @@
     L.srx_conv2d_bwd_filter_batch_workspace_bytes.restype = sz
     L.srx_conv2d_bwd_filter_batch_plan.argtypes = [dp, i, ctypes.POINTER(ctypes.c_int), ctypes.POINTER(ctypes.c_int)]
     L.srx_set_wgrad_batch.argtypes = [i]
+    L.srx_conv2d_bwd_filter_batch_side.argtypes = [dp, i, vp, vp, vp, vp, vp, f, vp, sz, dp, vp, vp, vp, vp, vp, vp, sz, ctypes.POINTER(ctypes.c_int), vp]
+    L.srx_conv2d_bwd_filter_batch_side_plan.argtypes = [dp, i, dp, ctypes.POINTER(ctypes.c_int), ctypes.POINTER(ctypes.c_int)]
+    L.srx_conv2d_bwd_filter_batch_side_workspace_bytes.argtypes = [dp, i, dp]
+    L.srx_conv2d_bwd_filter_batch_side_workspace_bytes.restype = sz
+    L.srx_set_wgrad_side.argtypes = [i]
     L.srx_act_bwd.argtypes = [vp, vp, vp, sz, i, vp]
     L.srx_depth_to_space.argtypes = [vp, vp, i, i, i, i, i, vp]
     L.srx_space_to_depth.argtypes = [vp, vp, i, i, i, i, i, vp]
diff --git a/ml_super_resolution_amd/csrc/conv_kernels.hip.h b/ml_super_resolution_amd/csrc/conv_kernels.hip.h
--- a/ml_super_resolution_amd/csrc/conv_kernels.hip.h
+++ b/ml_super_resolution_amd/csrc/conv_kernels.hip.h
@@ -2803,13 +2803,13 @@
     const float* w[kChainMax];
 };
 
-template <int KH, int KW, int CINP, int NCH, int OWC>
-__global__ __launch_bounds__(256, 1) void wgrad_rows_batch_kernel(const WgradArgs a, const WgradBatchPtrs c, const int wpl) {
-    const int layer = __builtin_amdgcn_readfirstlane((int)blockIdx.x / wpl);
-    const int sub = (int)blockIdx.x - layer * wpl;
-    const int u0 = (int)(((long)sub * a.units_total) / wpl);
-    const int u1 = (int)(((long)(sub + 1) * a.units_total) / wpl);
-    wgrad_rows_full_body<KH, KW, CINP, NCH, OWC>(a, c.x[layer], c.dpre[layer], a.part + (size_t)blockIdx.x * a.part_stride, u0, u1);
-}
-
-}
+struct WgradSideJob {
+    WgradArgs a;
+    long total_px;
+    int iters;
+    int n_blocks;
+    int n_side;
+    int nout;
+};
+
+}
diff --git a/ml_super_resolution_amd/csrc/conv_narrow.hip b/ml_super_resolution_amd/csrc/conv_narrow.hip
--- a/ml_super_resolution_amd/csrc/conv_narrow.hip
+++ b/ml_super_resolution_amd/csrc/conv_narrow.hip
@@ -1,46 +1,12 @@
 #include "launchers.h"
+#include "wgrad_narrow_body.hip.h"
 namespace srx {
-typedef float f32x3 __attribute__((ext_vector_type(3)));
 typedef unsigned u32x3v __attribute__((ext_vector_type(3)));
 
 template <int CTRL>
 __device__ __forceinline__ float dpp_add(float v) {
     const int moved = __builtin_amdgcn_update_dpp(0, __float_as_int(v), CTRL, 0xf, 0xf, false);
     return v + __int_as_float(moved);
-}
-
-struct PixWalk {
-    int n, oh, ow;
-    __device__ __forceinline__ void init(unsigned p, int OH, int OW) {
-        const unsigned t = p / (unsigned)OW;
-        ow = (int)(p - t * (unsigned)OW);
-        n = (int)(t / (unsigned)OH);
-        oh = (int)(t - (unsigned)n * (unsigned)OH);
-    }
-    __device__ __forceinline__ void step16(int OH, int OW) { step(16, OH, OW); }
-    __device__ __forceinline__ void step(int d, int OH, int OW) {
-        ow += d;
-        while (ow >= OW) {
-            ow -= OW;
-            oh += 1;
-            if (oh == OH) { oh = 0; n += 1; }
-        }
-    }
-};
-template <int KH, int KW>
-__device__ __forceinline__ void tap_offsets(int (&off)[KH * KW], const PixWalk& q, bool live, int H, int W, int pad_t, int pad_l,
-                                            int PB, int lane_b) {
-    const int centre = ((q.n * H + q.oh - pad_t) * W + (q.ow - pad_l)) * PB + lane_b;
-    bool rok[KH], cok[KW];
-#pragma unroll
-    for (int kh = 0; kh < KH; ++kh) rok[kh] = live && (unsigned)(q.oh + kh - pad_t) < (unsigned)H;
-#pragma unroll
-    for (int kw = 0; kw < KW; ++kw) cok[kw] = (unsigned)(q.ow + kw - pad_l) < (unsigned)W;
-#pragma unroll
-    for (int kh = 0; kh < KH; ++kh)
-#pragma unroll
-        for (int kw = 0; kw < KW; ++kw)
-            off[kh * KW + kw] = (rok[kh] && cok[kw]) ? centre + (kh * W + kw) * PB : kOobOffset;
 }
 
 template <int KH, int KW, int CIN, int CO>
@@ -104,97 +70,11 @@
 
 template <int KH, int KW, bool NOUT, int CW = 64>
 __global__ __launch_bounds__(256) void wgrad_narrow_kernel(const WgradArgs a, long total_px, int iters) {
-    constexpr int TAPS = KH * KW, CN = 3;
-    constexpr int LPP = CW / 4;
-    constexpr int PPI = 256 / LPP;
-    constexpr int NB = NOUT ? CN : 4;
-    constexpr int NV = TAPS * 4 * CN + NB;
-    __shared__ float red[4 * NV * LPP];
-    const int c4 = threadIdx.x & (LPP - 1);
-    const int sub = threadIdx.x / LPP;
-    const int wave = threadIdx.x >> 6;
-    float acc[NV];
-#pragma unroll
-    for (int i = 0; i < NV; ++i) acc[i] = 0.0f;
-    const __amdgpu_buffer_rsrc_t xrs = __builtin_amdgcn_make_buffer_rsrc(
-        const_cast<float*>(a.x), 0, a.N * a.H * a.W * (NOUT ? CW : CN) * 4, 0x00020000);
-    const __amdgpu_buffer_rsrc_t drs = __builtin_amdgcn_make_buffer_rsrc(
-        const_cast<float*>(a.dpre), 0, a.N * a.OH * a.OW * (NOUT ? CN : CW) * 4, 0x00020000);
-    const unsigned p0 = blockIdx.x * (unsigned)iters * (unsigned)PPI + sub;
-    PixWalk q;
-    q.init(p0 < (unsigned)total_px ? p0 : 0u, a.OH, a.OW);
-    for (int it = 0; it < iters; ++it, q.step(PPI, a.OH, a.OW)) {
-        const unsigned p = p0 + (unsigned)it * (unsigned)PPI;
-        const bool live = p < (unsigned)total_px;
-        int off[TAPS];
-        tap_offsets<KH, KW>(off, q, live, a.H, a.W, a.pad_t, a.pad_l, (NOUT ? CW : CN) * 4, NOUT ? 16 * c4 : 0);
-        if constexpr (NOUT) {
-            const f32x3 d = __builtin_bit_cast(f32x3, __builtin_amdgcn_raw_buffer_load_b96(drs, live ? (int)(p * CN * 4) : kOobOffset, 0, 0));
-            f32x4 v[TAPS];
-#pragma unroll
-            for (int tp = 0; tp < TAPS; ++tp)
-                v[tp] = __builtin_bit_cast(f32x4, __builtin_amdgcn_raw_buffer_load_b128(xrs, off[tp], 0, 0));
-#pragma unroll
-            for (int tp = 0; tp < TAPS; ++tp)
-#pragma unroll
-                for (int e = 0; e < 4; ++e)
-#pragma unroll
-                    for (int c = 0; c < CN; ++c) acc[(tp * 4 + e) * CN + c] = fmaf(v[tp][e], d[c], acc[(tp * 4 + e) * CN + c]);
-#pragma unroll
-            for (int c = 0; c < CN; ++c) acc[TAPS * 4 * CN + c] += d[c];
-        } else {
-            const f32x4 d = __builtin_bit_cast(f32x4, __builtin_amdgcn_raw_buffer_load_b128(
-                drs, live ? (int)((p * CW + 4 * c4) * 4) : kOobOffset, 0, 0));
-            f32x3 v[TAPS];
-#pragma unroll
-            for (int tp = 0; tp < TAPS; ++tp)
-                v[tp] = __builtin_bit_cast(f32x3, __builtin_amdgcn_raw_buffer_load_b96(xrs, off[tp], 0, 0));
-#pragma unroll
-            for (int tp = 0; tp < TAPS; ++tp)
-#pragma unroll
-                for (int cn = 0; cn < CN; ++cn)
-#pragma unroll
-                    for (int e = 0; e < 4; ++e) acc[(tp * CN + cn) * 4 + e] = fmaf(v[tp][cn], d[e], acc[(tp * CN + cn) * 4 + e]);
-#pragma unroll
-            for (int e = 0; e < 4; ++e) acc[TAPS * 4 * CN + e] += d[e];
-        }
-    }
-#pragma unroll
-    for (int i = 0; i < NV; ++i) {
-        float r = acc[i];
-#pragma unroll
-        for (int o = LPP; o < 64; o <<= 1) r += __shfl_xor(r, o);
-        if (sub % (64 / LPP) == 0) red[(wave * NV + i) * LPP + c4] = r;
-    }
-    __syncthreads();
-    float* part = a.part + (size_t)blockIdx.x * a.part_stride;
-    const int wn = TAPS * CW * CN;
-    for (int q = threadIdx.x; q < NV * LPP; q += 256) {
-        const int i = q / LPP, l = q % LPP;
-        const float r = (red[(0 * NV + i) * LPP + l] + red[(1 * NV + i) * LPP + l]) +
-                        (red[(2 * NV + i) * LPP + l] + red[(3 * NV + i) * LPP + l]);
-        if (i < TAPS * 4 * CN) {
-            int idx;
-            if constexpr (NOUT) {
-                const int c = i % CN, te = i / CN, e = te & 3, tp = te >> 2;
-                idx = (tp * CW + 4 * l + e) * CN + c;
-            } else {
-                const int e = i & 3, tc = i >> 2;
-                idx = tc * CW + 4 * l + e;
-            }
-            part[idx] = r;
-        } else {
-            const int b = i - TAPS * 4 * CN;
-            if constexpr (NOUT) {
-                if (l == 0) part[wn + b] = r;
-            } else {
-                part[wn + 4 * l + b] = r;
-            }
-        }
-    }
+    __shared__ float red[WgradNarrowGeo<KH, KW, NOUT, CW>::RED_FLOATS];
+    wgrad_narrow_body<KH, KW, NOUT, CW, 1>(a, total_px, iters, (int)blockIdx.x, a.part + (size_t)blockIdx.x * a.part_stride, red);
 }
 
-bool launch_wgrad_narrow(const ConvKey& k, const WgradArgs& a, int grid, hipStream_t s, hipError_t* err) {
+bool wgrad_narrow_split(const ConvKey& k, const WgradArgs& a, int grid, long* total_px, int* iters_out, int* kind) {
     if (k.kh != 3 || k.kw != 3) return false;
     const bool nout = a.Cin == 64 && a.Cout == 3, nin = a.Cin == 3 && a.Cout == 64, nin32 = a.Cin == 3 && a.Cout == 32;
     if (!nout && !nin && !nin32) return false;
@@ -202,7 +82,17 @@
     if (total >= (1L << 31) - 4096 || (long)a.N * a.H * a.W * 64 * 4 >= (1L << 31) - 4096 || total * 64 * 4 >= (1L << 31) - 4096)
         return false;
     const long ppi = nin32 ? 32 : 16;
-    const int iters = (int)((total + ppi * grid - 1) / (ppi * grid));
+    *total_px = total;
+    *iters_out = (int)((total + ppi * grid - 1) / (ppi * grid));
+    *kind = nout ? 0 : (nin ? 1 : 2);
+    return true;
+}
+
+bool launch_wgrad_narrow(const ConvKey& k, const WgradArgs& a, int grid, hipStream_t s, hipError_t* err) {
+    long total = 0;
+    int iters = 0, kind = 0;
+    if (!wgrad_narrow_split(k, a, grid, &total, &iters, &kind)) return false;
+    const bool nout = kind == 0, nin = kind == 1;
     if (nout)
         hipLaunchKernelGGL((wgrad_narrow_kernel<3, 3, true>), dim3(grid), dim3(256), 0, s, a, total, iters);
     else if (nin)
diff --git a/ml_super_resolution_amd/csrc/launchers.h b/ml_super_resolution_amd/csrc/launchers.h
--- a/ml_super_resolution_amd/csrc/launchers.h
+++ b/ml_super_resolution_amd/csrc/launchers.h
@@ -15,6 +15,7 @@
 bool launch_pipe_k3c64(const ConvKey& k, const ConvArgs& a, int grid, size_t lds, hipStream_t s, hipError_t* err);
 bool launch_pipe_other(const ConvKey& k, const ConvArgs& a, int grid, size_t lds, hipStream_t s, hipError_t* err);
 bool launch_wgrad_narrow(const ConvKey& k, const WgradArgs& a, int grid, hipStream_t s, hipError_t* err);
+__attribute__((weak)) bool wgrad_narrow_split(const ConvKey& k, const WgradArgs& a, int grid, long* total_px, int* iters, int* kind);
 bool launch_conv_narrow(const ConvKey& k, const ConvArgs& a, hipStream_t s, hipError_t* err);
 bool launch_conv_1x1(const ConvKey& k, const ConvArgs& a, long min_pixels, hipStream_t s, hipError_t* err);
 bool launch_conv_rows3x3(const ConvKey& k, const ConvArgs& a, long min_pixels, hipStream_t s, hipError_t* err);
@@ -36,7 +37,8 @@
 
 __attribute__((weak)) hipError_t launch_conv_chain(bool wt, bool aux, bool fixed, const ConvArgs& a, const ChainPtrs& c, int grid, size_t lds, hipStream_t s);
 
-__attribute__((weak)) hipError_t launch_wgrad_rows_batch(const WgradArgs& a, const WgradBatchPtrs& c, int wpl, int layers, size_t lds, hipStream_t s);
+__attribute__((weak)) hipError_t launch_wgrad_rows_batch(const WgradArgs& a, const WgradBatchPtrs& c, int wpl, int layers, const WgradSideJob& side,
+                                                         size_t lds, hipStream_t s);
 __attribute__((weak)) hipError_t launch_wgrad_batch_reduce(const float* part, int wpl, int layers, int stride, int wn, int cout,
                                                            const WgradBatchOut& o, float wd, hipStream_t s);
 
diff --git a/ml_super_resolution_amd/csrc/srx_api.hip b/ml_super_resolution_amd/csrc/srx_api.hip
--- a/ml_super_resolution_amd/csrc/srx_api.hip
+++ b/ml_super_resolution_amd/csrc/srx_api.hip
@@ -20,7 +20,7 @@
 
 struct Knobs {
     int pipe_default, narrow, wgrad_lin, wgrad_pipe, wgrad_pipe_strip, wgrad_rows_full, wgrad_1x1, wgrad_pack3, kwrows_min_pixels, big_route_min_pixels, strip_d2s, conv_1x1_min_pixels, pack3_dgrad;
-    int chain, chain_fixed, wgrad_batch;
+    int chain, chain_fixed, wgrad_batch, wgrad_side;
     unsigned long long* trace;
     int dbg;
 };
@@ -42,6 +42,7 @@
     k.wgrad_pack3 = env_int("SRX_WGRAD_PACK3", 1);
     k.chain = env_int("SRX_CHAIN", 1);
     k.chain_fixed = env_int("SRX_CHAIN_FIXED", 1);
+    k.wgrad_side = env_int("SRX_WGRAD_SIDE", 1);
     k.wgrad_batch = env_int("SRX_WGRAD_BATCH", 1);
     k.trace = nullptr;
     k.dbg = 0;
@@ -60,6 +61,8 @@
 int use_chain_fixed() { const int v = g_chain_fixed.load(std::memory_order_relaxed); return v < 0 ? (knobs().chain_fixed ? 1 : 0) : v; }
 std::atomic<int> g_wgrad_batch{-1};
 int use_wgrad_batch() { const int v = g_wgrad_batch.load(std::memory_order_relaxed); return v < 0 ? (knobs().wgrad_batch ? 1 : 0) : v; }
+std::atomic<int> g_wgrad_side{-1};
+int use_wgrad_side() { const int v = g_wgrad_side.load(std::memory_order_relaxed); return v < 0 ? (knobs().wgrad_side ? 1 : 0) : v; }
 int use_pipe() { const int v = g_use_pipe.load(std::memory_order_relaxed); return v < 0 ? knobs().pipe_default : v; }
 std::atomic<int> g_wgrad_path{-1};
 int wgrad_path_default() { return !knobs().wgrad_lin ? 0 : ((knobs().wgrad_pipe || knobs().wgrad_pipe_strip) ? 2 : 1); }
@@ -818,14 +821,91 @@
     return (size_t)n_layers * wpl * part_stride(d) * sizeof(float);
 }
 
-int srx_conv2d_bwd_filter_batch(const srx_conv_desc* d, int n_layers, const float* const* x, const float* const* dpre, float* const* dw,
-                                float* const* dbias, const float* const* w_for_decay, float wd_scale, void* ws, size_t ws_bytes,
-                                srx_stream_t stream) {
+namespace {
+constexpr int kSideCap = 8;
+
+int wgrad_side_plan(const srx_conv_desc* sd, int spare, WgradSideJob* job) {
+    int rc = check_desc(sd);
+    if (rc) return rc;
+    memset(job, 0, sizeof(*job));
+    const bool narrow = sd->KH == 3 && sd->KW == 3 && sd->stride == 1 && ((sd->Cin == 64 && sd->Cout == 3) || (sd->Cin == 3 && sd->Cout == 64));
+    if (!narrow || sd->precision != SRX_PRECISION_FP32 || !knobs().narrow || !wgrad_narrow_split)
+        return fail(SRX_ERR_UNSUPPORTED, "bwd_filter_batch_side: the side layer is not on wgrad_narrow_kernel's route (3x3 stride-1 64<->3, exact fp32)");
+    int pt, pl, OH, OW;
+    geometry(sd, &pt, &pl, &OH, &OW);
+    Plan p;
+    rc = make_plan(sd->N, sd->H, sd->W, OH, OW, sd->Cin, sd->Cout, sd->KH, sd->KW, pt, pl, &p);
+    if (rc) return rc;
+    wgrad_tile_for_linear_walk(sd, &p);
+    WgradArgs& a = job->a;
+    a.part_stride = (int)part_stride(sd);
+    a.N = sd->N; a.H = sd->H; a.W = sd->W; a.OH = OH; a.OW = OW; a.Cin = sd->Cin; a.Cout = sd->Cout;
+    a.pad_t = pt; a.pad_l = pl; a.stride = 1;
+    ConvKey k{sd->KH, sd->KW, p.cinp, p.nch, false};
+    int kind = 0;
+    if (!wgrad_narrow_split(k, a, p.grid, &job->total_px, &job->iters, &kind) || kind > 1)
+        return fail(SRX_ERR_UNSUPPORTED, "bwd_filter_batch_side: the side layer is too large for wgrad_narrow_kernel");
+    job->n_blocks = p.grid;
+    job->nout = kind == 0;
+    int n = use_wgrad_side() ? spare : 0;
+    if (n > kSideCap) n = kSideCap;
+    if (n > p.grid) n = p.grid;
+    job->n_side = n < 0 ? 0 : n;
+    return SRX_OK;
+}
+}
+
+int srx_set_wgrad_side(int on) {
+    const int old = g_wgrad_side.exchange(on < 0 ? -1 : (on ? 1 : 0), std::memory_order_relaxed);
+    return old < 0 ? (knobs().wgrad_side ? 1 : 0) : old;
+}
+
+int srx_conv2d_bwd_filter_batch_side_plan(const srx_conv_desc* d, int n_layers, const srx_conv_desc* side, int* n_side, int* side_partials) {
+    WgradArgs a;
+    WgradSideJob job;
+    int wpl = 0, g = 0;
+    if (n_side) *n_side = 0;
+    if (side_partials) *side_partials = 0;
+    int rc = wgrad_batch_plan(d, n_layers, &a, &wpl, &g);
+    if (rc) return rc;
+    if (!side) return fail(SRX_ERR_BAD_ARG, "null descriptor");
+    if ((rc = wgrad_side_plan(side, g - n_layers * wpl, &job)) != SRX_OK) return rc;
+    if (n_side) *n_side = job.n_side;
+    if (side_partials) *side_partials = job.n_side ? job.n_blocks : 0;
+    return SRX_OK;
+}
+
+size_t srx_conv2d_bwd_filter_batch_side_workspace_bytes(const srx_conv_desc* d, int n_layers, const srx_conv_desc* side) {
+    int n = 0, parts = 0;
+    if (srx_conv2d_bwd_filter_batch_side_plan(d, n_layers, side, &n, &parts) != SRX_OK) return 0;
+    return (size_t)parts * part_stride(side) * sizeof(float);
+}
+
+int srx_conv2d_bwd_filter_batch_side(const srx_conv_desc* d, int n_layers, const float* const* x, const float* const* dpre, float* const* dw,
+                                     float* const* dbias, const float* const* w_for_decay, float wd_scale, void* ws, size_t ws_bytes,
+                                     const srx_conv_desc* side, const float* side_x, const float* side_dpre, float* side_dw, float* side_dbias,
+                                     const float* side_w_for_decay, void* side_ws, size_t side_ws_bytes, int* n_side, srx_stream_t stream) {
     WgradArgs a;
     int wpl = 0, g = 0;
+    if (n_side) *n_side = 0;
     int rc = wgrad_batch_plan(d, n_layers, &a, &wpl, &g);
     if (rc) return rc;
     if (!x || !dpre || !dw) return fail(SRX_ERR_BAD_ARG, "null pointer array");
+    WgradSideJob job;
+    memset(&job, 0, sizeof(job));
+    if (side) {
+        if ((rc = wgrad_side_plan(side, g - n_layers * wpl, &job)) != SRX_OK) return rc;
+        if (job.n_side) {
+            if (!side_x || !side_dpre || !side_dw) return fail(SRX_ERR_BAD_ARG, "bwd_filter_batch_side: null tensor pointer of the side layer");
+            if (!aligned16(side_x) || !aligned16(side_dpre))
+                return fail(SRX_ERR_UNSUPPORTED, "bwd_filter_batch_side: the side layer's tensors must be 16-byte aligned");
+            const size_t sneed = (size_t)job.n_blocks * part_stride(side) * sizeof(float);
+            if (!side_ws || side_ws_bytes < sneed)
+                return fail(SRX_ERR_WORKSPACE, "bwd_filter_batch_side needs %zu side workspace bytes, got %zu", sneed, side_ws_bytes);
+            if (!aligned16(side_ws)) return fail(SRX_ERR_UNSUPPORTED, "bwd_filter_batch_side: the side workspace must be 16-byte aligned");
+            job.a.x = side_x; job.a.dpre = side_dpre; job.a.part = (float*)side_ws;
+        }
+    }
     WgradBatchPtrs c;
     WgradBatchOut o;
     memset(&c, 0, sizeof(c));
@@ -843,12 +923,25 @@
     if (!ws || ws_bytes < need) return fail(SRX_ERR_WORKSPACE, "bwd_filter_batch needs %zu workspace bytes, got %zu", need, ws_bytes);
     if (!aligned16(ws)) return fail(SRX_ERR_UNSUPPORTED, "bwd_filter_batch: the workspace must be 16-byte aligned");
     a.part = (float*)ws;
-    hipError_t err = launch_wgrad_rows_batch(a, c, wpl, n_layers, 2 * (size_t)(a.zero_slot + 4) * (64 + 4) * 4, (hipStream_t)stream);
+    hipError_t err = launch_wgrad_rows_batch(a, c, wpl, n_layers, job, 2 * (size_t)(a.zero_slot + 4) * (64 + 4) * 4, (hipStream_t)stream);
     if (err != hipSuccess) return fail(SRX_ERR_LAUNCH, "wgrad batch launch failed: %s", hipGetErrorString(err));
     err = launch_wgrad_batch_reduce((const float*)ws, wpl, n_layers, a.part_stride, d->KH * d->KW * d->Cin * d->Cout, d->Cout, o, wd_scale,
                                     (hipStream_t)stream);
     if (err != hipSuccess) return fail(SRX_ERR_LAUNCH, "reduce launch failed: %s", hipGetErrorString(err));
-    return SRX_OK;
+    if (job.n_side) {
+        err = launch_reduce_partials((const float*)side_ws, job.n_blocks, job.a.part_stride, side->KH * side->KW * side->Cin * side->Cout, side->Cout,
+                                     side_dw, side_dbias, side_w_for_decay, wd_scale, (hipStream_t)stream);
+        if (err != hipSuccess) return fail(SRX_ERR_LAUNCH, "reduce launch failed: %s", hipGetErrorString(err));
+        if (n_side) *n_side = job.n_side;
+    }
+    return SRX_OK;
+}
+
+int srx_conv2d_bwd_filter_batch(const srx_conv_desc* d, int n_layers, const float* const* x, const float* const* dpre, float* const* dw,
+                                float* const* dbias, const float* const* w_for_decay, float wd_scale, void* ws, size_t ws_bytes,
+                                srx_stream_t stream) {
+    return srx_conv2d_bwd_filter_batch_side(d, n_layers, x, dpre, dw, dbias, w_for_decay, wd_scale, ws, ws_bytes, nullptr, nullptr, nullptr, nullptr,
+                                            nullptr, nullptr, nullptr, 0, nullptr, stream);
 }
 
 namespace {
diff --git a/ml_super_resolution_amd/csrc/wgrad_batch.hip b/ml_super_resolution_amd/csrc/wgrad_batch.hip
--- a/ml_super_resolution_amd/csrc/wgrad_batch.hip
+++ b/ml_super_resolution_amd/csrc/wgrad_batch.hip
@@ -1,5 +1,32 @@
 #include "launchers.h"
+#include "wgrad_narrow_body.hip.h"
 namespace srx {
+
+constexpr int kSideDepth = 4;
+
+template <int KH, int KW, int CINP, int NCH, int OWC>
+__global__ __launch_bounds__(256, 1) void wgrad_rows_batch_kernel(const WgradArgs a, const WgradBatchPtrs c, const int wpl, const WgradSideJob side) {
+    const int n_body = (int)gridDim.x - side.n_side;
+    if ((int)blockIdx.x >= n_body) {
+        extern __shared__ __attribute__((aligned(16))) float lds[];
+        const int j = (int)blockIdx.x - n_body;
+        const int b0 = (int)(((long)j * side.n_blocks) / side.n_side), b1 = (int)(((long)(j + 1) * side.n_blocks) / side.n_side);
+        for (int b = b0; b < b1; ++b) {
+            float* part = side.a.part + (size_t)b * side.a.part_stride;
+            if (side.nout)
+                wgrad_narrow_body<3, 3, true, 64, kSideDepth>(side.a, side.total_px, side.iters, b, part, lds);
+            else
+                wgrad_narrow_body<3, 3, false, 64, kSideDepth>(side.a, side.total_px, side.iters, b, part, lds);
+            __syncthreads();
+        }
+        return;
+    }
+    const int layer = __builtin_amdgcn_readfirstlane((int)blockIdx.x / wpl);
+    const int sub = (int)blockIdx.x - layer * wpl;
+    const int u0 = (int)(((long)sub * a.units_total) / wpl);
+    const int u1 = (int)(((long)(sub + 1) * a.units_total) / wpl);
+    wgrad_rows_full_body<KH, KW, CINP, NCH, OWC>(a, c.x[layer], c.dpre[layer], a.part + (size_t)blockIdx.x * a.part_stride, u0, u1);
+}
 
 __global__ __launch_bounds__(256) void wgrad_batch_reduce_kernel(const float* __restrict__ part, const int wpl, const int stride,
                                                                  const int wn, const int n, const WgradBatchOut o, const float wd) {
@@ -30,7 +57,8 @@
     }
 }
 
-hipError_t launch_wgrad_rows_batch(const WgradArgs& a, const WgradBatchPtrs& c, int wpl, int layers, size_t lds, hipStream_t s) {
+hipError_t launch_wgrad_rows_batch(const WgradArgs& a, const WgradBatchPtrs& c, int wpl, int layers, const WgradSideJob& side, size_t lds,
+                                   hipStream_t s) {
     static thread_local bool configured = false;
     const void* fn = reinterpret_cast<const void*>(wgrad_rows_batch_kernel<3, 3, 64, 4, 41>);
     if (!configured) {
@@ -38,7 +66,8 @@
         if (e != hipSuccess) return e;
         configured = true;
     }
-    hipLaunchKernelGGL((wgrad_rows_batch_kernel<3, 3, 64, 4, 41>), dim3((unsigned)(wpl * layers)), dim3(256), lds, s, a, c, wpl);
+    hipLaunchKernelGGL((wgrad_rows_batch_kernel<3, 3, 64, 4, 41>), dim3((unsigned)(wpl * layers + side.n_side)), dim3(256), lds, s, a, c,
+                       wpl, side);
     return hipGetLastError();
 }
 
diff --git a/ml_super_resolution_amd/csrc/wgrad_narrow_body.hip.h b/ml_super_resolution_amd/csrc/wgrad_narrow_body.hip.h
--- /dev/null
+++ b/ml_super_resolution_amd/csrc/wgrad_narrow_body.hip.h
@@ -0,0 +1,148 @@
+#pragma once
+#include "conv_kernels.hip.h"
+namespace srx {
+typedef float f32x3 __attribute__((ext_vector_type(3)));
+
+struct PixWalk {
+    int n, oh, ow;
+    __device__ __forceinline__ void init(unsigned p, int OH, int OW) {
+        const unsigned t = p / (unsigned)OW;
+        ow = (int)(p - t * (unsigned)OW);
+        n = (int)(t / (unsigned)OH);
+        oh = (int)(t - (unsigned)n * (unsigned)OH);
+    }
+    __device__ __forceinline__ void step16(int OH, int OW) { step(16, OH, OW); }
+    __device__ __forceinline__ void step(int d, int OH, int OW) {
+        ow += d;
+        while (ow >= OW) {
+            ow -= OW;
+            oh += 1;
+            if (oh == OH) { oh = 0; n += 1; }
+        }
+    }
+};
+template <int KH, int KW>
+__device__ __forceinline__ void tap_offsets(int (&off)[KH * KW], const PixWalk& q, bool live, int H, int W, int pad_t, int pad_l,
+                                            int PB, int lane_b) {
+    const int centre = ((q.n * H + q.oh - pad_t) * W + (q.ow - pad_l)) * PB + lane_b;
+    bool rok[KH], cok[KW];
+#pragma unroll
+    for (int kh = 0; kh < KH; ++kh) rok[kh] = live && (unsigned)(q.oh + kh - pad_t) < (unsigned)H;
+#pragma unroll
+    for (int kw = 0; kw < KW; ++kw) cok[kw] = (unsigned)(q.ow + kw - pad_l) < (unsigned)W;
+#pragma unroll
+    for (int kh = 0; kh < KH; ++kh)
+#pragma unroll
+        for (int kw = 0; kw < KW; ++kw)
+            off[kh * KW + kw] = (rok[kh] && cok[kw]) ? centre + (kh * W + kw) * PB : kOobOffset;
+}
+
+template <int KH, int KW, bool NOUT, int CW>
+struct WgradNarrowGeo {
+    static constexpr int TAPS = KH * KW, CN = 3;
+    static constexpr int LPP = CW / 4;
+    static constexpr int PPI = 256 / LPP;
+    static constexpr int NB = NOUT ? CN : 4;
+    static constexpr int NV = TAPS * 4 * CN + NB;
+    static constexpr int RED_FLOATS = 4 * NV * LPP;
+};
+
+template <int KH, int KW, bool NOUT, int CW, int DEPTH>
+__device__ __forceinline__ void wgrad_narrow_body(const WgradArgs& a, const long total_px, const int iters, const int blk,
+                                                  float* __restrict__ part, float* red) {
+    typedef WgradNarrowGeo<KH, KW, NOUT, CW> G;
+    constexpr int TAPS = G::TAPS, CN = G::CN, LPP = G::LPP, PPI = G::PPI, NV = G::NV;
+    typedef __attribute__((ext_vector_type(NOUT ? 3 : 4))) float dvec;
+    typedef __attribute__((ext_vector_type(NOUT ? 4 : 3))) float xvec;
+    const int c4 = threadIdx.x & (LPP - 1);
+    const int sub = threadIdx.x / LPP;
+    const int wave = threadIdx.x >> 6;
+    float acc[NV];
+#pragma unroll
+    for (int i = 0; i < NV; ++i) acc[i] = 0.0f;
+    const __amdgpu_buffer_rsrc_t xrs = __builtin_amdgcn_make_buffer_rsrc(
+        const_cast<float*>(a.x), 0, a.N * a.H * a.W * (NOUT ? CW : CN) * 4, 0x00020000);
+    const __amdgpu_buffer_rsrc_t drs = __builtin_amdgcn_make_buffer_rsrc(
+        const_cast<float*>(a.dpre), 0, a.N * a.OH * a.OW * (NOUT ? CN : CW) * 4, 0x00020000);
+    const unsigned p0 = (unsigned)blk * (unsigned)iters * (unsigned)PPI + sub;
+    PixWalk q;
+    q.init(p0 < (unsigned)total_px ? p0 : 0u, a.OH, a.OW);
+    for (int it = 0; it < iters; it += DEPTH) {
+        dvec d[DEPTH];
+        xvec v[DEPTH][TAPS];
+#pragma unroll
+        for (int s = 0; s < DEPTH; ++s, q.step(PPI, a.OH, a.OW)) {
+            const unsigned p = p0 + (unsigned)(it + s) * (unsigned)PPI;
+            const bool live = p < (unsigned)total_px && (DEPTH == 1 || it + s < iters);
+            int off[TAPS];
+            tap_offsets<KH, KW>(off, q, live, a.H, a.W, a.pad_t, a.pad_l, (NOUT ? CW : CN) * 4, NOUT ? 16 * c4 : 0);
+            if constexpr (NOUT) {
+                d[s] = __builtin_bit_cast(f32x3, __builtin_amdgcn_raw_buffer_load_b96(drs, live ? (int)(p * CN * 4) : kOobOffset, 0, 0));
+#pragma unroll
+                for (int tp = 0; tp < TAPS; ++tp)
+                    v[s][tp] = __builtin_bit_cast(f32x4, __builtin_amdgcn_raw_buffer_load_b128(xrs, off[tp], 0, 0));
+            } else {
+                d[s] = __builtin_bit_cast(f32x4, __builtin_amdgcn_raw_buffer_load_b128(
+                    drs, live ? (int)((p * CW + 4 * c4) * 4) : kOobOffset, 0, 0));
+#pragma unroll
+                for (int tp = 0; tp < TAPS; ++tp)
+                    v[s][tp] = __builtin_bit_cast(f32x3, __builtin_amdgcn_raw_buffer_load_b96(xrs, off[tp], 0, 0));
+            }
+        }
+#pragma unroll
+        for (int s = 0; s < DEPTH; ++s) {
+            if constexpr (NOUT) {
+#pragma unroll
+                for (int tp = 0; tp < TAPS; ++tp)
+#pragma unroll
+                    for (int e = 0; e < 4; ++e)
+#pragma unroll
+                        for (int c = 0; c < CN; ++c) acc[(tp * 4 + e) * CN + c] = fmaf(v[s][tp][e], d[s][c], acc[(tp * 4 + e) * CN + c]);
+#pragma unroll
+                for (int c = 0; c < CN; ++c) acc[TAPS * 4 * CN + c] += d[s][c];
+            } else {
+#pragma unroll
+                for (int tp = 0; tp < TAPS; ++tp)
+#pragma unroll
+                    for (int cn = 0; cn < CN; ++cn)
+#pragma unroll
+                        for (int e = 0; e < 4; ++e) acc[(tp * CN + cn) * 4 + e] = fmaf(v[s][tp][cn], d[s][e], acc[(tp * CN + cn) * 4 + e]);
+#pragma unroll
+                for (int e = 0; e < 4; ++e) acc[TAPS * 4 * CN + e] += d[s][e];
+            }
+        }
+    }
+#pragma unroll
+    for (int i = 0; i < NV; ++i) {
+        float r = acc[i];
+#pragma unroll
+        for (int o = LPP; o < 64; o <<= 1) r += __shfl_xor(r, o);
+        if (sub % (64 / LPP) == 0) red[(wave * NV + i) * LPP + c4] = r;
+    }
+    __syncthreads();
+    const int wn = TAPS * CW * CN;
+    for (int q = threadIdx.x; q < NV * LPP; q += 256) {
+        const int i = q / LPP, l = q % LPP;
+        const float r = (red[(0 * NV + i) * LPP + l] + red[(1 * NV + i) * LPP + l]) +
+                        (red[(2 * NV + i) * LPP + l] + red[(3 * NV + i) * LPP + l]);
+        if (i < TAPS * 4 * CN) {
+            int idx;
+            if constexpr (NOUT) {
+                const int c = i % CN, te = i / CN, e = te & 3, tp = te >> 2;
+                idx = (tp * CW + 4 * l + e) * CN + c;
+            } else {
+                const int e = i & 3, tc = i >> 2;
+                idx = tc * CW + 4 * l + e;
+            }
+            part[idx] = r;
+        } else {
+            const int b = i - TAPS * 4 * CN;
+            if constexpr (NOUT) {
+                if (l == 0) part[wn + b] = r;
+            } else {
+                part[wn + 4 * l + b] = r;
+            }
+        }
+    }
+}
+}
diff --git a/ml_super_resolution_amd/engine.py b/ml_super_resolution_amd/engine.py
--- a/ml_super_resolution_amd/engine.py
+++ b/ml_super_resolution_amd/engine.py
@@ -71,6 +71,7 @@
         self.forward_keep_hook = None
         self._bufs = {}
         self._ws = None
+        self._ws_side = None
         self.grad_hook = None
         self.loss_kind = 'mse'
         self._decay_mask = None
@@ -264,11 +265,25 @@
             self._step_graphs.clear()
             self._ws = torch.empty((need + 3) // 4, dtype=torch.float32, device=self.device)
         chain = self._dgrad_chain(acts)
+        side = None
+        if batch is not None and chain is not None and batch[0] >= 1 and chain[0] <= batch[0] <= chain[1] and prec[batch[0] - 1] == 'highest':
+            sl = batch[0] - 1
+            side_args = (acts[batch[0]].shape, self.specs[batch[0]].kernel_shape, batch[1] - batch[0] + 1, acts[sl].shape,
+                         self.specs[sl].kernel_shape, self.specs[batch[0]].padding)
+            if self.specs[sl].padding == self.specs[batch[0]].padding and ops.bwd_filter_batch_side_plan(*side_args)[0] > 0:
+                side = sl
+                sneed = ops.bwd_filter_batch_side_workspace_bytes(*side_args)
+                if self._ws_side is None or self._ws_side.numel() * 4 < sneed:
+                    self._step_graphs.clear()
+                    self._ws_side = torch.empty((sneed + 3) // 4, dtype=torch.float32, device=self.device)
         in_batch = lambda k: batch is not None and batch[0] <= k <= batch[1]
         dpres = {}
-
-        def wgrad(i, dpre_i):
+        side_done = [False]
+
+        def wgrad(i, dpre_i, dpre_below=None):
             s = self.specs[i]
+            if i == side and side_done[0]:
+                return
             if not in_batch(i):
                 ops.conv2d_bwd_filter(acts[i], dpre_i, s.kernel_shape, s.padding,
                                       w_for_decay=self.kernel(i) if self.weight_decay else None,
@@ -278,10 +293,14 @@
             dpres[i] = dpre_i
             if i == batch[0]:
                 ks = list(range(batch[0], batch[1] + 1))
-                ops.conv2d_bwd_filter_batch([acts[k] for k in ks], [dpres[k] for k in ks], [self.kernel(k, self.grads) for k in ks],
-                                            [self.bias(k, self.grads) for k in ks],
-                                            [self.kernel(k) for k in ks] if self.weight_decay else None, self.weight_decay,
-                                            s.padding, workspace=self._ws)
+                lists = ([acts[k] for k in ks], [dpres[k] for k in ks], [self.kernel(k, self.grads) for k in ks],
+                         [self.bias(k, self.grads) for k in ks], [self.kernel(k) for k in ks] if self.weight_decay else None)
+                if side is not None and dpre_below is not None:
+                    side_done[0] = ops.conv2d_bwd_filter_batch_side(
+                        *lists, self.weight_decay, self._ws, acts[side], dpre_below, self.kernel(side, self.grads),
+                        self.bias(side, self.grads), self.kernel(side) if self.weight_decay else None, self._ws_side, s.padding) > 0
+                else:
+                    ops.conv2d_bwd_filter_batch(*lists, self.weight_decay, s.padding, workspace=self._ws)
 
         for i in range(last, -1, -1):
             s = self.specs[i]
@@ -295,7 +314,7 @@
                     cdpres = {hi: dpre}
                     for k in range(hi, lo - 1, -1):
                         cdpres[k - 1] = outs[hi - k]
-                wgrad(i, cdpres[i])
+                wgrad(i, cdpres[i], cdpres.get(i - 1))
                 if i == lo:
                     dpre = cdpres[lo - 1]
                 continue
diff --git a/ml_super_resolution_amd/espcn/model_espcn.py b/ml_super_resolution_amd/espcn/model_espcn.py
--- a/ml_super_resolution_amd/espcn/model_espcn.py
+++ b/ml_super_resolution_amd/espcn/model_espcn.py
@@ -1,4 +1,5 @@
 import os
+import weakref
 
 import numpy as np
 import torch
@@ -33,7 +34,8 @@
 
         self.use_single_launch_train = os.environ.get('SRX_ESPCN_FUSED_TRAIN', '1') != '0'
         self.single_launch_train_max_pixels = int(os.environ.get('SRX_ESPCN_FUSED_TRAIN_MAX_PIXELS', '30000'))
-        self.stack.forward_keep_hook = self._forward_keep_one_launch
+        me = weakref.ref(self)
+        self.stack.forward_keep_hook = lambda x, outs: me() is not None and me()._forward_keep_one_launch(x, outs)
         self.stack.step_graph_max_pixels = int(os.environ.get('SRX_ESPCN_STEP_GRAPH_MAX_PIXELS', '12000'))
 
     def _forward_keep_one_launch(self, x, outs):
diff --git a/ml_super_resolution_amd/ops.py b/ml_super_resolution_amd/ops.py
--- a/ml_super_resolution_amd/ops.py
+++ b/ml_super_resolution_amd/ops.py
@@ -233,6 +233,53 @@
 
 def set_wgrad_batch(on):
     return lib().srx_set_wgrad_batch(int(on))
+
+
+def bwd_filter_batch_side_plan(x_shape, w_shape, n_layers, side_x_shape, side_w_shape, padding='same'):
+    d = conv_desc(x_shape, w_shape, padding)
+    sd = conv_desc(side_x_shape, side_w_shape, padding)
+    n, parts = ctypes.c_int(0), ctypes.c_int(0)
+    _load_lib().srx_conv2d_bwd_filter_batch_side_plan(ctypes.byref(d), int(n_layers), ctypes.byref(sd), ctypes.byref(n), ctypes.byref(parts))
+    return n.value, parts.value
+
+
+def bwd_filter_batch_side_workspace_bytes(x_shape, w_shape, n_layers, side_x_shape, side_w_shape, padding='same'):
+    d = conv_desc(x_shape, w_shape, padding)
+    sd = conv_desc(side_x_shape, side_w_shape, padding)
+    return _load_lib().srx_conv2d_bwd_filter_batch_side_workspace_bytes(ctypes.byref(d), int(n_layers), ctypes.byref(sd))
+
+
+def conv2d_bwd_filter_batch_side(xs, dpres, dws, dbiases, w_for_decay, wd_scale, workspace, side_x, side_dpre, side_dw, side_dbias=None,
+                                 side_w_for_decay=None, side_workspace=None, padding='same'):
+    L = len(xs)
+    if not (len(dpres) == len(dws) == L) or (dbiases is not None and len(dbiases) != L) or (w_for_decay is not None and len(w_for_decay) != L):
+        raise ValueError('conv2d_bwd_filter_batch_side: the per-layer lists differ in length')
+    for l in range(L):
+        _chk(xs[l], 'x'); _chk(dpres[l], 'dpre'); _chk(dws[l], 'dw')
+        _chk(None if dbiases is None else dbiases[l], 'dbias'); _chk(None if w_for_decay is None else w_for_decay[l], 'w_for_decay')
+    for t, n in ((side_x, 'side_x'), (side_dpre, 'side_dpre'), (side_dw, 'side_dw'), (side_dbias, 'side_dbias'),
+                 (side_w_for_decay, 'side_w_for_decay'), (workspace, 'workspace'), (side_workspace, 'side_workspace')):
+        _chk(t, n)
+    d = conv_desc(xs[0].shape, dws[0].shape, padding)
+    sd = conv_desc(side_x.shape, side_dw.shape, padding)
+    for l in range(L):
+        if tuple(xs[l].shape) != tuple(xs[0].shape) or tuple(dpres[l].shape) != tuple(out_shape(d)) or tuple(dws[l].shape) != tuple(dws[0].shape):
+            raise ValueError('conv2d_bwd_filter_batch_side: layer %d does not have the shape of layer 0' % l)
+    if tuple(side_dpre.shape) != tuple(out_shape(sd)):
+        raise ValueError('side_dpre has shape %s, the side layer output is %s' % (tuple(side_dpre.shape), tuple(out_shape(sd))))
+    n = ctypes.c_int(0)
+    check(lib().srx_conv2d_bwd_filter_batch_side(ctypes.byref(d), L, _ptr_array(xs), _ptr_array(dpres), _ptr_array(dws),
+                                                 None if dbiases is None else _ptr_array(dbiases),
+                                                 None if w_for_decay is None else _ptr_array(w_for_decay), float(wd_scale),
+                                                 _ptr(workspace), workspace.numel() * 4, ctypes.byref(sd), _ptr(side_x), _ptr(side_dpre),
+                                                 _ptr(side_dw), _ptr(side_dbias), _ptr(side_w_for_decay), _ptr(side_workspace),
+                                                 0 if side_workspace is None else side_workspace.numel() * 4, ctypes.byref(n), _stream()),
+          'srx_conv2d_bwd_filter_batch_side')
+    return n.value
+
+
+def set_wgrad_side(on):
+    return lib().srx_set_wgrad_side(int(on))
 
 
 def act_bwd(dy, y, act, out=None):
```
